# adolliou/euispice_coreg

Hardware: AMD Instinct MI355X
Metric: lag-points/sec (whole node) on 2048² grid, 60×60 CRVAL sweep; argmax-shift match (higher is better)
Workload: dtype f64; 1 GPU; headline: Carrington 'fa' 2048x2048 grid lon(200,300) lat(-20,20), 60x60 CRVAL lags arange(-30,30,1) arcsec, small 2048^2 HRIEUV-like, ref 3072^2 FSI-like, order 2, solar_r 1.004; lag_points=3600, parallelism=single GPU, no collective, resident=True, sweeps_in_flight=2, small_stored_f32=True, use_lds=True

## Files before the change

### euispice_coreg_amd/_lib.py

```python
from __future__ import annotations

import ctypes as C
import os

import numpy as np

_HERE = os.path.dirname(os.path.abspath(__file__))
LIB_PATH = os.environ.get("COREG_HIP_LIB", os.path.join(_HERE, "libcoreg_hip.so"))

COREG_OK = 0
COREG_EINVAL, COREG_EHIP, COREG_ESTATE, COREG_ENOTIMPL, COREG_ENOMEM = -1, -2, -3, -4, -5
COREG_F32, COREG_F64 = 0, 1
PROJ_TAN, PROJ_CAR = 0, 1
METHOD_CORRELATION, METHOD_RESIDUS = 0, 1
CDELT_INTENDED, CDELT_REFERENCE = 0, 1


class CoregError(RuntimeError):
    def __init__(self, code, msg):
        super().__init__(f"libcoreg_hip error {code}: {msg}")
        self.code = code


class Wcs2d(C.Structure):
    _fields_ = [("naxis1", C.c_int32), ("naxis2", C.c_int32),
                ("crpix1", C.c_double), ("crpix2", C.c_double),
                ("crval1", C.c_double), ("crval2", C.c_double),
                ("cdelt1", C.c_double), ("cdelt2", C.c_double),
                ("pc1_1", C.c_double), ("pc1_2", C.c_double), ("pc2_1", C.c_double), ("pc2_2", C.c_double),
                ("crota", C.c_double), ("unit_to_deg", C.c_double), ("lonpole", C.c_double),
                ("dsun_obs", C.c_double), ("crln_obs", C.c_double), ("crlt_obs", C.c_double),
                ("latpole", C.c_double), ("proj", C.c_int32), ("reserved", C.c_int32)]


class Lags(C.Structure):
    _fields_ = [("crval1", C.POINTER(C.c_double)), ("n_crval1", C.c_int32),
                ("crval2", C.POINTER(C.c_double)), ("n_crval2", C.c_int32),
                ("cdelt1", C.POINTER(C.c_double)), ("n_cdelt1", C.c_int32),
                ("cdelt2", C.POINTER(C.c_double)), ("n_cdelt2", C.c_int32),
                ("crota", C.POINTER(C.c_double)), ("n_crota", C.c_int32)]


class CarrGrid(C.Structure):
    _fields_ = [("lon0", C.c_double), ("lon1", C.c_double), ("n_lon", C.c_int32),
                ("lat0", C.c_double), ("lat1", C.c_double), ("n_lat", C.c_int32),
                ("lat_cos", C.POINTER(C.c_float)), ("lat_sin", C.POINTER(C.c_float))]


class DiffRot(C.Structure):
    _fields_ = [("delta_t_days", C.c_double), ("c0", C.c_double), ("c1", C.c_double), ("c2", C.c_double)]


class Stats(C.Structure):
    _fields_ = [("sweep_kernel_ms", C.c_double), ("precompute_ms", C.c_double), ("total_gpu_ms", C.c_double),
                ("n_lags", C.c_int64), ("n_grid_points", C.c_int64), ("n_active_points", C.c_int64),
                ("n_sweep_launches", C.c_int64), ("small_is_f32", C.c_int32), ("used_lds", C.c_int32)]


class FitsPixels(C.Structure):
    _fields_ = [("data", C.c_void_p), ("bitpix", C.c_int32), ("reserved", C.c_int32), ("bscale", C.c_double),
                ("bzero", C.c_double)]


class FitsTiled(C.Structure):
    _fields_ = [("heap", C.c_void_p), ("heap_bytes", C.c_int64), ("tile_offset", C.c_void_p), ("tile_nbytes", C.c_void_p),
                ("n_tiles", C.c_int32), ("zbitpix", C.c_int32), ("naxis1", C.c_int32), ("naxis2", C.c_int32),
                ("ztile1", C.c_int32), ("ztile2", C.c_int32), ("blocksize", C.c_int32), ("bytepix", C.c_int32),
                ("quantize", C.c_int32), ("dither0", C.c_int32), ("has_blank", C.c_int32), ("blank", C.c_int32),
                ("zscale", C.c_void_p), ("zzero", C.c_void_p), ("zscale0", C.c_double), ("zzero0", C.c_double),
                ("bscale", C.c_double), ("bzero", C.c_double)]


def _is_tiled(img):
    return hasattr(img, "tile_nbytes") and hasattr(img, "ztile") and getattr(img, "on_gpu", False)


def _fits_tiled(ci):
    off = np.ascontiguousarray(ci.tile_offset, dtype=np.int64)
    nb = np.ascontiguousarray(ci.tile_nbytes, dtype=np.int32)
    keep = [off, nb, ci._heap]
    zs = zz = None
    if ci.zscale is not None and ci.zzero is not None:
        zs = np.ascontiguousarray(ci.zscale, dtype=np.float64)
        zz = np.ascontiguousarray(ci.zzero, dtype=np.float64)
        keep += [zs, zz]
    t = FitsTiled(ci._heap.ctypes.data, int(ci._heap.size), off.ctypes.data, nb.ctypes.data, int(ci.n_tiles), int(ci.zbitpix),
                  int(ci.shape[1]), int(ci.shape[0]), int(ci.ztile[0]), int(ci.ztile[1]), int(ci.blocksize), int(ci.bytepix),
                  int(ci.quantize), int(ci.dither0), int(bool(ci.has_blank)), int(ci.blank),
                  zs.ctypes.data if zs is not None else None, zz.ctypes.data if zz is not None else None,
                  float(ci.zscale0), float(ci.zzero0), float(ci.bscale), float(ci.bzero))
    return t, keep


def decode_tiled_host(ci, out):
    t, keep = _fits_tiled(ci)
    status = np.zeros(ci.n_tiles, dtype=np.int32)
    rc = load_library().coreg_decode_tiled_host(C.byref(t), out.ctypes.data, COREG_F32 if out.dtype == np.float32 else COREG_F64,
                                                status.ctypes.data)
    if rc != COREG_OK:
        raise CoregError(rc, "coreg_decode_tiled_host: bad arguments (unsupported tiling / codec parameters)")
    del keep
    return status


def encode_tiled_host(pixels, tile, bytepix=4, blocksize=32, quantize=0, dither0=1, scale=1.0):
    a = np.ascontiguousarray(pixels)
    if a.ndim != 2:
        raise ValueError("image must be 2-D")
    ny, nx = a.shape
    tx, ty = int(tile[0]), int(tile[1])
    nt = (-(-nx // tx)) * (-(-ny // ty))
    if a.dtype == np.float32:
        dt = COREG_F32
    elif a.dtype == np.float64:
        dt = COREG_F64
    elif a.dtype == np.int32:
        dt = 2
    else:
        raise TypeError("pixels must be float32, float64 or int32 (stored integers)")
    is_float = dt != 2
    n_blocks = nt * (-(-(tx * ty) // int(blocksize)) + 1)
    cap = a.size * int(bytepix) + n_blocks + 8 * nt + 64
    heap = np.empty(cap, dtype=np.uint8)
    nbytes = np.zeros(nt, dtype=np.int32)
    offs = np.zeros(nt, dtype=np.int64)
    zs = np.zeros(nt, dtype=np.float64) if is_float else None
    zz = np.zeros(nt, dtype=np.float64) if is_float else None
    used = C.c_longlong(0)
    rc = load_library().coreg_encode_tiled_host(a.ctypes.data, dt, ny, nx, tx, ty, int(bytepix), int(blocksize), int(quantize),
                                                int(dither0), float(scale), heap.ctypes.data, cap, nbytes.ctypes.data,
                                                offs.ctypes.data, zs.ctypes.data if is_float else None,
                                                zz.ctypes.data if is_float else None, C.byref(used))
    if rc != COREG_OK:
        raise CoregError(rc, "coreg_encode_tiled_host: bad arguments, or a tile's range does not fit 32-bit integers at "
                             "this scale")
    return heap[:used.value].copy(), nbytes, offs, zs, zz


def _is_raw(img):
    return hasattr(img, "bitpix") and hasattr(img, "ptr")


def _fits_pixels(raw) -> FitsPixels:
    if len(raw.shape) != 2:
        raise ValueError("image must be 2-D")
    return FitsPixels(raw.ptr, int(raw.bitpix), 0, float(raw.bscale), float(raw.bzero))


def _image_kind(img):
    if _is_tiled(img):
        return "tiled", int(img.zbitpix) == -32
    if _is_raw(img):
        return "fits", int(img.bitpix) == -32
    return "array", np.asarray(img).dtype == np.float32


def _image_args(img, what="image"):
    kind, f32 = _image_kind(img)
    if kind == "tiled":
        t, keep = _fits_tiled(img)
        return kind, (C.byref(t),), (img, t, keep)
    if kind == "fits":
        px = _fits_pixels(img)
        return kind, (C.byref(px), img.shape[0], img.shape[1]), (img, px)
    if np.ndim(img) != 2:
        raise ValueError(f"{what} must be 2-D")
    a = np.ascontiguousarray(img, dtype=np.float32 if f32 else np.float64)
    return ("f32" if f32 else "f64"), (a.ctypes.data, a.shape[0], a.shape[1]), a


def _sweep_out(n, out_dev_ptr):
    if out_dev_ptr is None:
        out = np.empty(n, dtype=np.float64)
        return out, _P(out.ctypes.data), 0
    return None, _P(int(out_dev_ptr)), 1


_P = C.c_void_p
_WP = C.POINTER(Wcs2d)
SYMBOLS = [
    ("coreg_version", C.c_char_p, []),
    ("coreg_create", C.c_int, [C.POINTER(_P), C.c_int]),
    ("coreg_destroy", None, [_P]),
    ("coreg_last_error", C.c_char_p, [_P]),
    ("coreg_set_stream", C.c_int, [_P, _P]),
    ("coreg_synchronize", C.c_int, [_P]),
    ("coreg_set_small", C.c_int, [_P, _P, C.c_int32, C.c_int32]),
    ("coreg_set_small_f32", C.c_int, [_P, _P, C.c_int32, C.c_int32]),
    ("coreg_set_small_fits", C.c_int, [_P, C.POINTER(FitsPixels), C.c_int32, C.c_int32]),
    ("coreg_prepare_reference_carrington_fits", C.c_int,
     [_P, C.POINTER(FitsPixels), C.c_int32, C.c_int32, _WP, C.POINTER(CarrGrid), C.c_double, C.c_int]),
    ("coreg_prepare_reference_helioprojective_fits", C.c_int,
     [_P, C.POINTER(FitsPixels), C.c_int32, C.c_int32, _WP, _WP, C.c_int]),
    ("coreg_set_small_tiled", C.c_int, [_P, C.POINTER(FitsTiled)]),
    ("coreg_prepare_reference_carrington_tiled", C.c_int,
     [_P, C.POINTER(FitsTiled), _WP, C.POINTER(CarrGrid), C.c_double, C.c_int]),
    ("coreg_prepare_reference_helioprojective_tiled", C.c_int, [_P, C.POINTER(FitsTiled), _WP, _WP, C.c_int]),
    ("coreg_decode_tiled_host", C.c_int, [C.POINTER(FitsTiled), _P, C.c_int, _P]),
    ("coreg_encode_tiled_host", C.c_int, [_P, C.c_int, C.c_int, C.c_int, C.c_int, C.c_int, C.c_int, C.c_int, C.c_int, C.c_int,
                                          C.c_double, _P, C.c_longlong, _P, _P, _P, _P, C.POINTER(C.c_longlong)]),
    ("coreg_threshold_small", C.c_int, [_P, C.c_int, C.c_double, C.c_int, C.c_double, C.POINTER(C.c_longlong)]),
    ("coreg_set_reference_on_grid", C.c_int, [_P, _P, C.c_int, C.c_int32, C.c_int32]),
    ("coreg_prepare_reference_carrington", C.c_int,
     [_P, _P, C.c_int32, C.c_int32, _WP, C.POINTER(CarrGrid), C.c_double, C.c_int]),
    ("coreg_prepare_reference_helioprojective", C.c_int, [_P, _P, C.c_int32, C.c_int32, _WP, _WP, C.c_int]),
    ("coreg_prepare_reference_carrington_f32", C.c_int,
     [_P, _P, C.c_int32, C.c_int32, _WP, C.POINTER(CarrGrid), C.c_double, C.c_int]),
    ("coreg_prepare_reference_helioprojective_f32", C.c_int, [_P, _P, C.c_int32, C.c_int32, _WP, _WP, C.c_int]),
    ("coreg_set_small_from_device", C.c_int, [_P, _P, C.c_int, C.c_int32, C.c_int32]),
    ("coreg_prepare_reference_carrington_from_device", C.c_int,
     [_P, _P, C.c_int, C.c_int32, C.c_int32, _WP, C.POINTER(CarrGrid), C.c_double, C.c_int]),
    ("coreg_prepare_reference_helioprojective_from_device", C.c_int,
     [_P, _P, C.c_int, C.c_int32, C.c_int32, _WP, _WP, C.c_int]),
    ("coreg_get_reference_on_grid", C.c_int, [_P, _P, C.c_int]),
    ("coreg_resample_carrington", C.c_int, [_P, _WP, C.POINTER(CarrGrid), C.c_double, C.c_int, _P]),
    ("coreg_resample_helioprojective", C.c_int, [_P, _WP, _WP, C.c_int, _P]),
    ("coreg_resample_helioprojective_f64", C.c_int, [_P, _WP, _WP, C.c_int, _P]),
    ("coreg_set_reference_rotation", C.c_int, [_P, C.POINTER(DiffRot)]),
    ("coreg_set_small_rotation", C.c_int, [_P, C.POINTER(DiffRot)]),
    ("coreg_sweep_carrington", C.c_int,
     [_P, _WP, C.POINTER(CarrGrid), C.c_double, C.POINTER(Lags), C.c_int, C.c_int, C.c_int, C.c_int64, C.c_int64, _P,
      C.c_int]),
    ("coreg_sweep_helioprojective", C.c_int,
     [_P, _WP, _WP, C.POINTER(Lags), C.c_int, C.c_int, C.c_int, C.c_int64, C.c_int64, _P, C.c_int]),
    ("coreg_sums_size", C.c_int, [_P, C.POINTER(C.c_int64)]),
    ("coreg_copy_sums", C.c_int, [_P, _P, C.c_int]),
    ("coreg_finalize_sums", C.c_int, [_P, _P, C.c_int, _P, C.c_int]),
    ("coreg_get_pivots", C.c_int, [_P, C.POINTER(C.c_double)]),
    ("coreg_set_pivots", C.c_int, [_P, C.POINTER(C.c_double)]),
    ("coreg_last_stats", C.c_int, [_P, C.POINTER(Stats)]),
    ("coreg_last_visit_counts", C.c_int, [_P, C.POINTER(C.c_int64)]),
    ("coreg_last_tap_fix", C.c_int, [_P, C.POINTER(C.c_int64)]),
    ("coreg_set_option", C.c_int, [_P, C.c_char_p, C.c_int64]),
    ("coreg_shift_header", C.c_int,
     [_WP, C.c_double, C.c_double, C.c_double, C.c_double, C.c_double, C.c_int, _WP]),
    ("coreg_homography", C.c_int, [_WP, _WP, C.POINTER(C.c_double)]),
    ("coreg_lag_homography", C.c_int,
     [_WP, _WP, C.POINTER(Lags), C.POINTER(C.c_int32), C.c_int, C.POINTER(C.c_double)]),
    ("coreg_carrington_origin", C.c_int, [_WP, C.POINTER(C.c_double), C.POINTER(C.c_double)]),
    ("coreg_diffrot_table", C.c_int, [C.POINTER(CarrGrid), C.POINTER(DiffRot), _P]),
    ("coreg_car_map", C.c_int, [_WP, _WP, C.c_int64, _P, _P, _P, _P]),
    ("coreg_wcslib_pixel_to_pixel", C.c_int, [_WP, _WP, C.c_int64, _P, _P, _P, _P, _P, _P]),
    ("coreg_car_tile_margin", C.c_int, [_WP, _WP, C.c_int32, C.c_double, C.POINTER(C.c_double)]),
    ("coreg_nansum_planes_be", C.c_int, [_P, C.c_int32, C.c_int64, _P, C.c_int32, _P]),
    ("coreg_fit_gaussian2d", C.c_int,
     [C.c_int32, _P, _P, _P, _P, _P, _P, C.c_int32, C.c_double, C.c_double, C.c_double, C.c_int32, _P,
      C.POINTER(C.c_int32), C.POINTER(C.c_int32)]),
    ("coreg_set_context_frames", C.c_int, [_P, C.c_int32, C.c_int32, C.c_int32, C.c_int, _WP, C.POINTER(_P)]),
    ("coreg_context_frame_from_small", C.c_int, [_P, C.c_int32]),
    ("coreg_sweep_context", C.c_int,
     [_P, _WP, _WP, C.POINTER(C.c_int32), C.POINTER(Lags), C.c_int, C.c_int, C.c_int, C.c_int, C.c_double, C.c_int,
      C.c_double, C.c_int64, C.c_int64, _P, C.c_int]),
    ("coreg_context_lag_headers", C.c_int,
     [_WP, _WP, C.c_double, C.c_double, C.c_double, C.c_double, C.c_double, C.c_int, _WP, _WP, _WP]),
    ("coreg_device_count", C.c_int, []),
    ("coreg_physical_device_count", C.c_int, []),
    ("coreg_multi_create", C.c_int, [C.POINTER(_P), C.c_int, C.POINTER(C.c_int)]),
    ("coreg_multi_destroy", None, [_P]),
    ("coreg_multi_size", C.c_int, [_P]),
    ("coreg_multi_handle", _P, [_P, C.c_int]),
    ("coreg_multi_last_error", C.c_char_p, [_P]),
    ("coreg_multi_collective", C.c_char_p, [_P]),
    ("coreg_multi_rccl_status", C.c_char_p, [_P]),
    ("coreg_multi_last_mode", C.c_int, [_P]),
    ("coreg_multi_set_option", C.c_int, [_P, C.c_char_p, C.c_int64]),
    ("coreg_multi_set_small", C.c_int, [_P, _P, C.c_int, C.c_int32, C.c_int32]),
    ("coreg_multi_set_small_fits", C.c_int, [_P, C.POINTER(FitsPixels), C.c_int32, C.c_int32]),
    ("coreg_multi_prepare_reference_carrington_fits", C.c_int,
     [_P, C.POINTER(FitsPixels), C.c_int32, C.c_int32, _WP, C.POINTER(CarrGrid), C.c_double, C.c_int]),
    ("coreg_multi_prepare_reference_helioprojective_fits", C.c_int,
     [_P, C.POINTER(FitsPixels), C.c_int32, C.c_int32, _WP, _WP, C.c_int]),
    ("coreg_multi_set_small_tiled", C.c_int, [_P, C.POINTER(FitsTiled)]),
    ("coreg_multi_prepare_reference_carrington_tiled", C.c_int,
     [_P, C.POINTER(FitsTiled), _WP, C.POINTER(CarrGrid), C.c_double, C.c_int]),
    ("coreg_multi_prepare_reference_helioprojective_tiled", C.c_int, [_P, C.POINTER(FitsTiled), _WP, _WP, C.c_int]),
    ("coreg_multi_threshold_small", C.c_int, [_P, C.c_int, C.c_double, C.c_int, C.c_double, C.POINTER(C.c_longlong)]),
    ("coreg_multi_set_reference_on_grid", C.c_int, [_P, _P, C.c_int, C.c_int32, C.c_int32]),
    ("coreg_multi_prepare_reference_carrington", C.c_int,
     [_P, _P, C.c_int, C.c_int32, C.c_int32, _WP, C.POINTER(CarrGrid), C.c_double, C.c_int]),
    ("coreg_multi_prepare_reference_helioprojective", C.c_int, [_P, _P, C.c_int, C.c_int32, C.c_int32, _WP, _WP, C.c_int]),
    ("coreg_multi_set_reference_rotation", C.c_int, [_P, C.POINTER(DiffRot)]),
    ("coreg_multi_set_small_rotation", C.c_int, [_P, C.POINTER(DiffRot)]),
    ("coreg_multi_sweep_carrington", C.c_int,
     [_P, _WP, C.POINTER(CarrGrid), C.c_double, C.POINTER(Lags), C.c_int, C.c_int, C.c_int, _P]),
    ("coreg_multi_sweep_helioprojective", C.c_int, [_P, _WP, _WP, C.POINTER(Lags), C.c_int, C.c_int, C.c_int, _P]),
    ("coreg_multi_last_stats", C.c_int, [_P, C.c_int, C.POINTER(Stats)]),
    ("coreg_multi_plan", C.c_int,
     [C.c_int32, C.c_int32, C.c_int64, C.c_int32, C.c_int32, C.POINTER(C.c_int32), C.POINTER(C.c_int32),
      C.POINTER(C.c_int32), C.POINTER(C.c_int32)]),
]

_lib = None


def _preload_torch_hip_runtime():
    import importlib.util
    import sys
    if "torch" in sys.modules or os.environ.get("COREG_NO_TORCH_PRELOAD", "0") == "1":
        return
    try:
        spec = importlib.util.find_spec("torch")
    except (ImportError, ValueError):
        return
    if spec is None or not spec.submodule_search_locations:
        return
    libdir = os.path.join(list(spec.submodule_search_locations)[0], "lib")
    cand = os.path.join(libdir, "libamdhip64.so")
    if os.path.exists(cand):
        try:
            C.CDLL(cand, mode=C.RTLD_GLOBAL)
        except OSError:
            return
        rccl = os.path.join(libdir, "librccl.so")
        if os.path.exists(rccl):
            os.environ.setdefault("COREG_RCCL_LIB", rccl)


def load_library():
    global _lib
    if _lib is not None:
        return _lib
    _preload_torch_hip_runtime()
    if not os.path.exists(LIB_PATH):
        raise ImportError(
            f"{LIB_PATH} not found: the HIP extension has not been built. "
            "Run `python -c 'import __graft_entry__ as g; g.build()'` at the repo root "
            "(hipcc --offload-arch=gfx950). There is no CPU fallback.")
    lib = C.CDLL(LIB_PATH)
    for name, restype, argtypes in SYMBOLS:
        fn = getattr(lib, name)
        fn.restype = restype
        fn.argtypes = argtypes
    _lib = lib
    return lib


_UNIT_TO_DEG = {"deg": 1.0, "arcsec": 1.0 / 3600.0, "arcmin": 1.0 / 60.0, "rad": 180.0 / np.pi, "mas": 1.0 / 3.6e6}


def unit_to_deg(unit) -> float:
    u = str(unit).strip()
    if u not in _UNIT_TO_DEG:
        raise ValueError(f"unsupported CUNIT {unit!r}")
    return _UNIT_TO_DEG[u]


def wcs_from_header(hdr, carrington=False) -> Wcs2d:
    w = Wcs2d()
    if "ZNAXIS1" in hdr:
        w.naxis1, w.naxis2 = int(hdr["ZNAXIS1"]), int(hdr["ZNAXIS2"])
    else:
        w.naxis1, w.naxis2 = int(hdr.get("NAXIS1", 0)), int(hdr.get("NAXIS2", 0))
    w.crpix1, w.crpix2 = float(hdr["CRPIX1"]), float(hdr["CRPIX2"])
    w.crval1, w.crval2 = float(hdr["CRVAL1"]), float(hdr["CRVAL2"])
    w.cdelt1, w.cdelt2 = float(hdr["CDELT1"]), float(hdr["CDELT2"])
    w.pc1_1, w.pc1_2 = float(hdr.get("PC1_1", 1.0)), float(hdr.get("PC1_2", 0.0))
    w.pc2_1, w.pc2_2 = float(hdr.get("PC2_1", 0.0)), float(hdr.get("PC2_2", 1.0))
    w.crota = float(hdr["CROTA"] if "CROTA" in hdr else hdr.get("CROTA2", 0.0))
    u1 = hdr.get("CUNIT1", "deg")
    if str(u1).strip() != str(hdr.get("CUNIT2", u1)).strip():
        raise ValueError("CUNIT1 and CUNIT2 must be equal")
    w.unit_to_deg = unit_to_deg(u1)
    if str(hdr.get("CTYPE1", "")).strip().upper().endswith("-CAR"):
        w.proj = PROJ_CAR
        w.lonpole = float(hdr["LONPOLE"]) if "LONPOLE" in hdr else float("nan")
    else:
        w.proj = PROJ_TAN
        w.lonpole = float(hdr.get("LONPOLE", 180.0))
    w.latpole = float(hdr["LATPOLE"]) if "LATPOLE" in hdr else float("nan")
    if carrington:
        w.dsun_obs = float(hdr["DSUN_OBS"])
        w.crln_obs = float(hdr["CRLN_OBS"])
        w.crlt_obs = float(hdr["CRLT_OBS"])
    return w


def _dptr(a):
    return a.ctypes.data_as(C.POINTER(C.c_double))


class LagSet:

    def __init__(self, crval1, crval2, cdelt1, cdelt2, crota):
        def arr(v):
            return np.ascontiguousarray(np.atleast_1d(np.asarray([0.0] if v is None else v, dtype=np.float64)))

        self.arrays = [arr(crval1), arr(crval2), arr(cdelt1), arr(cdelt2), arr(crota)]
        a = self.arrays
        self.c = Lags(_dptr(a[0]), len(a[0]), _dptr(a[1]), len(a[1]), _dptr(a[2]), len(a[2]), _dptr(a[3]), len(a[3]),
                      _dptr(a[4]), len(a[4]))
        self.shape = tuple(len(x) for x in a)
        self.size = int(np.prod(self.shape))


class Grid:

    def __init__(self, lonlims, latlims, shape, numpy_lat_trig=True):
        self.n_lon, self.n_lat = int(shape[0]), int(shape[1])
        self._cos = self._sin = None
        cp = sp = None
        if numpy_lat_trig:
            lat = np.radians(np.linspace(latlims[0], latlims[1], self.n_lat, dtype=np.float32))
            self._cos = np.ascontiguousarray(np.cos(lat), dtype=np.float32)
            self._sin = np.ascontiguousarray(np.sin(lat), dtype=np.float32)
            cp = self._cos.ctypes.data_as(C.POINTER(C.c_float))
            sp = self._sin.ctypes.data_as(C.POINTER(C.c_float))
        self.c = CarrGrid(float(lonlims[0]), float(lonlims[1]), self.n_lon, float(latlims[0]), float(latlims[1]),
                          self.n_lat, cp, sp)


class _ImageIntake:

    def _intake(self, stem, img, what, *tail):
        kind, args, keep = _image_args(img, what)
        suffix, dtype_arg = self._variants[kind]
        if dtype_arg:
            args = (args[0], COREG_F32 if kind == "f32" else COREG_F64) + args[1:]
        self._chk(getattr(self._lib, self._prefix + stem + suffix)(getattr(self, self._ptr), *args, *tail))
        return kind, keep

    def set_small(self, img):
        previous = getattr(self, "_small_keepalive", None)
        kind, keep = self._intake("set_small", img, "small image")
        if kind in ("fits", "f32"):
            self._small_keepalive = keep
            del previous

    def drop_small_keepalive(self):
        self._small_keepalive = None

    def set_rotation(self, role, rot):
        if role not in ("reference", "small"):
            raise ValueError("role must be 'reference' or 'small'")
        fn = getattr(self._lib, f"{self._prefix}set_{role}_rotation")
        arg = None if rot is None else C.byref(DiffRot(*(float(v) for v in rot)))
        self._chk(fn(getattr(self, self._ptr), arg))

    def prepare_reference_carrington(self, large, hdr_large, grid: Grid, solar_r, order=2):
        w = wcs_from_header(hdr_large, carrington=True)
        self.reference_tag = None
        self._intake("prepare_reference_carrington", large, "reference image", C.byref(w), C.byref(grid.c),
                     float(solar_r), int(order))

    def prepare_reference_helioprojective(self, large, hdr_large, hdr_small, order=2):
        wl, ws = wcs_from_header(hdr_large), wcs_from_header(hdr_small)
        self.reference_tag = None
        self._intake("prepare_reference_helioprojective", large, "reference image", C.byref(wl), C.byref(ws), int(order))


class CoregHandle(_ImageIntake):
    _prefix, _ptr = "coreg_", "_h"
    _variants = {"tiled": ("_tiled", False), "fits": ("_fits", False), "f32": ("_f32", False), "f64": ("", False)}

    def __init__(self, device=-1):
        self._lib = load_library()
        self._h = _P()
        rc = self._lib.coreg_create(C.byref(self._h), int(device))
        if rc != COREG_OK:
            self._h = None
            raise CoregError(rc, "coreg_create failed (no HIP device visible?)")
        self.reference_tag = None

    def close(self):
        if getattr(self, "_h", None):
            self._lib.coreg_destroy(self._h)
            self._h = None

    def __del__(self):
        try:
            self.close()
        except Exception:
            pass

    def __enter__(self):
        return self

    def __exit__(self, *exc):
        self.close()

    def _chk(self, rc):
        if rc != COREG_OK:
            raise CoregError(rc, self._lib.coreg_last_error(self._h).decode("utf-8", "replace"))

    def set_option(self, name, value):
        self._chk(self._lib.coreg_set_option(self._h, name.encode(), int(value)))

    def set_stream(self, stream_ptr):
        self._chk(self._lib.coreg_set_stream(self._h, _P(stream_ptr)))

    def synchronize(self):
        self._chk(self._lib.coreg_synchronize(self._h))

    def threshold_small(self, vmin=None, vmax=None) -> int:
        n = C.c_longlong(0)
        self._chk(self._lib.coreg_threshold_small(self._h, int(vmin is not None), float(vmin or 0.0),
                                                  int(vmax is not None), float(vmax or 0.0), C.byref(n)))
        return int(n.value)

    def set_reference_on_grid(self, ref):
        ref = np.ascontiguousarray(ref)
        if ref.ndim != 2 or ref.dtype not in (np.float32, np.float64):
            raise ValueError("reference on grid must be a 2-D float32/float64 array")
        dt = COREG_F32 if ref.dtype == np.float32 else COREG_F64
        self.reference_tag = None
        self._chk(self._lib.coreg_set_reference_on_grid(self._h, ref.ctypes.data, dt, ref.shape[0], ref.shape[1]))

    @staticmethod
    def _dev_dtype(dtype):
        dt = np.dtype(dtype)
        if dt == np.float32:
            return COREG_F32
        if dt == np.float64:
            return COREG_F64
        raise ValueError("device images must be float32 or float64")

    def set_small_from_device(self, dev_ptr, shape, dtype=np.float32):
        self._chk(self._lib.coreg_set_small_from_device(self._h, _P(int(dev_ptr)), self._dev_dtype(dtype),
                                                        int(shape[0]), int(shape[1])))

    def prepare_reference_carrington_from_device(self, dev_ptr, shape, dtype, hdr_large, grid: Grid, solar_r, order=2):
        w = wcs_from_header(hdr_large, carrington=True)
        self.reference_tag = None
        self._chk(self._lib.coreg_prepare_reference_carrington_from_device(
            self._h, _P(int(dev_ptr)), self._dev_dtype(dtype), int(shape[0]), int(shape[1]), C.byref(w),
            C.byref(grid.c), float(solar_r), int(order)))

    def prepare_reference_helioprojective_from_device(self, dev_ptr, shape, dtype, hdr_large, hdr_small, order=2):
        wl, ws = wcs_from_header(hdr_large), wcs_from_header(hdr_small)
        self.reference_tag = None
        self._chk(self._lib.coreg_prepare_reference_helioprojective_from_device(
            self._h, _P(int(dev_ptr)), self._dev_dtype(dtype), int(shape[0]), int(shape[1]), C.byref(wl), C.byref(ws),
            int(order)))

    def get_reference_on_grid(self, shape, dtype):
        out = np.empty(shape, dtype=dtype)
        dt = COREG_F32 if out.dtype == np.float32 else COREG_F64
        self._chk(self._lib.coreg_get_reference_on_grid(self._h, out.ctypes.data, dt))
        return out

    def resample_carrington(self, hdr, grid: Grid, solar_r, order=2):
        w = wcs_from_header(hdr, carrington=True)
        out = np.empty((grid.n_lat, grid.n_lon), dtype=np.float64)
        self._chk(self._lib.coreg_resample_carrington(self._h, C.byref(w), C.byref(grid.c), float(solar_r), int(order),
                                                      out.ctypes.data))
        return out

    def resample_helioprojective(self, hdr_target, hdr, order=2, dtype=np.float32):
        wt, w = wcs_from_header(hdr_target), wcs_from_header(hdr)
        out = np.empty((wt.naxis2, wt.naxis1), dtype=dtype)
        fn = self._lib.coreg_resample_helioprojective if out.dtype == np.float32 else \
            self._lib.coreg_resample_helioprojective_f64
        self._chk(fn(self._h, C.byref(wt), C.byref(w), int(order), out.ctypes.data))
        return out

    def sweep_carrington(self, hdr_small, grid: Grid, solar_r, lags: LagSet, order=2, method=METHOD_CORRELATION,
                         cdelt_semantics=CDELT_INTENDED, lag_begin=0, lag_end=None, out_dev_ptr=None):
        lag_end = lags.size if lag_end is None else int(lag_end)
        w = wcs_from_header(hdr_small, carrington=True)
        out, ptr, on_dev = _sweep_out(lag_end - lag_begin, out_dev_ptr)
        self._chk(self._lib.coreg_sweep_carrington(self._h, C.byref(w), C.byref(grid.c), float(solar_r),
                                                   C.byref(lags.c), int(order), int(method), int(cdelt_semantics),
                                                   int(lag_begin), lag_end, ptr, on_dev))
        return out

    def sweep_helioprojective(self, hdr_target, hdr_small, lags: LagSet, order=2, method=METHOD_CORRELATION,
                              cdelt_semantics=CDELT_INTENDED, lag_begin=0, lag_end=None, out_dev_ptr=None):
        lag_end = lags.size if lag_end is None else int(lag_end)
        wt, w = wcs_from_header(hdr_target), wcs_from_header(hdr_small)
        out, ptr, on_dev = _sweep_out(lag_end - lag_begin, out_dev_ptr)
        self._chk(self._lib.coreg_sweep_helioprojective(self._h, C.byref(wt), C.byref(w), C.byref(lags.c), int(order),
                                                        int(method), int(cdelt_semantics), int(lag_begin), lag_end,
                                                        ptr, on_dev))
        return out

    def set_context_frames(self, frames, headers, dtype=None):
        frames = list(frames)
        if len(frames) != len(headers) or not frames:
            raise ValueError("one header per frame, at least one frame")

        kinds = [_image_kind(f) for f in frames]
        if dtype is None:
            dtype = np.float32 if all(f32 for _, f32 in kinds) else np.float64
        dtype = np.dtype(dtype)
        shape = tuple(frames[0].shape)
        if any(tuple(f.shape) != shape for f in frames) or len(shape) != 2:
            raise ValueError("all frames must be 2-D images of one shape")
        hdrs = (Wcs2d * len(frames))(*[wcs_from_header(hh) for hh in headers])
        host = []
        ptrs = (_P * len(frames))()
        for k, f in enumerate(frames):
            if kinds[k][0] != "array":
                continue
            a = np.ascontiguousarray(f, dtype=dtype)
            host.append(a)
            ptrs[k] = a.ctypes.data
        self._chk(self._lib.coreg_set_context_frames(self._h, len(frames), shape[0], shape[1],
                                                     COREG_F32 if dtype == np.float32 else COREG_F64, hdrs, ptrs))
        for k, f in enumerate(frames):
            if kinds[k][0] != "array":
                self.set_small(f)
                self._chk(self._lib.coreg_context_frame_from_small(self._h, k))
        self._context_frames = (len(frames), shape, dtype)

    def sweep_context(self, hdr_target, hdr_small, col_frame, lags: LagSet, order=2, method=METHOD_CORRELATION,
                      cdelt_semantics=CDELT_INTENDED, vmin=None, vmax=None, lag_begin=0, lag_end=None, out_dev_ptr=None):
        lag_end = lags.size if lag_end is None else int(lag_end)
        wt, w = wcs_from_header(hdr_target), wcs_from_header(hdr_small)
        cf = np.ascontiguousarray(col_frame, dtype=np.int32)
        if cf.size != w.naxis1:
            raise ValueError("col_frame needs one entry per raster column")
        out, ptr, on_dev = _sweep_out(lag_end - lag_begin, out_dev_ptr)
        self._chk(self._lib.coreg_sweep_context(
            self._h, C.byref(wt), C.byref(w), cf.ctypes.data_as(C.POINTER(C.c_int32)), C.byref(lags.c), int(order),
            int(method), int(cdelt_semantics), int(vmin is not None), float(0.0 if vmin is None else vmin),
            int(vmax is not None), float(0.0 if vmax is None else vmax), int(lag_begin), lag_end, ptr, on_dev))
        return out

    def set_point_shard(self, rank, world):
        self.set_option("shard_world", int(world))
        self.set_option("shard_rank", int(rank))

    def sums_size(self) -> int:
        n = C.c_int64(0)
        self._chk(self._lib.coreg_sums_size(self._h, C.byref(n)))
        return int(n.value)

    def copy_sums(self, dst_ptr=None):
        if dst_ptr is not None:
            self._chk(self._lib.coreg_copy_sums(self._h, _P(int(dst_ptr)), 1))
            return None
        out = np.empty(self.sums_size(), dtype=np.float64)
        self._chk(self._lib.coreg_copy_sums(self._h, out.ctypes.data, 0))
        return out

    def finalize_sums(self, sums, n_out, out_dev_ptr=None):
        if isinstance(sums, np.ndarray):
            sums = np.ascontiguousarray(sums, dtype=np.float64)
            sptr, s_dev = sums.ctypes.data, 0
        else:
            sptr, s_dev = int(sums), 1
        if out_dev_ptr is None:
            out = np.empty(int(n_out), dtype=np.float64)
            self._chk(self._lib.coreg_finalize_sums(self._h, _P(sptr), s_dev, out.ctypes.data, 0))
            return out
        self._chk(self._lib.coreg_finalize_sums(self._h, _P(sptr), s_dev, _P(int(out_dev_ptr)), 1))
        return None

    def get_pivots(self):
        p = (C.c_double * 2)()
        self._chk(self._lib.coreg_get_pivots(self._h, p))
        return float(p[0]), float(p[1])

    def set_pivots(self, pivot_ref, pivot_small):
        p = (C.c_double * 2)(float(pivot_ref), float(pivot_small))
        self._chk(self._lib.coreg_set_pivots(self._h, p))

    def last_stats(self) -> dict:
        s = Stats()
        self._chk(self._lib.coreg_last_stats(self._h, C.byref(s)))
        return {f: getattr(s, f) for f, _ in Stats._fields_}

    def last_visit_counts(self) -> dict:
        c = (C.c_int64 * 6)()
        self._chk(self._lib.coreg_last_visit_counts(self._h, c))
        return {"visits": c[0], "lds": c[1], "interior": c[2], "all_finite": c[3], "refined_lag_points": c[4],
                "flagged_not_refined": c[5]}


    def last_tap_fix(self) -> dict:
        c = (C.c_int64 * 3)()
        self._chk(self._lib.coreg_last_tap_fix(self._h, c))
        return {"samples": c[0], "lag_points": c[1], "overflow": bool(c[2])}


class _HandleView(CoregHandle):

    def __init__(self, lib, ptr):
        self._lib = lib
        self._h = _P(ptr)
        self.reference_tag = None

    def close(self):
        self._h = None


MULTI_MODES = {0: "none", 1: "blocks", 2: "slices", 3: "points", 4: "combos"}


def device_count() -> int:
    return max(0, int(load_library().coreg_device_count()))


def physical_device_count() -> int:
    return max(0, int(load_library().coreg_physical_device_count()))


def multi_plan(n_crval1, n_crval2, n_inner, world, per_combo_launch=True):
    mode, gc, g1, g2 = C.c_int32(), C.c_int32(), C.c_int32(), C.c_int32()
    rc = load_library().coreg_multi_plan(int(n_crval1), int(n_crval2), int(n_inner), int(world), int(per_combo_launch),
                                         C.byref(mode), C.byref(gc), C.byref(g1), C.byref(g2))
    if rc != COREG_OK:
        raise CoregError(rc, "coreg_multi_plan: bad arguments")
    return MULTI_MODES[mode.value], gc.value, g1.value, g2.value


class MultiHandle(_ImageIntake):
    _prefix, _ptr = "coreg_multi_", "_m"
    _variants = {"tiled": ("_tiled", False), "fits": ("_fits", False), "f32": ("", True), "f64": ("", True)}

    def __init__(self, n_devices=0, device_ids=None):
        self._lib = load_library()
        self._m = _P()
        ids = None
        if device_ids is not None:
            ids = (C.c_int * len(device_ids))(*[int(d) for d in device_ids])
            n_devices = len(device_ids)
        rc = self._lib.coreg_multi_create(C.byref(self._m), int(n_devices), ids)
        if rc != COREG_OK:
            self._m = None
            raise CoregError(rc, "coreg_multi_create failed (no HIP device visible?)")
        self.reference_tag = None
        self.size = int(self._lib.coreg_multi_size(self._m))
        self.primary = _HandleView(self._lib, self._lib.coreg_multi_handle(self._m, 0))

    def close(self):
        if getattr(self, "_m", None):
            self.primary.close()
            self._lib.coreg_multi_destroy(self._m)
            self._m = None

    def __del__(self):
        try:
            self.close()
        except Exception:
            pass

    def __enter__(self):
        return self

    def __exit__(self, *exc):
        self.close()

    def _chk(self, rc):
        if rc != COREG_OK:
            raise CoregError(rc, self._lib.coreg_multi_last_error(self._m).decode("utf-8", "replace"))

    @property
    def collective(self) -> str:
        return self._lib.coreg_multi_collective(self._m).decode()

    @property
    def rccl_status(self) -> str:
        return self._lib.coreg_multi_rccl_status(self._m).decode()

    @property
    def last_mode(self) -> str:
        return MULTI_MODES[int(self._lib.coreg_multi_last_mode(self._m))]

    def handle(self, k) -> CoregHandle:
        ptr = self._lib.coreg_multi_handle(self._m, int(k))
        if not ptr:
            raise IndexError(k)
        return _HandleView(self._lib, ptr)

    def set_option(self, name, value):
        self._chk(self._lib.coreg_multi_set_option(self._m, name.encode(), int(value)))

    def synchronize(self):
        for k in range(self.size):
            self.handle(k).synchronize()

    def threshold_small(self, vmin=None, vmax=None) -> int:
        n = C.c_longlong(0)
        self._chk(self._lib.coreg_multi_threshold_small(self._m, int(vmin is not None), float(vmin or 0.0),
                                                        int(vmax is not None), float(vmax or 0.0), C.byref(n)))
        return int(n.value)

    def set_reference_on_grid(self, ref):
        ref = np.ascontiguousarray(ref)
        if ref.ndim != 2 or ref.dtype not in (np.float32, np.float64):
            raise ValueError("reference on grid must be a 2-D float32/float64 array")
        self.reference_tag = None
        self._chk(self._lib.coreg_multi_set_reference_on_grid(
            self._m, ref.ctypes.data, COREG_F32 if ref.dtype == np.float32 else COREG_F64, ref.shape[0], ref.shape[1]))

    def _whole(self, lags, lag_begin, lag_end):
        if int(lag_begin) != 0 or (lag_end is not None and int(lag_end) != lags.size):
            raise ValueError("a multi-GPU sweep covers the whole lag set (the library cuts it itself)")

    def sweep_carrington(self, hdr_small, grid: Grid, solar_r, lags: LagSet, order=2, method=METHOD_CORRELATION,
                         cdelt_semantics=CDELT_INTENDED, lag_begin=0, lag_end=None):
        self._whole(lags, lag_begin, lag_end)
        w = wcs_from_header(hdr_small, carrington=True)
        out = np.empty(lags.size, dtype=np.float64)
        self._chk(self._lib.coreg_multi_sweep_carrington(self._m, C.byref(w), C.byref(grid.c), float(solar_r),
                                                         C.byref(lags.c), int(order), int(method), int(cdelt_semantics),
                                                         out.ctypes.data))
        return out

    def sweep_helioprojective(self, hdr_target, hdr_small, lags: LagSet, order=2, method=METHOD_CORRELATION,
                              cdelt_semantics=CDELT_INTENDED, lag_begin=0, lag_end=None):
        self._whole(lags, lag_begin, lag_end)
        wt, w = wcs_from_header(hdr_target), wcs_from_header(hdr_small)
        out = np.empty(lags.size, dtype=np.float64)
        self._chk(self._lib.coreg_multi_sweep_helioprojective(self._m, C.byref(wt), C.byref(w), C.byref(lags.c),
                                                              int(order), int(method), int(cdelt_semantics),
                                                              out.ctypes.data))
        return out

    def resample_helioprojective(self, hdr_target, hdr, order=2, dtype=np.float32):
        return self.primary.resample_helioprojective(hdr_target, hdr, order=order, dtype=dtype)

    def get_reference_on_grid(self, shape, dtype):
        return self.primary.get_reference_on_grid(shape, dtype)

    def last_stats(self, k=None):
        def one(i):
            s = Stats()
            self._chk(self._lib.coreg_multi_last_stats(self._m, int(i), C.byref(s)))
            return {f: getattr(s, f) for f, _ in Stats._fields_}
        if k is not None:
            return one(k)
        per = [one(i) for i in range(self.size)]
        out = dict(per[0])
        out["per_device_sweep_kernel_ms"] = [p["sweep_kernel_ms"] for p in per]
        out["n_lags"] = sum(p["n_lags"] for p in per) if self.last_mode != "points" else per[0]["n_lags"]
        out["n_devices"] = self.size
        out["collective"] = self.collective
        out["lag_sharding"] = self.last_mode
        return out


_SHARED = {}


def shared_handle(device=-1, slot=0) -> CoregHandle:
    key = (int(device), int(slot))
    h = _SHARED.get(key)
    if h is None or getattr(h, "_h", None) is None:
        h = CoregHandle(device)
        _SHARED[key] = h
    return h


def shared_multi_handle() -> MultiHandle:
    h = _SHARED.get("multi")
    if h is None or getattr(h, "_m", None) is None:
        h = MultiHandle(0)
        _SHARED["multi"] = h
    return h


def _close_shared():
    for h in list(_SHARED.values()):
        try:
            h.close()
        except Exception:
            pass
    _SHARED.clear()


import atexit

atexit.register(_close_shared)


def shift_header(hdr, d_crval1, d_crval2, d_cdelt1, d_cdelt2, d_crota, cdelt_semantics=CDELT_INTENDED):
    lib = load_library()
    w = wcs_from_header(hdr)
    out = Wcs2d()
    rc = lib.coreg_shift_header(C.byref(w), d_crval1, d_crval2, d_cdelt1, d_cdelt2, d_crota, cdelt_semantics,
                                C.byref(out))
    if rc < 0:
        raise CoregError(rc, "coreg_shift_header")
    return rc, out


def homography(hdr_from, hdr_to):
    lib = load_library()
    a, b = wcs_from_header(hdr_from), wcs_from_header(hdr_to)
    h = (C.c_double * 9)()
    rc = lib.coreg_homography(C.byref(a), C.byref(b), h)
    if rc != COREG_OK:
        raise CoregError(rc, "coreg_homography")
    return np.array(h[:]).reshape(3, 3)


def lag_homography(hdr_target, hdr_small, lags: "LagSet", idx, cdelt_semantics=CDELT_INTENDED):
    lib = load_library()
    a, b = wcs_from_header(hdr_target), wcs_from_header(hdr_small)
    ii = (C.c_int32 * 5)(*[int(i) for i in idx])
    h = (C.c_double * 9)()
    rc = lib.coreg_lag_homography(C.byref(a), C.byref(b), C.byref(lags.c), ii, cdelt_semantics, h)
    if rc < 0:
        raise CoregError(rc, "coreg_lag_homography")
    return rc, np.array(h[:]).reshape(3, 3)


def car_map(hdr_from, hdr_to, px, py):
    lib = load_library()
    px = np.ascontiguousarray(px, dtype=np.float64).ravel()
    py = np.ascontiguousarray(py, dtype=np.float64).ravel()
    ox, oy = np.empty_like(px), np.empty_like(py)
    wf, wt = wcs_from_header(hdr_from), wcs_from_header(hdr_to)
    rc = lib.coreg_car_map(C.byref(wf), C.byref(wt), px.size, px.ctypes.data, py.ctypes.data, ox.ctypes.data,
                           oy.ctypes.data)
    if rc == 1:
        return None
    if rc != COREG_OK:
        raise CoregError(rc, "coreg_car_map: bad arguments")
    return ox, oy


def car_tile_margin(hdr_target, hdr_shifted, tile_w, tile_abs_lat_rad):
    lib = load_library()
    wf, wt = wcs_from_header(hdr_target), wcs_from_header(hdr_shifted)
    m = C.c_double()
    rc = lib.coreg_car_tile_margin(C.byref(wf), C.byref(wt), int(tile_w), float(tile_abs_lat_rad), C.byref(m))
    if rc == 1:
        return None
    if rc != COREG_OK:
        raise CoregError(rc, "coreg_car_tile_margin: bad arguments")
    return m.value


def context_lag_headers(hdr_target, hdr_small, d_crval1, d_crval2, d_cdelt1, d_cdelt2, d_crota,
                        cdelt_semantics=CDELT_INTENDED):
    lib = load_library()
    wt, w = wcs_from_header(hdr_target), wcs_from_header(hdr_small)
    out = [Wcs2d(), Wcs2d(), Wcs2d()]
    rc = lib.coreg_context_lag_headers(C.byref(wt), C.byref(w), float(d_crval1), float(d_crval2), float(d_cdelt1),
                                       float(d_cdelt2), float(d_crota), int(cdelt_semantics), *[C.byref(o) for o in out])
    if rc < 0:
        raise CoregError(rc, "coreg_context_lag_headers: bad arguments")
    return None if rc else tuple(out)


def wcs_to_dict(w: Wcs2d) -> dict:
    unit = {v: k for k, v in _UNIT_TO_DEG.items()}.get(w.unit_to_deg, "deg")
    return {"NAXIS1": w.naxis1, "NAXIS2": w.naxis2, "CRPIX1": w.crpix1, "CRPIX2": w.crpix2, "CRVAL1": w.crval1,
            "CRVAL2": w.crval2, "CDELT1": w.cdelt1, "CDELT2": w.cdelt2, "PC1_1": w.pc1_1, "PC1_2": w.pc1_2,
            "PC2_1": w.pc2_1, "PC2_2": w.pc2_2, "CROTA": w.crota, "CUNIT1": unit, "CUNIT2": unit,
            "CTYPE1": "HPLN-TAN", "CTYPE2": "HPLT-TAN", "LONPOLE": w.lonpole}


def wcslib_pixel_to_pixel(hdr_from, hdr_to, px, py):
    lib = load_library()
    px = np.ascontiguousarray(px, dtype=np.float64).ravel()
    py = np.ascontiguousarray(py, dtype=np.float64).ravel()
    out = [np.empty_like(px) for _ in range(4)]
    wf, wt = wcs_from_header(hdr_from), wcs_from_header(hdr_to)
    rc = lib.coreg_wcslib_pixel_to_pixel(C.byref(wf), C.byref(wt), px.size, px.ctypes.data, py.ctypes.data,
                                         *[o.ctypes.data for o in out])
    if rc != COREG_OK:
        raise CoregError(rc, "coreg_wcslib_pixel_to_pixel")
    return tuple(out)


def nansum_planes_be(cube_be, plane_index):
    a = cube_be
    if a.dtype.kind != "f" or a.dtype.byteorder != ">" or a.dtype.itemsize not in (4, 8) or not a.flags.c_contiguous:
        return None
    idx = np.ascontiguousarray(plane_index, dtype=np.int64)
    if idx.size and (idx.min() < 0 or idx.max() >= a.shape[0]):
        raise IndexError("plane index out of range")
    n_pix = int(np.prod(a.shape[1:]))
    out = np.empty(a.shape[1:], dtype=np.float64)
    rc = load_library().coreg_nansum_planes_be(a.ctypes.data, -8 * a.dtype.itemsize, n_pix, idx.ctypes.data, idx.size,
                                               out.ctypes.data)
    if rc != COREG_OK:
        raise CoregError(rc, "coreg_nansum_planes_be: bad arguments")
    return out


def fit_gaussian2d(x, y, z, p0, lb, ub, jac="2-point", ftol=1e-8, xtol=1e-8, gtol=1e-8, max_nfev=0):
    lib = load_library()
    arrs = [np.ascontiguousarray(np.asarray(a, dtype=np.float64).ravel()) for a in (x, y, z, p0, lb, ub)]
    if not (arrs[0].size == arrs[1].size == arrs[2].size) or any(a.size != 6 for a in arrs[3:]):
        raise ValueError("fit_gaussian2d: x, y, z must have one length; p0, lb, ub six entries")
    if jac not in ("2-point", "analytic"):
        raise ValueError("jac must be '2-point' or 'analytic'")
    popt = np.empty(6)
    nfev, status = C.c_int32(0), C.c_int32(0)
    rc = lib.coreg_fit_gaussian2d(arrs[0].size, *[a.ctypes.data for a in arrs], int(jac == "analytic"), float(ftol),
                                  float(xtol), float(gtol), int(max_nfev), popt.ctypes.data, C.byref(nfev),
                                  C.byref(status))
    if rc != COREG_OK:
        raise CoregError(rc, "coreg_fit_gaussian2d: bad arguments (sizes, bounds, or p0 outside the bounds)")
    return popt, int(status.value), int(nfev.value)


def diffrot_table(grid: Grid, rot):
    out = np.empty(grid.n_lat, dtype=np.float64)
    r = DiffRot(*(float(v) for v in rot))
    rc = load_library().coreg_diffrot_table(C.byref(grid.c), C.byref(r), out.ctypes.data)
    if rc != COREG_OK:
        raise CoregError(rc, "coreg_diffrot_table: bad grid, or a non-finite delta_t / coefficient")
    return out


def carrington_origin(hdr):
    lib = load_library()
    w = wcs_from_header(hdr, carrington=True)
    x0, y0 = C.c_double(), C.c_double()
    rc = lib.coreg_carrington_origin(C.byref(w), C.byref(x0), C.byref(y0))
    if rc != COREG_OK:
        raise CoregError(rc, "coreg_carrington_origin")
    return x0.value, y0.value
```

### euispice_coreg_amd/csrc/abi_host.hpp

```cpp
#pragma once
extern "C" {
int coreg_shift_header(const coreg_wcs2d* ref, double d_crval1, double d_crval2, double d_cdelt1, double d_cdelt2,
                       double d_crota, int cdelt_semantics, coreg_wcs2d* out) {
    if (!ref || !out) return COREG_EINVAL;
    return shift_header(*ref, d_crval1, d_crval2, d_cdelt1, d_cdelt2, d_crota, cdelt_semantics, out);
}

int coreg_car_map(const coreg_wcs2d* from, const coreg_wcs2d* to, int64_t n, const double* px, const double* py,
                  double* ox, double* oy) {
    if (!from || !to || n < 0 || (n > 0 && (!px || !py || !ox || !oy))) return COREG_EINVAL;
    if (from->proj != COREG_PROJ_CAR || to->proj != COREG_PROJ_CAR) return COREG_EINVAL;
    CarMapHost m;
    if (m.init(*from, *to)) return 1;
    for (int64_t i = 0; i < n; ++i) m.apply(px[i], py[i], &ox[i], &oy[i]);
    return COREG_OK;
}

int coreg_last_visit_counts(coreg_handle* h, int64_t* counts6) {
    int64_t* counts5 = counts6;
    if (!h || !counts5) return COREG_EINVAL;
    RETCHK(bind_device(h));
    HIPCHK(hipStreamSynchronize(h->stream));
    long long info[8] = {0, 0, 0, 0, 0, 0, 0, 0};
    if (h->tile_info.p) HIPCHK(hipMemcpy(info, h->tile_info.p, 7 * sizeof(long long), hipMemcpyDeviceToHost));
    for (int k = 0; k < 4; ++k) counts5[k] = info[3 + k];
    long long refined[2] = {0, 0};
    if (h->counters.p) HIPCHK(hipMemcpy(refined, h->counters.p, sizeof(refined), hipMemcpyDeviceToHost));
    counts5[4] = refined[0];
    counts6[5] = refined[1];
    return COREG_OK;
}

int coreg_last_tap_fix(coreg_handle* h, int64_t* counts3) {
    if (!h || !counts3) return COREG_EINVAL;
    for (int k = 0; k < 3; ++k) counts3[k] = h->tap_last[k];
    return COREG_OK;
}

int coreg_car_tile_margin(const coreg_wcs2d* hdr_target, const coreg_wcs2d* hdr_shifted, int32_t tile_w,
                          double tile_abs_lat_rad, double* margin_px) {
    if (!hdr_target || !hdr_shifted || !margin_px || tile_w < 1 || tile_w > kTilePts) return COREG_EINVAL;
    if (hdr_target->proj != COREG_PROJ_CAR || hdr_shifted->proj != COREG_PROJ_CAR) return COREG_EINVAL;
    CarMapHost m;
    if (m.init(*hdr_target, *hdr_shifted)) return 1;
    *margin_px = car_tile_margin(car_box_c(*hdr_target, *hdr_shifted, tile_w), tile_abs_lat_rad + car_pole_sep(m.r));
    return COREG_OK;
}

int coreg_homography(const coreg_wcs2d* from, const coreg_wcs2d* to, double* h9) {
    if (!from || !to || !h9) return COREG_EINVAL;
    if (from->proj != COREG_PROJ_TAN || to->proj != COREG_PROJ_TAN) return COREG_ENOTIMPL;
    homography(*from, *to, h9);
    return COREG_OK;
}

int coreg_lag_homography(const coreg_wcs2d* hdr_target, const coreg_wcs2d* hdr_small, const coreg_lags* lags,
                         const int32_t idx[5], int cdelt_semantics, double* h9) {
    if (!hdr_target || !hdr_small || !lags || !idx || !h9) return COREG_EINVAL;
    if (hdr_target->proj != COREG_PROJ_TAN || hdr_small->proj != COREG_PROJ_TAN) return COREG_ENOTIMPL;
    if (idx[0] < 0 || idx[0] >= lags->n_crval1 || idx[1] < 0 || idx[1] >= lags->n_crval2 || idx[2] < 0 ||
        idx[2] >= lags->n_cdelt1 || idx[3] < 0 || idx[3] >= lags->n_cdelt2 || idx[4] < 0 || idx[4] >= lags->n_crota)
        return COREG_EINVAL;
    coreg_wcs2d hc;
    if (shift_header(*hdr_small, 0.0, 0.0, lags->cdelt1[idx[2]], lags->cdelt2[idx[3]], lags->crota[idx[4]],
                     cdelt_semantics, &hc))
        return 1;
    HomographyFamily fam;
    fam.init(*hdr_target, *hdr_small, lags->crval1, lags->n_crval1, lags->crval2, lags->n_crval2);
    fam.get(HomographyFamily::combo(hc), idx[0], idx[1], h9);
    return COREG_OK;
}

int coreg_wcslib_pixel_to_pixel(const coreg_wcs2d* from, const coreg_wcs2d* to, int64_t n, const double* px,
                                const double* py, double* ox, double* oy, double* lng, double* lat) {
    if (!from || !to || n < 0 || (n > 0 && (!px || !py || !ox || !oy))) return COREG_EINVAL;
    if (from->proj == COREG_PROJ_CAR && to->proj == COREG_PROJ_CAR) {
        WcslibCar a, b;
        a.init(*from);
        b.init(*to);
        if (!a.valid || !b.valid) return COREG_EINVAL;
        for (int64_t i = 0; i < n; ++i) {
            double l, t;
            a.p2s(px[i], py[i], &l, &t);
            if (lng) lng[i] = l;
            if (lat) lat[i] = t;
            b.s2p(l, t, &ox[i], &oy[i]);
        }
        return COREG_OK;
    }
    if (from->proj != COREG_PROJ_TAN || to->proj != COREG_PROJ_TAN) return COREG_ENOTIMPL;
    WcslibTan a, b;
    a.init(*from);
    b.init(*to);
    for (int64_t i = 0; i < n; ++i) {
        double l, t;
        a.p2s(px[i], py[i], &l, &t);
        if (lng) lng[i] = l;
        if (lat) lat[i] = t;
        b.s2p(ang2pipi_deg(l), ang2pipi_deg(t), &ox[i], &oy[i]);
    }
    return COREG_OK;
}

int coreg_carrington_origin(const coreg_wcs2d* hdr, double* x0, double* y0) {
    if (!hdr || !x0 || !y0) return COREG_EINVAL;
    carr_origin(*hdr, x0, y0);
    return COREG_OK;
}

int coreg_diffrot_table(const coreg_carr_grid* grid, const coreg_diffrot* rot, double* dx) {
    if (!grid || !rot || !dx || grid->n_lon < 1 || grid->n_lat < 1 || !diffrot_valid(*rot)) return COREG_EINVAL;
    CarrTables t;
    carr_tables(*grid, 0.0, t);
    std::vector<double> v;
    diffrot_dx(t.sin_lat.data(), grid->n_lat, *rot, v);
    std::copy(v.begin(), v.end(), dx);
    return COREG_OK;
}

int coreg_nansum_planes_be(const void* cube, int32_t bitpix, int64_t n_pixels, const int64_t* plane_index, int32_t n_sel,
                           double* out) {
    if (!cube || !out || n_pixels < 0 || n_sel < 0 || (n_sel > 0 && !plane_index) || (bitpix != -32 && bitpix != -64))
        return COREG_EINVAL;
    for (int k = 0; k < n_sel; ++k)
        if (plane_index[k] < 0) return COREG_EINVAL;
    auto work = [&](int64_t lo, int64_t hi) {
        for (int64_t p = lo; p < hi; ++p) out[p] = 0.0;
        for (int k = 0; k < n_sel; ++k) {
            if (bitpix == -32) {
                const uint32_t* src = (const uint32_t*)cube + (size_t)plane_index[k] * (size_t)n_pixels;
                for (int64_t p = lo; p < hi; ++p) {
                    const uint32_t u = __builtin_bswap32(src[p]);
                    float f;
                    std::memcpy(&f, &u, sizeof(f));
                    const double v = (double)f;
                    out[p] += (v != v) ? 0.0 : v;
                }
            } else {
                const uint64_t* src = (const uint64_t*)cube + (size_t)plane_index[k] * (size_t)n_pixels;
                for (int64_t p = lo; p < hi; ++p) {
                    const uint64_t u = __builtin_bswap64(src[p]);
                    double v;
                    std::memcpy(&v, &u, sizeof(v));
                    out[p] += (v != v) ? 0.0 : v;
                }
            }
        }
    };
    parallel_for(n_pixels, (unsigned)std::min<int64_t>(12, n_pixels * std::max(n_sel, 1) / (1 << 18)), 0, work);
    return COREG_OK;
}

int coreg_fit_gaussian2d(int32_t m, const double* x, const double* y, const double* z, const double* p0,
                         const double* lb, const double* ub, int32_t jac, double ftol, double xtol, double gtol,
                         int32_t max_nfev, double* popt, int32_t* nfev, int32_t* status) {
    if (!x || !y || !z || !p0 || !lb || !ub || !popt || !status || m < 1 || m > coregfit::MMAX) return COREG_EINVAL;
    coregfit::Problem P{m, x, y, z};
    int n = 0;
    const int st = coregfit::fit(P, p0, lb, ub, jac != 0, ftol > 0 ? ftol : 1e-8, xtol > 0 ? xtol : 1e-8,
                                 gtol > 0 ? gtol : 1e-8, max_nfev, popt, &n, nullptr);
    if (st == -2) return COREG_EINVAL;
    if (nfev) *nfev = n;
    *status = st;
    return COREG_OK;
}

}
```

### euispice_coreg_amd/csrc/abi_sweeps.hpp

```cpp
#pragma once
namespace {
struct SweepCall {
    const coreg_lags* lags = nullptr;
    LagDims d;
    int order = 0, method = 0, sem = 0;
    long long lag_begin = 0, lag_end = 0, n_out = 0;
    double* corr_out = nullptr;
    int out_on_device = 0;
    double* out_dev = nullptr;
    long long row() const { return (long long)d.n2 * d.nc; }
    int i1_lo() const { return (int)(lag_begin / row()); }
    int i1_hi() const { return (int)((lag_end - 1) / row()); }
};

template <typename OwnChecks>
int open_sweep(coreg_handle* h, ComboRange combo, OwnChecks own_checks, const coreg_lags* lags, int order, int method,
               int sem, int64_t lag_begin, int64_t lag_end, int grid_w, int grid_h, const char* grid_what,
               double* corr_out, int out_on_device, SweepCall* call) {
    if (method != COREG_METHOD_CORRELATION && method != COREG_METHOD_RESIDUS)
        return fail(h, COREG_ENOTIMPL, "method must be COREG_METHOD_CORRELATION or COREG_METHOD_RESIDUS");
    RETCHK(check_order(h, order));
    RETCHK(own_checks());
    RETCHK(check_lags(h, lags, &call->d, lag_begin, lag_end, combo));
    RETCHK(bind_device_nowait(h));
    if (h->ref.p && (h->gW != grid_w || h->gH != grid_h))
        return fail(h, COREG_EINVAL, std::string("reference-on-grid shape differs from ") + grid_what);
    call->lags = lags;
    call->order = order;
    call->method = method;
    call->sem = sem;
    call->lag_begin = lag_begin;
    call->lag_end = lag_end;
    call->n_out = lag_end - lag_begin;
    call->corr_out = corr_out;
    call->out_on_device = out_on_device;
    return begin_sweep(h, call->n_out, corr_out, out_on_device, &call->out_dev);
}

int close_sweep(coreg_handle* h, const SweepCall& call) {
    return end_sweep(h, call.n_out, call.corr_out, call.out_on_device, call.out_dev);
}

int close_empty_sweep(coreg_handle* h, const SweepCall& call) {
    RETCHK(fill_nan(h, call.out_dev, call.n_out));
    return close_sweep(h, call);
}

template <typename MapAt>
Geometry local_geometry(const coreg_wcs2d& target, const SweepCall& call, MapAt at) {
    const coreg_lags& l = *call.lags;
    int e1[3], e2[3];
    extreme_lags(l.crval1, call.d.n1, e1);
    extreme_lags(l.crval2, call.d.n2, e2);
    const double v1 = l.crval1[e1[1]], v2 = l.crval2[e2[1]];
    const double s1 = lag_step(l.crval1, call.d.n1), s2 = lag_step(l.crval2, call.d.n2);
    const double u = target.naxis1 * 0.5, v = target.naxis2 * 0.5;
    double x0, y0, xi, yi, xj, yj, xa, ya, xb, yb;
    Geometry g;
    if (!at(v1, v2, u, v, &x0, &y0) || !at(v1, v2, u + 1, v, &xi, &yi) || !at(v1, v2, u, v + 1, &xj, &yj) ||
        !at(v1 + s1, v2, u, v, &xa, &ya) || !at(v1, v2 + s2, u, v, &xb, &yb))
        return g;
    g.dx_di = xi - x0;
    g.dy_di = yi - y0;
    g.dx_dj = xj - x0;
    g.dy_dj = yj - y0;
    g.ax = xa - x0;
    g.ay = ya - y0;
    g.bx = xb - x0;
    g.by = yb - y0;
    return g;
}

Plan plan_sweep(coreg_handle* h, const Geometry& geo, const SweepCall& call) {
    return choose_plan(h, geo, call.i1_hi() - call.i1_lo() + 1, call.d.n2, h->opt_use_lds ? lds_window_elems(h) : (1LL << 40));
}

bool combo_slots(const SweepCall& call, const coreg_wcs2d& small, const Plan& plan, long long c, coreg_wcs2d* hc,
                 SlotList* slots) {
    const long long first = (call.lag_begin - c + call.d.nc - 1) / call.d.nc;
    if (first * call.d.nc + c >= call.lag_end) return false;
    int i3, i4, i5;
    call.d.inner(c, &i3, &i4, &i5);
    if (shift_header(small, 0.0, 0.0, call.lags->cdelt1[i3], call.lags->cdelt2[i4], call.lags->crota[i5], call.sem, hc))
        return false;
    build_slots(call.d, c, call.lag_begin, call.lag_end, plan.sw, plan.sh, slots);
    return slots->n_batches > 0;
}

template <int MODE>
int precompute(coreg_handle* h, const PrecomputeArgs& pa, int n_tiles, int n_groups, int n_batches, bool launch = true) {
    if (launch) RETCHK(launch_precompute<MODE>(h, pa, n_tiles, n_groups, n_batches));
    h->last_precompute = [pa, n_tiles, n_groups, n_batches](coreg_handle* hh) {
        return launch_precompute<MODE>(hh, pa, n_tiles, n_groups, n_batches);
    };
    return COREG_OK;
}

int finalize_pending(coreg_handle* h, const coreg_handle::PendingFinalize& pf, long long* refine_count, double* out_dev,
                     FinalizeArgs* f) {
    *f = FinalizeArgs{};
    RETCHK(fill_refine(h, &f->refine, pf.refine.mode, pf.refine.order, pf.refine.lane_params, pf.refine.car_inv,
                       pf.n_slots));
    f->refine.enabled = pf.refine.enabled;
    f->refine_count = refine_count;
    f->partials = h->sums.as<double>() + pf.slot_off;
    f->n_groups = 1;
    f->n_slots = pf.n_slots;
    f->part_stride = h->sums_slots;
    f->out_index = h->fin_outidx.as<long long>() + pf.slot_off;
    f->lag_begin = pf.lag_begin;
    f->out = out_dev;
    f->residus = pf.residus;
    f->n_required = (long long)h->gW * h->gH;
    hipLaunchKernelGGL(k_finalize, dim3((unsigned)((pf.n_slots + kFinSlots - 1) / kFinSlots)),
                       dim3(kFinSlots * kFinLanes), 0, h->stream, *f);
    return COREG_OK;
}
}

extern "C" {
int coreg_sweep_carrington(coreg_handle* h, const coreg_wcs2d* hdr_small, const coreg_carr_grid* grid, double solar_r,
                           const coreg_lags* lags, int order, int method, int cdelt_semantics, int64_t lag_begin,
                           int64_t lag_end, double* corr_out, int out_on_device) {
    if (!h) return COREG_EINVAL;
    const ComboRange combo = take_combo_range(h);
    trace("sweep_carrington: enter");
    if (!hdr_small || !grid) return fail(h, COREG_EINVAL, "sweep_carrington: null header/grid");
    auto own_checks = [&] {
        RETCHK(check_wcs(h, hdr_small, true));
        RETCHK(check_grid(h, grid));
        if (!std::isfinite(solar_r) || !(solar_r > 0.0)) return fail(h, COREG_EINVAL, "solar_r must be positive");
        return COREG_OK;
    };
    SweepCall call;
    RETCHK(open_sweep(h, combo, own_checks, lags, order, method, cdelt_semantics, lag_begin, lag_end, grid->n_lon,
                      grid->n_lat, "the Carrington grid", corr_out, out_on_device, &call));
    if (call.n_out == 0) return close_sweep(h, call);
    const LagDims& d = call.d;

    CarrDev cd;
    std::memset(&cd, 0, sizeof(cd));
    RETCHK(upload_carr_tables(h, *grid, *hdr_small, &cd, h->has_rot_small ? &h->rot_small : nullptr));
    double row_slip = 0.0;
    for (size_t j = 1; j < h->tabs.dx.size(); ++j)
        row_slip = std::max(row_slip, std::fabs(h->tabs.dx[j] - h->tabs.dx[j - 1]));
    row_slip *= kDeg2Rad * (1.0 + 1e-9);

    Geometry geo;
    {
        const CarrCommon c0 = carr_common(*hdr_small, solar_r);
        const int ic = grid->n_lon / 2, jc = grid->n_lat / 2;
        double a0, a1, b0, b1, c0x, c0y;
        carr_term_host(h->tabs, c0, ic, jc, &a0, &a1);
        carr_term_host(h->tabs, c0, std::min(ic + 1, grid->n_lon - 1), jc, &b0, &b1);
        carr_term_host(h->tabs, c0, ic, std::min(jc + 1, grid->n_lat - 1), &c0x, &c0y);
        geo.dx_di = b0 - a0;
        geo.dy_di = b1 - a1;
        geo.dx_dj = c0x - a0;
        geo.dy_dj = c0y - a1;
        const double s1 = lag_step(lags->crval1, d.n1), s2 = lag_step(lags->crval2, d.n2);
        geo.ax = c0.cr * s1 / hdr_small->cdelt1;
        geo.ay = c0.sr * s1 / hdr_small->cdelt2;
        geo.bx = c0.sr * s2 / hdr_small->cdelt1;
        geo.by = c0.cr * s2 / hdr_small->cdelt2;
    }
    const Plan plan = plan_sweep(h, geo, call);
    PrecomputeArgs pa;
    int n_tiles;
    RETCHK(setup_precompute(h, plan, method, &pa, &n_tiles));

    struct Launch {
        size_t slot_off;
        int n_batches;
        CarrCommon cc;
        double f0lo, f0hi, f1lo, f1hi;
    };
    std::vector<Launch> launches;
    std::vector<double> params;
    std::vector<long long> outidx;
    SlotList slots;
    for (long long c = 0; c < d.nc; ++c) {
        coreg_wcs2d hc;
        if (!combo_slots(call, *hdr_small, plan, c, &hc, &slots)) continue;
        const size_t ns = slots.i1.size();
        Launch L;
        L.slot_off = outidx.size();
        L.n_batches = slots.n_batches;
        L.cc = carr_common(hc, solar_r);
        const size_t pbase = params.size();
        params.resize(pbase + 2 * ns);
        double x0min = 1e300, x0max = -1e300, y0min = 1e300, y0max = -1e300;
        const double roll = hc.crota * kDeg2Rad;
        const double rc = std::cos(roll), rs = std::sin(roll);
        const double nan = std::numeric_limits<double>::quiet_NaN();
        for (size_t s = 0; s < ns; ++s) {
            if (slots.outidx[s] < 0) {
                params[pbase + s] = nan;
                params[pbase + ns + s] = nan;
                continue;
            }
            const double v1 = hdr_small->crval1 + lags->crval1[slots.i1[s]];
            const double v2 = hdr_small->crval2 + lags->crval2[slots.i2[s]];
            const double dx = rc * v1 + rs * v2;
            const double dy = -rs * v1 + rc * v2;
            const double x0 = (hc.crpix1 - 1) - dx / hc.cdelt1;
            const double y0 = (hc.crpix2 - 1) - dy / hc.cdelt2;
            params[pbase + s] = x0;
            params[pbase + ns + s] = y0;
            x0min = std::min(x0min, x0);
            x0max = std::max(x0max, x0);
            y0min = std::min(y0min, y0);
            y0max = std::max(y0max, y0);
        }
        outidx.insert(outidx.end(), slots.outidx.begin(), slots.outidx.end());
        L.f0lo = -x0max;
        L.f0hi = (double)(h->sW - 1) - x0min;
        L.f1lo = -y0max;
        L.f1hi = (double)(h->sH - 1) - y0min;
        launches.push_back(L);
    }
    if (launches.empty()) return close_empty_sweep(h, call);
    RETCHK(upload_plan(h, params, outidx, call.out_dev, call.n_out));
    RETCHK(prepare_sharded(h, outidx.size(), call.n_out, lag_begin));
    for (const Launch& L : launches) {
        set_carr_common(&cd, L.cc);
        pa.carr = cd;
        pa.f0lo = L.f0lo;
        pa.f0hi = L.f0hi;
        pa.f1lo = L.f1lo;
        pa.f1hi = L.f1hi;
        {
            const double dm1 = L.cc.dist - 1.0;
            pa.tile_skip = (h->opt_tile_skip && dm1 > 0.0) ? 1 : 0;
            const double per_rad = pa.tile_skip ? (1.0 / dm1 + 1.0 / (dm1 * dm1)) * kRad2Deg * 3600.0 : 0.0;
            pa.lip_x = per_rad / std::fabs(L.cc.cdelt1) * (1.0 + 1e-9);
            pa.lip_y = per_rad / std::fabs(L.cc.cdelt2) * (1.0 + 1e-9);
            pa.dlon = grid->n_lon > 1 ? (std::fabs(grid->lon1 - grid->lon0) / (grid->n_lon - 1) * 1.001 + 1e-4) * kDeg2Rad : 0.0;
            pa.dlat = grid->n_lat > 1 ? (std::fabs(grid->lat1 - grid->lat0) / (grid->n_lat - 1) * 1.001 + 1e-4) * kDeg2Rad : 0.0;
            pa.dlat += row_slip;
        }
        RETCHK(precompute<MODE_TRANSLATE>(h, pa, n_tiles, pick_groups(h, L.n_batches, n_tiles), L.n_batches));
        RETCHK(launch_sweep(h, MODE_TRANSLATE, order, method, h->lane_params.as<double>() + 2 * L.slot_off,
                            h->out_index.as<long long>() + L.slot_off, L.n_batches, n_tiles, lag_begin, call.out_dev,
                            nullptr, nullptr, (long long)L.slot_off,
                            pick_pitch(h, plan, h->opt_use_lds ? lds_window_elems(h) : 0, order)));
    }
    return close_sweep(h, call);
}

static int sweep_car(coreg_handle* h, const SweepCall& call, const coreg_wcs2d* hdr_target, const coreg_wcs2d* hdr_small) {
    const coreg_lags* lags = call.lags;
    const LagDims& d = call.d;
    const int order = call.order;
    Mat3 r_target;
    if (car_native_to_celestial(*hdr_target, &r_target))
        return fail(h, COREG_EINVAL, "hdr_target: no valid native pole for this CRVAL2 / LONPOLE (CAR)");
    auto shifted_by = [&](const coreg_wcs2d& base, double v1, double v2) {
        coreg_wcs2d hl = base;
        hl.crval1 = hdr_small->crval1 + v1;
        hl.crval2 = hdr_small->crval2 + v2;
        return hl;
    };
    auto shifted = [&](const coreg_wcs2d& base, int i1, int i2) {
        return shifted_by(base, lags->crval1[i1], lags->crval2[i2]);
    };
    const Plan plan = plan_sweep(h, local_geometry(*hdr_target, call, [&](double v1, double v2, double u, double v,
                                                                        double* x, double* y) {
        CarMapHost m;
        if (m.init(*hdr_target, shifted_by(*hdr_small, v1, v2))) return false;
        m.apply(u, v, x, y);
        return true;
    }), call);

    const int i1_lo = call.i1_lo(), i1_hi = call.i1_hi();
    std::vector<double> rot((size_t)(i1_hi - i1_lo + 1) * d.n2 * 9);
    const double nanv = std::numeric_limits<double>::quiet_NaN();
    for (int i1 = i1_lo; i1 <= i1_hi; ++i1)
        for (int i2 = 0; i2 < d.n2; ++i2) {
            double* r = &rot[((size_t)(i1 - i1_lo) * d.n2 + i2) * 9];
            Mat3 rs;
            if (car_native_to_celestial(shifted(*hdr_small, i1, i2), &rs)) {
                for (int k = 0; k < 9; ++k) r[k] = nanv;
                continue;
            }
            const Mat3 m = mat_mul(mat_T(rs), r_target);
            for (int a = 0; a < 3; ++a)
                for (int b = 0; b < 3; ++b) r[3 * a + b] = (double)m.m[a][b];
        }

    struct Launch {
        size_t slot_off;
        int n_batches;
        LaunchU inv;
        bool identity;
        coreg_wcs2d hc;
        std::vector<int> i1, i2;
        std::vector<unsigned char> tap_skip;
        bool tap_any = false;
    };
    std::vector<Launch> launches;
    std::vector<double> params;
    std::vector<long long> outidx;
    SlotList slots;
    long long identity_out = -1;
    BorderFix id_fix;
    std::vector<std::vector<unsigned char>> id_flags;
    auto same_header = [](const coreg_wcs2d& a, const coreg_wcs2d& b) {
        auto eq = [](double x, double y) { return x == y || (x != x && y != y); };
        return a.proj == b.proj && a.crpix1 == b.crpix1 && a.crpix2 == b.crpix2 && a.crval1 == b.crval1 &&
               a.crval2 == b.crval2 && a.cdelt1 == b.cdelt1 && a.cdelt2 == b.cdelt2 && a.pc1_1 == b.pc1_1 &&
               a.pc1_2 == b.pc1_2 && a.pc2_1 == b.pc2_1 && a.pc2_2 == b.pc2_2 && a.unit_to_deg == b.unit_to_deg &&
               eq(a.lonpole, b.lonpole) && eq(a.latpole, b.latpole) && a.naxis1 == b.naxis1 && a.naxis2 == b.naxis2;
    };
    for (long long c = 0; c < d.nc; ++c) {
        coreg_wcs2d hc;
        if (!combo_slots(call, *hdr_small, plan, c, &hc, &slots)) continue;
        const size_t ns = slots.i1.size();
        Launch L;
        L.slot_off = outidx.size();
        L.n_batches = slots.n_batches;
        std::memset(&L.inv, 0, sizeof(L.inv));
        set_affine(&L.inv, car_native_to_pix(hc));
        L.inv.box_c = car_box_c(*hdr_target, hc, plan.tile_w);
        L.inv.pole_sep = 0.0;
        L.identity = false;
        const size_t pbase = params.size();
        params.resize(pbase + 9 * ns);
        for (size_t s = 0; s < ns; ++s) {
            bool pad = slots.outidx[s] < 0;
            if (!pad && h->opt_border_fix && identity_out < 0 && h->gW == h->sW && h->gH == h->sH) {
                const coreg_wcs2d hl = shifted(hc, slots.i1[s], slots.i2[s]);
                if (same_header(hl, *hdr_target)) {
                    identity_out = slots.outidx[s];
                    slots.outidx[s] = -1;
                    pad = true;
                }
            }
            const double* r = &rot[((size_t)(slots.i1[s] - i1_lo) * d.n2 + slots.i2[s]) * 9];
            for (int k = 0; k < 9; ++k) params[pbase + (size_t)k * ns + s] = pad ? nanv : r[k];
            if (!pad && r[8] == r[8]) L.inv.pole_sep = std::max(L.inv.pole_sep, car_pole_sep(r));
            unsigned char skip = 1;
            if (!pad && h->opt_tap_fix && r[8] == r[8] && h->gW == h->sW && h->gH == h->sH) {
                const coreg_wcs2d hl = shifted(hc, slots.i1[s], slots.i2[s]);
                if (hl.crval1 == hdr_target->crval1 || hl.crval2 == hdr_target->crval2) skip = 0;
            }
            L.tap_skip.push_back(skip);
            L.tap_any = L.tap_any || !skip;
        }
        L.hc = hc;
        L.i1 = slots.i1;
        L.i2 = slots.i2;
        outidx.insert(outidx.end(), slots.outidx.begin(), slots.outidx.end());
        launches.push_back(L);
    }
    if (identity_out >= 0) {
        Launch L;
        std::memset(&L.inv, 0, sizeof(L.inv));
        L.slot_off = outidx.size();
        L.n_batches = 1;
        L.identity = true;
        const size_t ns = kBlock, pbase = params.size();
        params.resize(pbase + 9 * ns, nanv);
        const double ident[9] = {1, 0, 0, 0, 1, 0, 0, 0, 1};
        for (int k = 0; k < 9; ++k) params[pbase + (size_t)k * ns] = ident[k];
        outidx.push_back(identity_out);
        outidx.insert(outidx.end(), ns - 1, -1);
        launches.push_back(L);
        {
            AxisInvariance inv;
            inv.rows = inv.cols = true;
            BorderFix::Item it;
            it.slot = 0;
            it.first = 0;
            wcslib_dropped_border_pixels(h, *hdr_target, *hdr_target, inv, &id_fix.pixels);
            it.n = (int)id_fix.pixels.size();
            it.flags_off = -1;
            if (order & 1) {
                it.flags_off = 0;
                id_flags.push_back(wcslib_tap_shift_flags(h, *hdr_target, *hdr_target, inv));
            }
            if (it.n > 0 || it.flags_off >= 0) id_fix.items.push_back(it);
        }
    }
    if (launches.empty()) return close_empty_sweep(h, call);
    trace("sweep_helioprojective: lane parameters laid out");
    RETCHK(upload_plan(h, params, outidx, call.out_dev, call.n_out));
    RETCHK(prepare_sharded(h, outidx.size(), call.n_out, call.lag_begin));
    trace("sweep_helioprojective: plan in page-locked memory");

    PrecomputeArgs pa;
    int n_tiles;
    RETCHK(setup_precompute(h, plan, call.method, &pa, &n_tiles));
    set_affine(&pa.car_fwd, car_pix_to_native(*hdr_target));
    const double inf = std::numeric_limits<double>::infinity();
    pa.f0lo = pa.f1lo = -inf;
    pa.f0hi = pa.f1hi = inf;
    if (!id_fix.items.empty()) RETCHK(upload_border_pixels(h, id_fix.pixels));
    RETCHK(upload_border_flags(h, id_flags));
    int last_groups = -1, last_batches = -1;
    for (const Launch& L : launches) {
        if (L.identity) {
            PrecomputeArgs pi = pa;
            std::memset(&pi.car_fwd, 0, sizeof(pi.car_fwd));
            RETCHK(precompute<MODE_HOMOGRAPHY>(h, pi, n_tiles, pick_groups(h, 1, n_tiles), 1));
            last_groups = last_batches = -1;
            RETCHK(launch_sweep(h, MODE_HOMOGRAPHY, order, call.method, h->lane_params.as<double>() + 9 * L.slot_off,
                                h->out_index.as<long long>() + L.slot_off, 1, n_tiles, call.lag_begin, call.out_dev, nullptr,
                                &id_fix, (long long)L.slot_off));
            continue;
        }
        const int ng = pick_groups(h, L.n_batches, n_tiles);
        RETCHK(precompute<MODE_CAR>(h, pa, n_tiles, ng, L.n_batches, ng != last_groups || L.n_batches != last_batches));
        last_groups = ng;
        last_batches = L.n_batches;
        BorderFix tap;
        if (L.tap_any) {
            const double box[4] = {0.0, (double)(h->gW - 1), 0.0, (double)(h->gH - 1)};
            h->tap_last[0] = h->tap_last[1] = h->tap_last[2] = 0;
            RETCHK(prepare_tap_fix(
                h, MODE_CAR, order, *hdr_target, (long long)L.tap_skip.size(), L.tap_skip, box,
                [&](int slot) { return shifted(L.hc, L.i1[(size_t)slot], L.i2[(size_t)slot]); }, &tap,
                h->lane_params.as<double>() + 9 * L.slot_off, &L.inv, &pa.car_fwd));
        }
        RETCHK(launch_sweep(h, MODE_CAR, order, call.method, h->lane_params.as<double>() + 9 * L.slot_off,
                            h->out_index.as<long long>() + L.slot_off, L.n_batches, n_tiles, call.lag_begin, call.out_dev,
                            &L.inv, L.tap_any ? &tap : nullptr, (long long)L.slot_off));
    }
    return close_sweep(h, call);
}

int coreg_sweep_helioprojective(coreg_handle* h, const coreg_wcs2d* hdr_target, const coreg_wcs2d* hdr_small,
                                const coreg_lags* lags, int order, int method, int cdelt_semantics, int64_t lag_begin,
                                int64_t lag_end, double* corr_out, int out_on_device) {
    if (!h) return COREG_EINVAL;
    const ComboRange combo = take_combo_range(h);
    if (!hdr_target || !hdr_small) return fail(h, COREG_EINVAL, "sweep_helioprojective: null header");
    if (hdr_target->proj != hdr_small->proj || (hdr_small->proj != COREG_PROJ_TAN && hdr_small->proj != COREG_PROJ_CAR))
        return fail(h, COREG_ENOTIMPL, "both headers must be TAN (helioprojective) or both CAR (Carrington maps)");
    auto own_checks = [&] {
        RETCHK(check_wcs(h, hdr_target, false));
        return check_wcs(h, hdr_small, false);
    };
    SweepCall call;
    RETCHK(open_sweep(h, combo, own_checks, lags, order, method, cdelt_semantics, lag_begin, lag_end,
                      hdr_target->naxis1, hdr_target->naxis2, "hdr_target NAXIS1/NAXIS2", corr_out, out_on_device, &call));
    if (call.n_out == 0) return close_sweep(h, call);
    if (hdr_small->proj == COREG_PROJ_CAR) return sweep_car(h, call, hdr_target, hdr_small);
    const LagDims& d = call.d;

    trace("sweep_helioprojective: enter (checks done)");
    const Plan plan = plan_sweep(h, local_geometry(*hdr_target, call, [&](double v1, double v2, double u, double v,
                                                                        double* x, double* y) {
        coreg_wcs2d hl = *hdr_small;
        hl.crval1 = hdr_small->crval1 + v1;
        hl.crval2 = hdr_small->crval2 + v2;
        double hm[9];
        homography(*hdr_target, hl, hm);
        apply_h(hm, u, v, x, y);
        return true;
    }), call);

    std::vector<long long> outidx;
    int n_batches = 0;
    double fx0 = 1e300, fx1 = -1e300, fy0 = 1e300, fy1 = -1e300;
    HomographyFamily fam;
    fam.init(*hdr_target, *hdr_small, lags->crval1, d.n1, lags->crval2, d.n2, d.nc > 1);
    BorderFix fix;
    std::vector<std::vector<unsigned char>> flags_host;
    const bool tap_fixing = h->opt_tap_fix != 0;
    std::vector<coreg_wcs2d> tap_combo;
    std::vector<int> tap_slot_combo, tap_slot_i1, tap_slot_i2;
    std::vector<unsigned char> tap_skip;
    const int i1_lo = call.i1_lo(), i1_hi = call.i1_hi();
    fam.fill_products(i1_lo, i1_hi);
    const double nanv = std::numeric_limits<double>::quiet_NaN();
    struct ComboPlan {
        bool used = false;
        coreg_wcs2d hc;
        SlotList slots;
        std::vector<double> hs;
        double box[4] = {1e300, -1e300, 1e300, -1e300};
    };
    std::vector<ComboPlan> cps((size_t)d.nc);
    int e1[3], e2[3];
    extreme_lags(lags->crval1 + i1_lo, i1_hi - i1_lo + 1, e1);
    extreme_lags(lags->crval2, d.n2, e2);
    auto plan_combo = [&](long long c) {
        ComboPlan& cp = cps[(size_t)c];
        cp.used = combo_slots(call, *hdr_small, plan, c, &cp.hc, &cp.slots);
        if (!cp.used) return;
        const Mat3d B = HomographyFamily::combo(cp.hc);
        const size_t n = cp.slots.i1.size();
        cp.hs.resize(9 * n);
        for (size_t s = 0; s < n; ++s) {
            double* hm = &cp.hs[9 * s];
            if (cp.slots.outidx[s] < 0) {
                for (int k = 0; k < 9; ++k) hm[k] = nanv;
            } else {
                fam.get(B, cp.slots.i1[s], cp.slots.i2[s], hm);
            }
        }
        for (int a1 = 0; a1 < 3; ++a1)
            for (int a2 = 0; a2 < 3; ++a2) {
                coreg_wcs2d hl = cp.hc;
                hl.crval1 = hdr_small->crval1 + lags->crval1[i1_lo + e1[a1]];
                hl.crval2 = hdr_small->crval2 + lags->crval2[e2[a2]];
                double hi[9];
                homography(hl, *hdr_target, hi);
                for (int k = 0; k < 4; ++k) {
                    double px, py;
                    apply_h(hi, (k & 1) ? (double)(h->sW - 1) : 0.0, (k & 2) ? (double)(h->sH - 1) : 0.0, &px, &py);
                    cp.box[0] = std::min(cp.box[0], px);
                    cp.box[1] = std::max(cp.box[1], px);
                    cp.box[2] = std::min(cp.box[2], py);
                    cp.box[3] = std::max(cp.box[3], py);
                }
            }
    };
    trace("sweep_helioprojective: geometry + lag family ready");
    const unsigned plan_threads = (d.nc >= 2 && (long long)d.nc * d.n1 * d.n2 >= 16384) ? 8u : 1u;
    parallel_for(d.nc, plan_threads, 1, [&](long long lo, long long hi) {
        for (long long c = lo; c < hi; ++c) plan_combo(c);
    });
    for (long long c = 0; c < d.nc; ++c) {
        ComboPlan& cp = cps[(size_t)c];
        if (!cp.used) continue;
        const SlotList& slots = cp.slots;
        const coreg_wcs2d& hc = cp.hc;
        if (tap_fixing) {
            tap_combo.push_back(hc);
            for (size_t s = 0; s < slots.i1.size(); ++s) {
                tap_slot_combo.push_back((int)tap_combo.size() - 1);
                tap_slot_i1.push_back(slots.outidx[s] < 0 ? 0 : slots.i1[s]);
                tap_slot_i2.push_back(slots.outidx[s] < 0 ? 0 : slots.i2[s]);
                tap_skip.push_back(slots.outidx[s] < 0 ? 1 : 0);
            }
        }
        if (h->opt_border_fix) {
            for (size_t s = 0; s < slots.i1.size(); ++s) {
                if (slots.outidx[s] < 0) continue;
                const double v1 = hdr_small->crval1 + lags->crval1[slots.i1[s]];
                const double v2 = hdr_small->crval2 + lags->crval2[slots.i2[s]];
                if (v1 != hdr_target->crval1 || v2 != hdr_target->crval2) continue;
                coreg_wcs2d hl = hc;
                hl.crval1 = v1;
                hl.crval2 = v2;
                double* hm = &cp.hs[9 * s];
                const AxisInvariance inv = snap_invariant_axes(*hdr_target, hl, h->gW, h->gH, hm);
                if (inv.rows || inv.cols) {
                    BorderFix::Item it;
                    it.slot = (long long)(outidx.size() + s);
                    it.first = (int)fix.pixels.size();
                    wcslib_dropped_border_pixels(h, *hdr_target, hl, inv, &fix.pixels);
                    it.n = (int)fix.pixels.size() - it.first;
                    it.flags_off = -1;
                    if (order & 1) {
                        it.flags_off = (long long)flags_host.size() * h->gW * h->gH;
                        flags_host.push_back(wcslib_tap_shift_flags(h, *hdr_target, hl, inv));
                    }
                    if (it.n > 0 || it.flags_off >= 0) fix.items.push_back(it);
                    if (tap_fixing) tap_skip[(size_t)it.slot] = 1;
                }
            }
        }
        fx0 = std::min(fx0, cp.box[0]);
        fx1 = std::max(fx1, cp.box[1]);
        fy0 = std::min(fy0, cp.box[2]);
        fy1 = std::max(fy1, cp.box[3]);
        outidx.insert(outidx.end(), slots.outidx.begin(), slots.outidx.end());
        n_batches += slots.n_batches;
    }
    if (n_batches == 0) return close_empty_sweep(h, call);
    trace("sweep_helioprojective: combinations planned");
    const size_t ns = outidx.size();
    std::vector<double> params(9 * ns);
    double eps_max = 0.0;
    {
        std::vector<size_t> off((size_t)d.nc + 1, 0);
        for (long long c = 0; c < d.nc; ++c) off[(size_t)c + 1] = off[(size_t)c] + (cps[(size_t)c].used ? cps[(size_t)c].slots.i1.size() : 0);
        std::vector<double> eps_of((size_t)d.nc, 0.0);
        auto transpose = [&](long long c) {
            const ComboPlan& cp = cps[(size_t)c];
            if (!cp.used) return;
            const size_t n = cp.slots.i1.size(), at = off[(size_t)c];
            double em = 0.0;
            for (size_t s = 0; s < n; ++s) {
                const double* hm = &cp.hs[9 * s];
                for (int k = 0; k < 9; ++k) params[(size_t)k * ns + at + s] = hm[k];
                const double e = std::fabs(hm[6]) * (double)h->gW + std::fabs(hm[7]) * (double)h->gH;
                if (e == e) em = std::max(em, e);
            }
            eps_of[(size_t)c] = em;
        };
        parallel_for(d.nc, plan_threads, 1, [&](long long lo, long long hi) {
            for (long long c = lo; c < hi; ++c) transpose(c);
        });
        for (double e : eps_of) eps_max = std::max(eps_max, e);
    }
    const int sweep_mode = (h->opt_h_series && eps_max < 4.0e-6) ? MODE_HOMOGRAPHY_SERIES : MODE_HOMOGRAPHY;
    RETCHK(upload_plan(h, params, outidx, call.out_dev, call.n_out));
    RETCHK(prepare_sharded(h, outidx.size(), call.n_out, lag_begin));

    PrecomputeArgs pa;
    int n_tiles;
    RETCHK(setup_precompute(h, plan, method, &pa, &n_tiles));
    pa.f0lo = std::floor(fx0) - 3.0;
    pa.f0hi = std::ceil(fx1) + 3.0;
    pa.f1lo = std::floor(fy0) - 3.0;
    pa.f1hi = std::ceil(fy1) + 3.0;
    if (!fix.items.empty()) RETCHK(upload_border_pixels(h, fix.pixels));
    RETCHK(upload_border_flags(h, flags_host));
    RETCHK(precompute<MODE_HOMOGRAPHY>(h, pa, n_tiles, pick_groups(h, n_batches, n_tiles), n_batches));
    h->tap_last[0] = h->tap_last[1] = h->tap_last[2] = 0;
    const double tap_box[4] = {pa.f0lo, pa.f0hi, pa.f1lo, pa.f1hi};
    trace("sweep_helioprojective: precompute launched");
    if (tap_fixing)
        RETCHK(prepare_tap_fix(
            h, sweep_mode, order, *hdr_target, (long long)ns, tap_skip, tap_box,
            [&](int slot) {
                coreg_wcs2d hl = tap_combo[(size_t)tap_slot_combo[(size_t)slot]];
                hl.crval1 = hdr_small->crval1 + lags->crval1[tap_slot_i1[(size_t)slot]];
                hl.crval2 = hdr_small->crval2 + lags->crval2[tap_slot_i2[(size_t)slot]];
                return hl;
            },
            &fix));
    trace("sweep_helioprojective: single-sample scan done");
    RETCHK(launch_sweep(h, sweep_mode, order, method, h->lane_params.as<double>(), h->out_index.as<long long>(), n_batches,
                        n_tiles, lag_begin, call.out_dev, nullptr, &fix, 0,
                        pick_pitch(h, plan, h->opt_use_lds ? lds_window_elems(h) : 0, order)));
    return close_sweep(h, call);
}


int coreg_sums_size(coreg_handle* h, int64_t* n_doubles) {
    if (!h || !n_doubles) return COREG_EINVAL;
    *n_doubles = (int64_t)h->sums_slots * kNumSums;
    return COREG_OK;
}

int coreg_copy_sums(coreg_handle* h, double* dst, int dst_on_device) {
    if (!h || !dst) return COREG_EINVAL;
    if (h->sums_slots <= 0 || h->pending_fin.empty()) return fail(h, COREG_ESTATE, "no point-sharded sweep is pending");
    RETCHK(bind_device(h));
    const size_t bytes = (size_t)h->sums_slots * kNumSums * sizeof(double);
    HIPCHK(hipMemcpyAsync(dst, h->sums.p, bytes, dst_on_device ? hipMemcpyDeviceToDevice : hipMemcpyDeviceToHost,
                          h->stream));
    if (!dst_on_device) HIPCHK(hipStreamSynchronize(h->stream));
    return COREG_OK;
}

int coreg_finalize_sums(coreg_handle* h, const double* sums, int sums_on_device, double* corr_out, int out_on_device) {
    if (!h || !sums) return COREG_EINVAL;
    if (h->sums_slots <= 0 || h->pending_fin.empty()) return fail(h, COREG_ESTATE, "no point-sharded sweep is pending");
    if (!corr_out && h->pending_n_out > 0) return fail(h, COREG_EINVAL, "corr_out is null");
    RETCHK(bind_device(h));
    const long long n_out = h->pending_n_out;
    const size_t bytes = (size_t)h->sums_slots * kNumSums * sizeof(double);
    if ((const void*)sums != h->sums.p) {
        HIPCHK(hipMemcpyAsync(h->sums.p, sums, bytes, sums_on_device ? hipMemcpyDeviceToDevice : hipMemcpyHostToDevice,
                              h->stream));
        if (!sums_on_device) HIPCHK(hipStreamSynchronize(h->stream));
    }
    double* out_dev = corr_out;
    if (!out_on_device) {
        HIPCHK(h->out_dev.reserve((size_t)std::max<long long>(n_out, 1) * sizeof(double)));
        out_dev = h->out_dev.as<double>();
    }
    if (n_out > 0) {
        hipLaunchKernelGGL(k_fill, dim3((unsigned)((n_out + 255) / 256)), dim3(256), 0, h->stream, out_dev,
                           (long long)n_out, std::numeric_limits<double>::quiet_NaN());
        HIPCHK(hipGetLastError());
    }
    const size_t n_pending = h->pending_fin.size();
    size_t points_of = n_pending - 1;
    bool probe_says_nothing_flagged = false;
    if (n_pending > 1) {
        long long* probe = h->counters.as<long long>() + 2;
        HIPCHK(hipMemsetAsync(probe, 0, sizeof(long long), h->stream));
        for (size_t ip = 0; ip < n_pending; ++ip) {
            const coreg_handle::PendingFinalize& pf = h->pending_fin[ip];
            FinalizeArgs f;
            RETCHK(finalize_pending(h, pf, nullptr, out_dev, &f));
            if (f.refine.enabled)
                hipLaunchKernelGGL(k_refine_list, dim3(1), dim3(kListThreads), 0, h->stream, f.refine, pf.n_slots, probe);
        }
        HIPCHK(hipGetLastError());
        long long flagged = 0;
        HIPCHK(hipMemcpyAsync(&flagged, probe, sizeof(flagged), hipMemcpyDeviceToHost, h->stream));
        HIPCHK(hipStreamSynchronize(h->stream));
        probe_says_nothing_flagged = flagged == 0;
    }
    for (size_t ip = 0; ip < n_pending && !probe_says_nothing_flagged; ++ip) {
        const coreg_handle::PendingFinalize& pf = h->pending_fin[ip];
        FinalizeArgs f;
        RETCHK(finalize_pending(h, pf, h->counters.as<long long>(), out_dev, &f));
        const RefineArgs rf = f.refine;
        if (!rf.enabled) continue;
        hipLaunchKernelGGL(k_refine_list, dim3(1), dim3(kListThreads), 0, h->stream, rf, pf.n_slots, h->counters.as<long long>());
        HIPCHK(hipGetLastError());
        int head[2] = {0, 0};
        HIPCHK(hipMemcpyAsync(head, rf.head, sizeof(head), hipMemcpyDeviceToHost, h->stream));
        HIPCHK(hipStreamSynchronize(h->stream));
        if (head[0] == 0) continue;
        if (points_of != ip && pf.replay_precompute) {
            RETCHK(pf.replay_precompute(h));
            points_of = ip;
        }
        RefineArgs rf2 = rf;
        if (!pf.fixes.empty()) {
            HIPCHK(h->rf_fix_slab.reserve((size_t)kNumSums * pf.n_slots * sizeof(double)));
            HIPCHK(hipMemsetAsync(h->rf_fix_slab.p, 0, (size_t)kNumSums * pf.n_slots * sizeof(double), h->stream));
            rf2.fix_slab = h->rf_fix_slab.as<double>();
            RETCHK(launch_fix_kernels(h, pf.fixes, h->rf_fix_slab.as<double>(), rf.slot_pivots, rf.flags));
        }
        RETCHK(launch_refine(h, rf2, pf.n_slots, f.out_index, pf.lag_begin, out_dev, false));
    }
    HIPCHK(hipGetLastError());
    if (!out_on_device && n_out > 0) {
        HIPCHK(hipMemcpyAsync(corr_out, out_dev, (size_t)n_out * sizeof(double), hipMemcpyDeviceToHost, h->stream));
        HIPCHK(hipStreamSynchronize(h->stream));
    }
    return COREG_OK;
}

int coreg_get_pivots(coreg_handle* h, double* pivots2) {
    if (!h || !pivots2) return COREG_EINVAL;
    RETCHK(bind_device(h));
    HIPCHK(hipMemcpyAsync(pivots2, h->pivots.p, 2 * sizeof(double), hipMemcpyDeviceToHost, h->stream));
    HIPCHK(hipStreamSynchronize(h->stream));
    return COREG_OK;
}

int coreg_set_pivots(coreg_handle* h, const double* pivots2) {
    if (!h || !pivots2) return COREG_EINVAL;
    if (!(pivots2[0] == pivots2[0]) || !(pivots2[1] == pivots2[1]) || std::isinf(pivots2[0]) || std::isinf(pivots2[1]))
        return fail(h, COREG_EINVAL, "set_pivots: pivots must be finite");
    RETCHK(bind_device(h));
    HIPCHK(hipMemcpyAsync(h->pivots.p, pivots2, 2 * sizeof(double), hipMemcpyHostToDevice, h->stream));
    HIPCHK(hipStreamSynchronize(h->stream));
    return COREG_OK;
}

int coreg_last_stats(coreg_handle* h, coreg_stats* out) {
    if (!h || !out) return COREG_EINVAL;
    RETCHK(bind_device(h));
    RETCHK(collect_stats(h));
    *out = h->stats;
    return COREG_OK;
}

}
```

### euispice_coreg_amd/csrc/coreg_hip.hip

```cpp
#include <hip/hip_runtime.h>

#include <algorithm>
#include <chrono>
#include <cmath>
#include <cstdio>
#include <cstdlib>
#include <cstring>
#include <limits>
#include <condition_variable>
#include <map>
#include <memory>
#include <mutex>
#include <string>
#include <thread>
#include <functional>
#include <vector>

#include "fit.hpp"
#include "geometry.hpp"
#include "kernels.hpp"
#include <atomic>
#include "ricecomp.hpp"
#include "riceenc.hpp"

using namespace coreg;

#define COREG_VERSION "0.1.0"

#include "host_state.hpp"
#include "host_upload.hpp"
#include "host_plan.hpp"
#include "host_fix_launch.hpp"
#include "host_sweep_launch.hpp"
#include "host_fix_lists.hpp"
#include "host_sweep_io.hpp"
#include "host_context.hpp"


extern "C" {

const char* coreg_version(void) { return "coreg_hip " COREG_VERSION " (gfx950)"; }

int coreg_create(coreg_handle** out, int device) {
    if (!out) return COREG_EINVAL;
    *out = nullptr;
    coreg_handle* h = new (std::nothrow) coreg_handle();
    if (!h) return COREG_ENOMEM;
    int ndev = 0;
    hipError_t e = hipGetDeviceCount(&ndev);
    if (e != hipSuccess || ndev < 1) {
        delete h;
        return COREG_EHIP;
    }
    if (device < 0) {
        if (hipGetDevice(&device) != hipSuccess) device = 0;
    }
    if (device >= ndev) {
        delete h;
        return COREG_EINVAL;
    }
    h->device = device;
    if (hipSetDevice(device) != hipSuccess || hipStreamCreateWithFlags(&h->stream, hipStreamNonBlocking) != hipSuccess ||
        hipEventCreate(&h->ev_end[0]) != hipSuccess ||
        hipEventCreate(&h->ev_end[1]) != hipSuccess || hipEventRecord(h->ev_end[0], h->stream) != hipSuccess ||
        hipEventRecord(h->ev_end[1], h->stream) != hipSuccess ||
        h->pivots.reserve(2 * sizeof(double)) != hipSuccess ||
        hipMemsetAsync(h->pivots.p, 0, 2 * sizeof(double), h->stream) != hipSuccess) {
        h->own_stream = h->stream != nullptr;
        coreg_destroy(h);
        return COREG_EHIP;
    }
    h->own_stream = true;
    std::memset(&h->stats, 0, sizeof(h->stats));
    *out = h;
    return COREG_OK;
}

void coreg_destroy(coreg_handle* h) {
    if (!h) return;
    (void)hipSetDevice(h->device);
    if (h->up_thread.joinable()) {
        {
            std::unique_lock<std::mutex> lk(h->up_m);
            h->up_cv.wait(lk, [&] { return !h->up_busy && !h->up_has; });
            h->up_stop = true;
        }
        h->up_cv.notify_all();
        h->up_thread.join();
    }
    if (h->stream) (void)hipStreamSynchronize(h->stream);
    context_release(h);
    if (h->up_stream) (void)hipStreamSynchronize(h->up_stream);
    for (int k = 0; k < 2; ++k) {
        h->pin_small[k].release();
        if (h->ev_pin_small[k]) (void)hipEventDestroy(h->ev_pin_small[k]);
    }
    DevBuf* bufs[] = {&h->rf_flags, &h->rf_pivots, &h->rf_list, &h->rf_head, &h->rf_partial, &h->small, &h->ref, &h->pivots, &h->red_sum, &h->red_cnt, &h->t_sin_lon, &h->t_cos_lon,
                      &h->t_cos_lat, &h->t_sin_lat, &h->pts, &h->tile_count, &h->tile_list, &h->tile_cum, &h->group_first,
                      &h->tile_info, &h->tile_bbox, &h->counters, &h->lane_params, &h->out_index, &h->partials, &h->out_dev,
                      &h->tmp_img, &h->up_f64, &h->up_flag, &h->up_raw, &h->rice_blob, &h->rice_rand, &h->dec_img, &h->border_dev, &h->sums, &h->fin_outidx, &h->border_flags, &h->fix_partial, &h->rf_fix_slab};
    for (DevBuf* b : bufs) b->release();
    for (int k = 0; k < 2; ++k) {
        h->pin_img[k].release();
        if (h->ev_img[k]) (void)hipEventDestroy(h->ev_img[k]);
    }
    for (auto& e : h->ev_sweep) {
        (void)hipEventDestroy(e.a);
        (void)hipEventDestroy(e.b);
    }
    for (auto& e : h->ev_pre) {
        (void)hipEventDestroy(e.a);
        (void)hipEventDestroy(e.b);
    }
    for (int k = 0; k < 2; ++k) {
        if (h->ev_end[k]) (void)hipEventDestroy(h->ev_end[k]);
        h->pin_plan[k].release();
    }
    h->pin_info.release();
    h->pin_border.release();
    h->bbox_buf.release();
    if (h->aux_stream) (void)hipStreamDestroy(h->aux_stream);
    if (h->up_stream) (void)hipStreamDestroy(h->up_stream);
    if (h->ev_small) (void)hipEventDestroy(h->ev_small);
    if (h->ev_main) (void)hipEventDestroy(h->ev_main);
    h->red_sum_up.release();
    h->red_cnt_up.release();
    if (h->own_stream && h->stream) (void)hipStreamDestroy(h->stream);
    delete h;
}

const char* coreg_last_error(const coreg_handle* h) { return h ? h->err.c_str() : "null handle"; }

int coreg_set_stream(coreg_handle* h, void* hip_stream) {
    if (!h) return COREG_EINVAL;
    RETCHK(bind_device(h));
    RETCHK(collect_stats(h));
    HIPCHK(hipStreamSynchronize(h->stream));
    if (h->own_stream && h->stream) HIPCHK(hipStreamDestroy(h->stream));
    h->stream = (hipStream_t)hip_stream;
    h->own_stream = false;
    return COREG_OK;
}

int coreg_synchronize(coreg_handle* h) {
    if (!h) return COREG_EINVAL;
    RETCHK(bind_device(h));
    HIPCHK(hipStreamSynchronize(h->stream));
    return COREG_OK;
}

int coreg_set_option(coreg_handle* h, const char* name, int64_t value) {
    if (!h || !name) return COREG_EINVAL;
    const std::string n(name);
    if (n == "use_lds") {
        h->opt_use_lds = value ? 1 : 0;
    } else if (n == "clean_path") {
        h->opt_clean_path = value ? 1 : 0;
    } else if (n == "tap_nan_filter") {
        if (value < 0 || value > 2) return fail(h, COREG_EINVAL, "tap_nan_filter must be 0, 1 or 2");
        h->opt_tap_nan_filter = value;
    } else if (n == "overlap_upload") {
        h->opt_overlap_upload = value ? 1 : 0;
    } else if (n == "async_upload") {
        h->opt_async_upload = value ? 1 : 0;
    } else if (n == "refine") {
        h->opt_refine = value ? 1 : 0;
    } else if (n == "refine_cond_log10") {
        if (value < -3 || value > 15) return fail(h, COREG_EINVAL, "refine_cond_log10 must be in [-3, 15]");
        h->opt_refine_cond_log10 = value;
    } else if (n == "refine_max") {
        if (value < 0 || value > 16) return fail(h, COREG_EINVAL, "refine_max must be in [0, 16]");
    } else if (n == "tile_w") {
        if (value != 0 && (value < 1 || value > kTilePts || (value & (value - 1)) != 0))
            return fail(h, COREG_EINVAL, "tile_w must be 0 or a power of two <= 1024");
        h->opt_tile_w = value;
    } else if (n == "n_groups") {
        if (value < 0) return fail(h, COREG_EINVAL, "n_groups must be >= 0");
        h->opt_n_groups = value;
    } else if (n == "skew") {
        (void)value;
    } else if (n == "shard_world") {
        if (value < 1 || value > 64) return fail(h, COREG_EINVAL, "shard_world must be in [1, 64]");
        h->opt_shard_world = value;
        if (h->opt_shard_rank >= value) h->opt_shard_rank = 0;
    } else if (n == "combo_begin") {
        if (value < 0) return fail(h, COREG_EINVAL, "combo_begin must be >= 0");
        h->opt_combo_begin = value;
    } else if (n == "combo_end") {
        if (value < 0) return fail(h, COREG_EINVAL, "combo_end must be >= 0");
        h->opt_combo_end = value;
    } else if (n == "shard_rank") {
        if (value < 0 || value >= h->opt_shard_world) return fail(h, COREG_EINVAL, "shard_rank must be in [0, shard_world)");
        h->opt_shard_rank = value;
    } else if (n == "border_fix") {
        h->opt_border_fix = value ? 1 : 0;
    } else if (n == "tap_fix") {
        h->opt_tap_fix = value ? 1 : 0;
    } else if (n == "tap_cap") {
        if (value < 1 || value > (1 << 26)) return fail(h, COREG_EINVAL, "tap_cap must be in [1, 2^26]");
        h->opt_tap_cap = value;
    } else if (n == "pitch") {
        h->opt_pitch = value;
    } else if (n == "taper_frac") {
        if (value < -1 || value > 1000) return fail(h, COREG_EINVAL, "taper_frac must be in [-1, 1000]");
        h->opt_taper_frac = value;
    } else if (n == "taper_min") {
        if (value < 16 || value > 1024) return fail(h, COREG_EINVAL, "taper_min must be in [16, 1024]");
        h->opt_taper_min = value;
    } else if (n == "taper_rounds") {
        if (value < 1) return fail(h, COREG_EINVAL, "taper_rounds must be >= 1");
        h->opt_taper_rounds = value;
    } else if (n == "crop_reference") {
        h->opt_crop_reference = value ? 1 : 0;
    } else if (n == "tile_skip") {
        h->opt_tile_skip = value ? 1 : 0;
    } else if (n == "h_series") {
        h->opt_h_series = value ? 1 : 0;
    } else if (n == "h_incr") {
        h->opt_h_incr = value ? 1 : 0;
    } else if (n == "patch_w") {
        if (value < 0 || value > kBlock) return fail(h, COREG_EINVAL, "patch_w must be in [0, 256]");
        h->opt_patch_w = value;
    } else if (n == "lds_bytes") {
        if (value < 1024 || value > 159 * 1024) return fail(h, COREG_EINVAL, "lds_bytes must be in [1 KiB, 159 KiB]");
        h->opt_lds_bytes = value;
    } else {
        return fail(h, COREG_EINVAL, "unknown option: " + n);
    }
    return COREG_OK;
}

}

#include "abi_images.hpp"
#include "abi_sweeps.hpp"
#include "abi_host.hpp"
#include "abi_context.hpp"


#include "multi.hpp"
```

### euispice_coreg_amd/csrc/host_plan.hpp

```cpp
#pragma once
namespace {
template <typename Fn>
void parallel_for(long long n, unsigned max_threads, long long grain, Fn fn) {
    if (n <= 0) return;
    const long long nt_max = std::max<long long>(1, std::min(max_threads, std::thread::hardware_concurrency()));
    if (grain <= 0) grain = (n + nt_max - 1) / nt_max;
    const long long nt = std::min(nt_max, (n + grain - 1) / grain);
    if (nt <= 1) {
        fn(0ll, n);
        return;
    }
    std::atomic<long long> next(0);
    auto worker = [&] {
        for (long long lo = next.fetch_add(grain); lo < n; lo = next.fetch_add(grain)) fn(lo, std::min(n, lo + grain));
    };
    std::vector<std::thread> th;
    for (long long t = 1; t < nt; ++t) th.emplace_back(worker);
    worker();
    for (auto& x : th) x.join();
}

struct LagDims {
    int n1, n2, n3, n4, n5;
    long long nc;
    long long c0;
    long long total() const { return (long long)n1 * n2 * nc; }
    void inner(long long c, int* i3, int* i4, int* i5) const {
        const long long g = c + c0;
        *i5 = (int)(g % n5);
        *i4 = (int)((g / n5) % n4);
        *i3 = (int)(g / ((long long)n5 * n4));
    }
};

struct ComboRange {
    long long begin = 0, end = 0;
};
ComboRange take_combo_range(coreg_handle* h) {
    ComboRange r;
    r.begin = h->opt_combo_begin;
    r.end = h->opt_combo_end;
    h->opt_combo_begin = h->opt_combo_end = 0;
    return r;
}
int check_lags(coreg_handle* h, const coreg_lags* l, LagDims* d, int64_t begin, int64_t end, ComboRange combo = ComboRange()) {
    if (!l || !l->crval1 || !l->crval2 || !l->cdelt1 || !l->cdelt2 || !l->crota)
        return fail(h, COREG_EINVAL, "lags: null array");
    if (l->n_crval1 < 1 || l->n_crval2 < 1 || l->n_cdelt1 < 1 || l->n_cdelt2 < 1 || l->n_crota < 1)
        return fail(h, COREG_EINVAL, "lags: every axis needs at least one value");
    d->n1 = l->n_crval1;
    d->n2 = l->n_crval2;
    d->n3 = l->n_cdelt1;
    d->n4 = l->n_cdelt2;
    d->n5 = l->n_crota;
    d->nc = (long long)d->n3 * d->n4 * d->n5;
    d->c0 = 0;
    {
        const long long cb = combo.begin, ce = combo.end;
        if (cb != 0 || ce != 0) {
            if (cb < 0 || ce <= cb || ce > d->nc)
                return fail(h, COREG_EINVAL, "combo_begin/combo_end outside [0, n_cdelt1 * n_cdelt2 * n_crota]");
            d->c0 = cb;
            d->nc = ce - cb;
        }
    }
    if (begin < 0 || end > d->total() || begin > end)
        return fail(h, COREG_EINVAL, "lag_begin/lag_end outside [0, n_lags]");
    const double* ax[5] = {l->crval1, l->crval2, l->cdelt1, l->cdelt2, l->crota};
    const int32_t na[5] = {l->n_crval1, l->n_crval2, l->n_cdelt1, l->n_cdelt2, l->n_crota};
    for (int k = 0; k < 5; ++k)
        for (int32_t i = 0; i < na[k]; ++i)
            if (!std::isfinite(ax[k][i])) return fail(h, COREG_EINVAL, "lags: a non-finite value");
    return COREG_OK;
}

static int check_wcs(coreg_handle* h, const coreg_wcs2d* w, bool carrington_transform) {
    const char* why = wcs_problem(*w, carrington_transform);
    return why ? fail(h, COREG_EINVAL, why) : COREG_OK;
}
static int check_grid(coreg_handle* h, const coreg_carr_grid* g) {
    if (g->n_lon >= 1 && g->n_lat >= 1 && too_many(g->n_lon, g->n_lat))
        return fail(h, COREG_EINVAL, "Carrington grid: more than 2^31 - 1 points");
    const char* why = grid_problem(*g);
    return why ? fail(h, COREG_EINVAL, why) : COREG_OK;
}

struct Geometry {
    double dx_di = 1, dx_dj = 0, dy_di = 0, dy_dj = 1;
    double ax = 0, ay = 0, bx = 0, by = 0;
};
struct Plan {
    int tile_w = 32;
    int sw = 16, sh = 16;
    double window = 0;
    double win_w = 0, win_h = 0;
};

Plan choose_plan(coreg_handle* h, const Geometry& g, int m1, int n2, long long lds_elems) {
    Plan best, fallback;
    double best_cost = std::numeric_limits<double>::max(), fb_win = std::numeric_limits<double>::max();
    const int sw_hi = h->opt_patch_w > 0 ? std::min<int>((int)h->opt_patch_w, kBlock) : kBlock;
    for (int tw = 4; tw <= 256; tw *= 2) {
        if (h->opt_tile_w > 0 && tw != h->opt_tile_w) continue;
        const int th = kTilePts / tw;
        if (th < 1) continue;
        const double tex = tw * std::fabs(g.dx_di) + th * std::fabs(g.dx_dj);
        const double tey = tw * std::fabs(g.dy_di) + th * std::fabs(g.dy_dj);
        for (int sw = 1; sw <= std::min(m1, sw_hi); ++sw) {
            int sh = std::min(n2, kBlock / sw);
            if (sh < 1) break;
            const int cols = (m1 + sw - 1) / sw, rows = (n2 + sh - 1) / sh;
            sh = (n2 + rows - 1) / rows;
            const int sw2 = (m1 + cols - 1) / cols;
            const double ex = tex + sw2 * std::fabs(g.ax) + sh * std::fabs(g.bx) + 6.0;
            const double ey = tey + sw2 * std::fabs(g.ay) + sh * std::fabs(g.by) + 6.0;
            const double win = (ex + 1.0) * ey;
            if (win < fb_win) {
                fb_win = win;
                fallback.tile_w = tw;
                fallback.sw = sw2;
                fallback.sh = sh;
                fallback.window = win;
                fallback.win_w = ex + 1.0;
                fallback.win_h = ey;
            }
            if (win > 0.94 * (double)lds_elems) continue;
            const double cost = (double)cols * rows * (1.0 + 0.08 * win / (double)lds_elems);
            if (cost < best_cost) {
                best_cost = cost;
                best.tile_w = tw;
                best.sw = sw2;
                best.sh = sh;
                best.window = win;
                best.win_w = ex + 1.0;
                best.win_h = ey;
            }
        }
    }
    const Plan& r = best_cost < std::numeric_limits<double>::max() ? best : fallback;
    if (std::getenv("COREG_DEBUG_PLAN"))
        std::fprintf(stderr, "[coreg plan] tile %d x %d, lag patch %d x %d, window estimate %.0f (%.1f x %.1f) of %lld elements; "
                     "geometry d/di (%.3f, %.3f) d/dj (%.3f, %.3f) lag1 (%.3f, %.3f) lag2 (%.3f, %.3f)\n", r.tile_w,
                     kTilePts / r.tile_w, r.sw, r.sh, r.window, r.win_w, r.win_h, lds_elems, g.dx_di, g.dy_di, g.dx_dj, g.dy_dj, g.ax, g.ay,
                     g.bx, g.by);
    return r;
}

void extreme_lags(const double* v, int n, int out[3]) {
    int lo = 0, hi = 0;
    for (int i = 1; i < n; ++i) {
        if (v[i] < v[lo] || v[lo] != v[lo]) lo = i;
        if (v[i] > v[hi] || v[hi] != v[hi]) hi = i;
    }
    const double mid = 0.5 * (v[lo] + v[hi]);
    int m = lo;
    for (int i = 0; i < n; ++i)
        if (std::fabs(v[i] - mid) < std::fabs(v[m] - mid)) m = i;
    out[0] = lo;
    out[1] = m;
    out[2] = hi;
}

double lag_step(const double* v, int n) {
    if (n < 2) return 0.0;
    double lo = v[0], hi = v[0];
    for (int i = 1; i < n; ++i) {
        lo = std::min(lo, v[i]);
        hi = std::max(hi, v[i]);
    }
    return (hi - lo) / (double)(n - 1);
}

struct SlotList {
    std::vector<int> i1, i2;
    std::vector<long long> outidx;
    int n_batches = 0;
};

void build_slots(const LagDims& d, long long c, long long begin, long long end, int sw, int sh, SlotList* s) {
    s->i1.clear();
    s->i2.clear();
    s->outidx.clear();
    s->n_batches = 0;
    {
        const size_t cap = (size_t)((d.n1 + sw - 1) / sw + 1) * ((d.n2 + sh - 1) / sh) * kBlock;
        s->i1.reserve(cap);
        s->i2.reserve(cap);
        s->outidx.reserve(cap);
    }
    const long long row = (long long)d.n2 * d.nc;
    const int i1_lo = (int)(begin / row);
    const int i1_hi = (int)((end - 1) / row);
    const int m1 = i1_hi - i1_lo + 1;
    for (int p1 = 0; p1 * sw < m1; ++p1)
        for (int p2 = 0; p2 * sh < d.n2; ++p2) {
            bool any = false;
            const size_t at = s->i1.size();
            for (int t = 0; t < kBlock; ++t) {
                int lx = t % sw, ly = t / sw;
                bool valid = ly < sh;
                if (!valid) lx = ly = 0;
                int i1 = i1_lo + p1 * sw + lx, i2 = p2 * sh + ly;
                if (i1 > i1_hi) {
                    i1 = i1_hi;
                    valid = false;
                }
                if (i2 > d.n2 - 1) {
                    i2 = d.n2 - 1;
                    valid = false;
                }
                const long long idx = ((long long)i1 * d.n2 + i2) * d.nc + c;
                if (idx < begin || idx >= end) valid = false;
                s->i1.push_back(i1);
                s->i2.push_back(i2);
                s->outidx.push_back(valid ? idx : -1);
                any |= valid;
            }
            if (!any) {
                s->i1.resize(at);
                s->i2.resize(at);
                s->outidx.resize(at);
            } else {
                s->n_batches++;
            }
        }
}

int pick_groups(coreg_handle* h, int n_batches, int n_tiles) {
    if (h->opt_shard_world > 1) {
        const long long per_rank = 8 * std::max<long long>(1, std::llround(256.0 / (8.0 * n_batches)));
        return (int)std::min<long long>(per_rank * h->opt_shard_world, 1000 / (8 * h->opt_shard_world) * 8 * h->opt_shard_world);
    }
    long long g = h->opt_n_groups > 0 ? h->opt_n_groups : (4096 + n_batches - 1) / n_batches;
    (void)n_tiles;
    g = std::max<long long>(8, std::min<long long>(h->opt_n_groups > 0 ? 1000 : 256, ((g + 7) / 8) * 8));
    return (int)g;
}

void pick_taper(const coreg_handle* h, int n_groups, int n_batches, int* tmin, int* tfrac) {
    *tmin = (int)h->opt_taper_min;
    if (h->opt_taper_frac >= 0) {
        *tfrac = (int)h->opt_taper_frac;
        return;
    }
    const double rounds = (double)n_groups * n_batches / 256.0;
    *tfrac = (rounds >= (double)h->opt_taper_rounds && n_groups >= 128 && h->opt_shard_world <= 1) ? 512 : 0;
}

template <int MODE>
int launch_precompute(coreg_handle* h, const PrecomputeArgs& a, int n_tiles, int n_groups, int n_batches) {
    EventPair* ev = next_event(h, h->ev_pre, h->ev_pre_used);
    if (!ev) return fail(h, COREG_EHIP, "hipEventCreate failed");
    int tmin, tfrac;
    pick_taper(h, n_groups, n_batches, &tmin, &tfrac);
    PrecomputeArgs b = a;
    b.prologue = h->pending_prologue;
    const bool with_prologue = b.prologue.src != nullptr;
    std::memset(&h->pending_prologue, 0, sizeof(h->pending_prologue));
    HIPCHK(hipEventRecord(ev->a, h->stream));
    if (h->ref_dtype == COREG_F32)
        hipLaunchKernelGGL((k_precompute<MODE, float>), dim3(n_tiles), dim3(256), 0, h->stream, b);
    else
        hipLaunchKernelGGL((k_precompute<MODE, double>), dim3(n_tiles), dim3(256), 0, h->stream, b);
    (void)with_prologue;
    hipLaunchKernelGGL(k_tile_list, dim3(1), dim3(1024), 0, h->stream, (const int*)a.tile_count, n_tiles, n_groups,
                       h->tile_list.as<int>(), h->tile_cum.as<int>(), h->group_first.as<int>(),
                       h->tile_info.as<long long>(), tmin, tfrac);
    ev->b_is_next_sweep = true;
    ev->next_sweep_index = h->ev_sweep_used;
    HIPCHK(hipGetLastError());
    return COREG_OK;
}

int reserve_tiles(coreg_handle* h, int n_tiles) {
    const size_t pts = (size_t)n_tiles * kTilePts + (size_t)(kPointGroups + 1) * kChunk;
    HIPCHK(h->pts.reserve(pts * sizeof(Pt)));
    HIPCHK(h->tile_count.reserve(n_tiles * sizeof(int)));
    HIPCHK(h->tile_list.reserve(n_tiles * sizeof(int)));
    HIPCHK(h->tile_cum.reserve((n_tiles + 1) * sizeof(int)));
    HIPCHK(h->group_first.reserve(2 * 1024 * sizeof(int) + 64));
    HIPCHK(h->tile_info.reserve(8 * sizeof(long long)));
    HIPCHK(h->tile_bbox.reserve((size_t)n_tiles * 4 * sizeof(double)));
    return COREG_OK;
}

int setup_precompute(coreg_handle* h, const Plan& plan, int method, PrecomputeArgs* a, int* n_tiles) {
    std::memset(a, 0, sizeof(*a));
    a->tile_w = plan.tile_w;
    a->tile_h = kTilePts / plan.tile_w;
    a->tiles_x = (h->gW + a->tile_w - 1) / a->tile_w;
    a->tiles_y = (h->gH + a->tile_h - 1) / a->tile_h;
    *n_tiles = a->tiles_x * a->tiles_y;
    RETCHK(reserve_tiles(h, *n_tiles));
    a->ref = h->ref.p;
    a->gw = h->gW;
    a->gh = h->gH;
    a->pivot_a = h->pivots.as<double>();
    a->pts = h->pts.as<Pt>();
    a->tile_count = h->tile_count.as<int>();
    a->tile_bbox = h->tile_bbox.as<double>();
    a->residus = method == COREG_METHOD_RESIDUS ? 1 : 0;
    return COREG_OK;
}

long long lds_window_elems(const coreg_handle* h);

int pick_pitch(const coreg_handle* h, const Plan& plan, long long lds_elems, int order = 2) {
    if (h->opt_pitch == 0 || !h->opt_use_lds) return 0;
    static const int kPitches[] = {89, 121, 153, 185, 217};
    if (h->opt_pitch > 0) {
        for (int p : kPitches)
            if (p == h->opt_pitch) return p;
        return 0;
    }
    for (int p : kPitches)
        if ((double)p >= plan.win_w + (order > 2 ? 4.0 : 2.0) &&
            (double)p * (plan.win_h + (order > 2 ? 2.0 : 0.0)) <= 0.985 * (double)lds_elems)
            return p;
    return 0;
}

}
```

### euispice_coreg_amd/csrc/host_state.hpp

```cpp
#pragma once
namespace {

struct DevBuf {
    void* p = nullptr;
    size_t cap = 0;
    hipError_t reserve(size_t bytes) {
        if (bytes <= cap) return hipSuccess;
        if (p) {
            hipError_t e = hipFree(p);
            if (e != hipSuccess) return e;
            p = nullptr;
            cap = 0;
        }
        const size_t want = bytes + bytes / 4 + 256;
        hipError_t e = hipMalloc(&p, want);
        if (e != hipSuccess) return e;
        cap = want;
        return hipSuccess;
    }
    void release() {
        if (p) (void)hipFree(p);
        p = nullptr;
        cap = 0;
    }
    template <typename T>
    T* as() const {
        return (T*)p;
    }
};

struct PinBuf {
    void* p = nullptr;
    size_t cap = 0;
    hipError_t reserve(size_t bytes) {
        if (bytes <= cap) return hipSuccess;
        if (p) (void)hipHostFree(p);
        p = nullptr;
        cap = 0;
        const size_t want = bytes + bytes / 2 + 4096;
        hipError_t e = hipHostMalloc(&p, want, hipHostMallocDefault);
        if (e != hipSuccess) return e;
        cap = want;
        return hipSuccess;
    }
    void release() {
        if (p) (void)hipHostFree(p);
        p = nullptr;
        cap = 0;
    }
};

enum SrcKind {
    SRC_HOST = 0,
    SRC_PINNED = 1,
    SRC_DEVICE = 2,
    SRC_TILED = 3,
};

struct PixFmt {
    int bitpix = 0;
    bool f32 = false;
    double bscale = 1.0, bzero = 0.0;
    bool raw() const { return bitpix != 0; }
    bool scaled() const { return bscale != 1.0 || bzero != 0.0; }
    size_t elem() const { return raw() ? (size_t)(bitpix < 0 ? -bitpix : bitpix) / 8 : (f32 ? 4 : 8); }
    bool swap_only() const { return bitpix == -32 && !scaled(); }
    static PixFmt native(bool is_f32) {
        PixFmt f;
        f.f32 = is_f32;
        return f;
    }
};

constexpr int kMaxDevices = 64;
std::mutex g_attr_mutex;

struct EventPair {
    hipEvent_t a = nullptr, b = nullptr;
    bool b_is_next_sweep = false;
    size_t next_sweep_index = 0;
};

}

struct KeptTapLists {
    DevBuf all;
    ~KeptTapLists() { all.release(); }
};
struct FixLaunch {
    std::vector<BorderFixArgs> border;
    std::vector<ParityFixArgs> parity;
    TapFixArgs tap = {};
    bool have_tap = false;
    int tap_segs = 0, tap_mode = 0;
    long long tap_count = 0;
    std::shared_ptr<KeptTapLists> kept;
    bool small_f32 = true;
    bool empty() const { return border.empty() && parity.empty() && !have_tap; }
};

struct ContextState;

struct coreg_handle {
    int device = 0;
    hipStream_t stream = nullptr;
    bool own_stream = false;
    std::string err;

    ContextState* ctx = nullptr;

    DevBuf small;
    int sW = 0, sH = 0;
    bool small_f32 = false;
    DevBuf ref;
    int gW = 0, gH = 0;
    int ref_dtype = -1;
    DevBuf pivots, red_sum, red_cnt;
    DevBuf t_sin_lon, t_cos_lon, t_cos_lat, t_sin_lat, t_lon_deg, t_dx;
    coreg_diffrot rot_ref = {}, rot_small = {};
    bool has_rot_ref = false, has_rot_small = false;
    CarrTables tabs;
    std::vector<double> tabs_key;
    PinBuf pin_img[2];
    hipEvent_t ev_img[2] = {nullptr, nullptr};
    int pin_img_next = 0;
    DevBuf pts, tile_count, tile_list, tile_cum, group_first, tile_info, tile_bbox;
    DevBuf rf_fix_slab;
    DevBuf counters;
    DevBuf lane_params, out_index, partials, out_dev, tmp_img;
    DevBuf up_f64, up_flag;
    DevBuf up_raw;
    DevBuf rice_blob, rice_rand, dec_img;
    PrologueArgs pending_prologue = {};
    DevBuf bbox_buf;
    hipStream_t aux_stream = nullptr;
    hipStream_t up_stream = nullptr;
    hipEvent_t ev_small = nullptr, ev_main = nullptr;
    bool small_pending = false;
    DevBuf red_sum_up, red_cnt_up;
    int64_t opt_overlap_upload = 1;
    int64_t opt_tap_nan_filter = 2;
    int64_t opt_async_upload = 0;
    std::thread up_thread;
    std::mutex up_m;
    std::condition_variable up_cv;
    std::function<hipError_t()> up_job;
    bool up_has = false, up_stop = false, up_busy = false;
    hipError_t up_rc = hipSuccess;
    PinBuf pin_small[2];
    hipEvent_t ev_pin_small[2] = {nullptr, nullptr};
    int pin_small_next = 0;
    std::map<std::vector<double>, std::vector<int>> border_cache;
    std::map<std::vector<double>, std::vector<unsigned char>> flags_cache;
    DevBuf border_flags, fix_partial;
    DevBuf border_dev;
    PinBuf pin_border;
    int64_t opt_border_fix = 1;
    int64_t opt_tap_fix = 1, opt_tap_cap = 1 << 24;
    DevBuf tap_count, tap_segq, tap_list, tap_skip, tap_seg_slot, tap_seg_begin, tap_pixel, tap_xw, tap_yw;
    long long tap_last[3] = {0, 0, 0};
    int64_t opt_shard_world = 1, opt_shard_rank = 0;
    int64_t opt_combo_begin = 0, opt_combo_end = 0;
    DevBuf sums;
    long long sums_slots = 0;
    struct PendingFinalize {
        long long slot_off, n_slots, lag_begin;
        const long long* outidx_dev;
        int residus;
        RefineArgs refine;
        std::function<int(coreg_handle*)> replay_precompute;
        FixLaunch fixes;
    };
    std::function<int(coreg_handle*)> last_precompute;
    DevBuf rf_flags, rf_pivots, rf_list, rf_head, rf_partial;
    std::vector<PendingFinalize> pending_fin;
    DevBuf fin_outidx;
    long long pending_n_out = 0;

    int64_t opt_crop_reference = 1;
    int64_t opt_taper_min = 128, opt_taper_frac = -1, opt_taper_rounds = 6;
    int64_t opt_use_lds = 1, opt_clean_path = 1, opt_refine = 1, opt_refine_cond_log10 = 5, opt_tile_w = 0, opt_n_groups = 0, opt_lds_bytes = (159 * 1024 * kPointGroups) / 4, opt_patch_w = 0, opt_h_series = 1, opt_h_incr = 1, opt_tile_skip = 1, opt_pitch = -1;

    coreg_stats stats;
    bool stats_pending = false;
    PinBuf pin_info;
    std::vector<EventPair> ev_sweep, ev_pre;
    size_t ev_sweep_used = 0, ev_pre_used = 0;
    hipEvent_t ev_t1 = nullptr;
    hipEvent_t ev_end[2] = {nullptr, nullptr};
    PinBuf pin_plan[2];
    int plan_slot = 0;
    bool plan_open = false;
};
```

### euispice_coreg_amd/csrc/kernels_sweep.hpp

```cpp
#pragma once
namespace coreg {
struct SweepArgs {
    const void* img;
    int W, H;
    const Pt* pts;
    const int* tile_count;
    const int* tile_list;
    const int* tile_cum;
    const int* group_first;
    long long* tile_info;
    const double* tile_bbox;
    const double* lane_params;
    long long n_slots;
    int n_batches;
    int n_groups;
    int group_lo;
    double* partials;
    const double* pivots;
    int use_lds;
    int clean_path;
    int lds_elems;
    LaunchU car_inv;
};

struct Acc {
    int n;
    double a, b, aa, bb, ab;
};

template <int N>
struct Taps;
template <>
struct Taps<3> {
    double t[9];
    __device__ __forceinline__ void issue(unsigned a0, unsigned a1, unsigned a2) {
        asm volatile(
            "ds_read_b64 %0, %9\n\tds_read_b64 %1, %9 offset:8\n\tds_read_b64 %2, %9 offset:16\n\t"
            "ds_read_b64 %3, %10\n\tds_read_b64 %4, %10 offset:8\n\tds_read_b64 %5, %10 offset:16\n\t"
            "ds_read_b64 %6, %11\n\tds_read_b64 %7, %11 offset:8\n\tds_read_b64 %8, %11 offset:16"
            : "=&v"(t[0]), "=&v"(t[1]), "=&v"(t[2]), "=&v"(t[3]), "=&v"(t[4]), "=&v"(t[5]), "=&v"(t[6]), "=&v"(t[7]),
              "=&v"(t[8])
            : "v"(a0), "v"(a1), "v"(a2));
    }
    __device__ __forceinline__ void wait_after(double& w0, double& w1, double& w2, double& w3, double& w4, double& w5) {
        asm volatile("s_waitcnt lgkmcnt(0)"
                     : "+v"(t[0]), "+v"(t[1]), "+v"(t[2]), "+v"(t[3]), "+v"(t[4]), "+v"(t[5]), "+v"(t[6]), "+v"(t[7]),
                       "+v"(t[8]), "+v"(w0), "+v"(w1), "+v"(w2), "+v"(w3), "+v"(w4), "+v"(w5));
    }
    __device__ __forceinline__ void issue_before(unsigned a0, unsigned a1, unsigned a2, double& fx, double& fy) {
        asm volatile(
            "ds_read_b64 %0, %11\n\tds_read_b64 %1, %11 offset:8\n\tds_read_b64 %2, %11 offset:16\n\t"
            "ds_read_b64 %3, %12\n\tds_read_b64 %4, %12 offset:8\n\tds_read_b64 %5, %12 offset:16\n\t"
            "ds_read_b64 %6, %13\n\tds_read_b64 %7, %13 offset:8\n\tds_read_b64 %8, %13 offset:16"
            : "=&v"(t[0]), "=&v"(t[1]), "=&v"(t[2]), "=&v"(t[3]), "=&v"(t[4]), "=&v"(t[5]), "=&v"(t[6]), "=&v"(t[7]),
              "=&v"(t[8]), "+v"(fx), "+v"(fy)
            : "v"(a0), "v"(a1), "v"(a2));
    }
    __device__ __forceinline__ void wait() {
        asm volatile("s_waitcnt lgkmcnt(0)"
                     : "+v"(t[0]), "+v"(t[1]), "+v"(t[2]), "+v"(t[3]), "+v"(t[4]), "+v"(t[5]), "+v"(t[6]), "+v"(t[7]),
                       "+v"(t[8]));
    }
    template <int P>
    __device__ __forceinline__ void issue_before_imm(unsigned a0, double& fx, double& fy) {
        static_assert(P > 0 && (2 * P + 2) * 8 < 65536, "LDS immediate offsets are 16 bits");
        asm volatile(
            "ds_read_b64 %0, %11\n\tds_read_b64 %1, %11 offset:8\n\tds_read_b64 %2, %11 offset:16\n\t"
            "ds_read_b64 %3, %11 offset:%12\n\tds_read_b64 %4, %11 offset:%13\n\tds_read_b64 %5, %11 offset:%14\n\t"
            "ds_read_b64 %6, %11 offset:%15\n\tds_read_b64 %7, %11 offset:%16\n\tds_read_b64 %8, %11 offset:%17"
            : "=&v"(t[0]), "=&v"(t[1]), "=&v"(t[2]), "=&v"(t[3]), "=&v"(t[4]), "=&v"(t[5]), "=&v"(t[6]), "=&v"(t[7]),
              "=&v"(t[8]), "+v"(fx), "+v"(fy)
            : "v"(a0), "n"(P * 8), "n"(P * 8 + 8), "n"(P * 8 + 16), "n"(2 * P * 8), "n"(2 * P * 8 + 8),
              "n"(2 * P * 8 + 16));
    }
};
template <>
struct Taps<2> {
    double t[4];
    __device__ __forceinline__ void issue(unsigned a0, unsigned a1, unsigned) {
        asm volatile(
            "ds_read_b64 %0, %4\n\tds_read_b64 %1, %4 offset:8\n\t"
            "ds_read_b64 %2, %5\n\tds_read_b64 %3, %5 offset:8"
            : "=&v"(t[0]), "=&v"(t[1]), "=&v"(t[2]), "=&v"(t[3])
            : "v"(a0), "v"(a1));
    }
    __device__ __forceinline__ void issue_before(unsigned a0, unsigned a1, unsigned a2, double&, double&) {
        issue(a0, a1, a2);
    }
    __device__ __forceinline__ void wait_after(double&, double&, double&, double&, double&, double&) { wait(); }
    __device__ __forceinline__ void wait() {
        asm volatile("s_waitcnt lgkmcnt(0)" : "+v"(t[0]), "+v"(t[1]), "+v"(t[2]), "+v"(t[3]));
    }
};

template <>
struct Taps<4> {
    double t[16];
    __device__ __forceinline__ void issue_before(unsigned a0, unsigned a1, unsigned a2, unsigned a3, double& fx,
                                                 double& fy) {
        asm volatile(
            "ds_read_b64 %0, %18\n\tds_read_b64 %1, %18 offset:8\n\tds_read_b64 %2, %18 offset:16\n\t"
            "ds_read_b64 %3, %18 offset:24\n\t"
            "ds_read_b64 %4, %19\n\tds_read_b64 %5, %19 offset:8\n\tds_read_b64 %6, %19 offset:16\n\t"
            "ds_read_b64 %7, %19 offset:24\n\t"
            "ds_read_b64 %8, %20\n\tds_read_b64 %9, %20 offset:8\n\tds_read_b64 %10, %20 offset:16\n\t"
            "ds_read_b64 %11, %20 offset:24\n\t"
            "ds_read_b64 %12, %21\n\tds_read_b64 %13, %21 offset:8\n\tds_read_b64 %14, %21 offset:16\n\t"
            "ds_read_b64 %15, %21 offset:24"
            : "=&v"(t[0]), "=&v"(t[1]), "=&v"(t[2]), "=&v"(t[3]), "=&v"(t[4]), "=&v"(t[5]), "=&v"(t[6]), "=&v"(t[7]),
              "=&v"(t[8]), "=&v"(t[9]), "=&v"(t[10]), "=&v"(t[11]), "=&v"(t[12]), "=&v"(t[13]), "=&v"(t[14]),
              "=&v"(t[15]), "+v"(fx), "+v"(fy)
            : "v"(a0), "v"(a1), "v"(a2), "v"(a3));
    }
    template <int P>
    __device__ __forceinline__ void issue_before_imm(unsigned a0, double& fx, double& fy) {
        static_assert(P > 0 && (3 * P + 3) * 8 < 65536, "LDS immediate offsets are 16 bits");
        asm volatile(
            "ds_read_b64 %0, %18\n\tds_read_b64 %1, %18 offset:8\n\tds_read_b64 %2, %18 offset:16\n\t"
            "ds_read_b64 %3, %18 offset:24\n\t"
            "ds_read_b64 %4, %18 offset:%19\n\tds_read_b64 %5, %18 offset:%20\n\tds_read_b64 %6, %18 offset:%21\n\t"
            "ds_read_b64 %7, %18 offset:%22\n\t"
            "ds_read_b64 %8, %18 offset:%23\n\tds_read_b64 %9, %18 offset:%24\n\tds_read_b64 %10, %18 offset:%25\n\t"
            "ds_read_b64 %11, %18 offset:%26\n\t"
            "ds_read_b64 %12, %18 offset:%27\n\tds_read_b64 %13, %18 offset:%28\n\tds_read_b64 %14, %18 offset:%29\n\t"
            "ds_read_b64 %15, %18 offset:%30"
            : "=&v"(t[0]), "=&v"(t[1]), "=&v"(t[2]), "=&v"(t[3]), "=&v"(t[4]), "=&v"(t[5]), "=&v"(t[6]), "=&v"(t[7]),
              "=&v"(t[8]), "=&v"(t[9]), "=&v"(t[10]), "=&v"(t[11]), "=&v"(t[12]), "=&v"(t[13]), "=&v"(t[14]),
              "=&v"(t[15]), "+v"(fx), "+v"(fy)
            : "v"(a0), "n"(P * 8), "n"(P * 8 + 8), "n"(P * 8 + 16), "n"(P * 8 + 24), "n"(2 * P * 8), "n"(2 * P * 8 + 8),
              "n"(2 * P * 8 + 16), "n"(2 * P * 8 + 24), "n"(3 * P * 8), "n"(3 * P * 8 + 8), "n"(3 * P * 8 + 16),
              "n"(3 * P * 8 + 24));
    }
    __device__ __forceinline__ void wait_after(double* wx, double* wy) {
        asm volatile("s_waitcnt lgkmcnt(0)"
                     : "+v"(t[0]), "+v"(t[1]), "+v"(t[2]), "+v"(t[3]), "+v"(t[4]), "+v"(t[5]), "+v"(t[6]), "+v"(t[7]),
                       "+v"(t[8]), "+v"(t[9]), "+v"(t[10]), "+v"(t[11]), "+v"(t[12]), "+v"(t[13]), "+v"(t[14]),
                       "+v"(t[15]), "+v"(wx[0]), "+v"(wx[1]), "+v"(wx[2]), "+v"(wx[3]), "+v"(wy[0]), "+v"(wy[1]),
                       "+v"(wy[2]), "+v"(wy[3]));
    }
};

template <int PITCH, bool FOLDED = false>
__device__ __forceinline__ double gather_o3(unsigned win, int pitch, double cx, double cy, double offx, double offy) {
    int c0, r0;
    double fx, fy;
    if constexpr (FOLDED) {
        c0 = (int)cx;
        r0 = (int)cy;
        fx = __builtin_amdgcn_fract(cx);
        fy = __builtin_amdgcn_fract(cy);
    } else {
        const double flx = floor(cx), fly = floor(cy);
        c0 = (int)flx + (int)offx;
        r0 = (int)fly + (int)offy;
        fx = cx - flx;
        fy = cy - fly;
    }
    const unsigned a0 = win + 8u * (unsigned)(__mul24(r0, PITCH > 0 ? PITCH : pitch) + c0);
    Taps<4> tp;
    if constexpr (PITCH > 0) {
        tp.template issue_before_imm<PITCH>(a0, fx, fy);
    } else {
        const unsigned a1 = a0 + 8u * (unsigned)pitch;
        const unsigned a2 = a1 + 8u * (unsigned)pitch;
        const unsigned a3 = a2 + 8u * (unsigned)pitch;
        tp.issue_before(a0, a1, a2, a3, fx, fy);
    }
    double wx[4], wy[4];
    spline_weights6_o3(fx, wx);
    spline_weights6_o3(fy, wy);
    tp.wait_after(wx, wy);
    double v = 0.0;
#pragma unroll
    for (int r = 0; r < 4; ++r) {
        double row = 0.0;
#pragma unroll
        for (int c = 0; c < 4; ++c) row = fma(tp.t[r * 4 + c], wx[c], row);
        v = fma(row, wy[r], v);
    }
    return v * (1.0 / 36.0);
}

template <int PITCH>
__device__ __forceinline__ double gather_o2(unsigned win, int pitch, double ux, double uy) {
    const int c0 = (int)ux, r0 = (int)uy;
    const unsigned a0 = win + 8u * (unsigned)(__mul24(r0, PITCH > 0 ? PITCH : pitch) + c0);
    Taps<3> tp;
    double fx = __builtin_amdgcn_fract(ux), fy = __builtin_amdgcn_fract(uy);
    if constexpr (PITCH > 0) {
        tp.template issue_before_imm<PITCH>(a0, fx, fy);
    } else {
        const unsigned a1 = a0 + 8u * (unsigned)pitch;
        const unsigned a2 = a1 + 8u * (unsigned)pitch;
        tp.issue_before(a0, a1, a2, fx, fy);
    }
    double wx[3], wy[3];
    const double gx = 1.0 - fx, gy = 1.0 - fy;
    wx[0] = gx * gx;
    wx[2] = fx * fx;
    wx[1] = (2.0 - wx[0]) - wx[2];
    wy[0] = gy * gy;
    wy[2] = fy * fy;
    wy[1] = (2.0 - wy[0]) - wy[2];
    tp.wait_after(wx[0], wx[1], wx[2], wy[0], wy[1], wy[2]);
    double v = 0.0;
#pragma unroll
    for (int r = 0; r < 3; ++r) {
        double row = 0.0;
#pragma unroll
        for (int c = 0; c < 3; ++c) row = fma(tp.t[r * 3 + c], wx[c], row);
        v = fma(row, wy[r], v);
    }
    return v;
}

template <int MODE, int ORDER, typename TS, bool LDS, bool ROUND, bool RESID, bool INTERIOR = false, int PITCH = 0,
          bool CLEAN = false, bool PREMAPPED = false>
__device__ __forceinline__ void point_lag(Acc& acc, unsigned win, const TS* __restrict__ img, int pitch,
                                          int ox, int oy, int W, int H, double wmax, double hmax, double px0, double py0,
                                          double pxw, double pyw, const H9& hm, const LaunchU& cu, double b0, double b1, double av,
                                          double isa, double pivot_b) {
    constexpr int N = Spline<ORDER>::N;
    if constexpr (INTERIOR && LDS) {
        double ux, uy, mx = 0.0, my = 0.0;
        if constexpr (PREMAPPED) {
            static_assert(ORDER == 2, "the cubic gather wants the unshifted coordinate");
            ux = b0;
            uy = b1;
        } else if (MODE == MODE_TRANSLATE) {
            ux = pxw + b0;
            uy = pyw + b1;
        } else {
            if (MODE == MODE_CAR) apply_car_vec(hm, cu, b0, b1, isa, mx, my);
            else apply_map<MODE>(hm, cu, b0, b1, mx, my);
            ux = mx + pxw;
            uy = my + pyw;
        }
        double v = 0.0;
        if constexpr (ORDER == 2) {
            v = gather_o2<PITCH>(win, pitch, ux, uy);
        } else if constexpr (ORDER == 3) {
            if (MODE == MODE_TRANSLATE) v = gather_o3<PITCH, true>(win, pitch, ux, uy, 0.0, 0.0);
            else v = gather_o3<PITCH>(win, pitch, mx, my, pxw, pyw);
        } else {
            const int c0 = (int)ux, r0 = (int)uy;
            const unsigned a0 = win + 8u * (unsigned)(__mul24(r0, pitch) + c0);
            const unsigned a1 = a0 + 8u * (unsigned)pitch;
            const unsigned a2 = a1 + 8u * (unsigned)pitch;
            Taps<N> tp;
            double wx[N], wy[N];
            tp.issue(a0, a1, a2);
            spline_weights_t<ORDER>(__builtin_amdgcn_fract(ux), wx);
            spline_weights_t<ORDER>(__builtin_amdgcn_fract(uy), wy);
            tp.wait();
#pragma unroll
            for (int r = 0; r < N; ++r) {
                double row = 0.0;
#pragma unroll
                for (int c = 0; c < N; ++c) row = fma(tp.t[r * N + c], wx[c], row);
                v = fma(row, wy[r], v);
            }
        }
        double bm;
        if (ROUND) {
            v = (double)(float)v;
            bm = v - pivot_b;
        } else {
            bm = v;
        }
        if constexpr (CLEAN) {
            static_assert(!RESID && MODE != MODE_CAR, "no room for the chunk sums in Pt");
            acc.b += bm;
            acc.bb = fma(bm, bm, acc.bb);
            acc.ab = fma(av, bm, acc.ab);
        } else if (RESID) {
            const double d = (av - (ROUND ? v : v + pivot_b)) * (MODE == MODE_CAR ? 1.0 / sqrt(av) : isa);
            if (isfinite(d)) {
                acc.n += 1;
                acc.b += d;
                acc.bb = fma(d, d, acc.bb);
            }
        } else if (isfinite(v)) {
            acc.n += 1;
            acc.a += av;
            acc.b += bm;
            acc.aa = fma(av, av, acc.aa);
            acc.bb = fma(bm, bm, acc.bb);
            acc.ab = fma(av, bm, acc.ab);
        }
        return;
    }
    double nx, ny;
    if (MODE == MODE_TRANSLATE) {
        nx = px0 + b0;
        ny = py0 + b1;
    } else {
        if (MODE == MODE_CAR) apply_car_vec(hm, cu, b0, b1, isa, nx, ny);
        else apply_map<MODE>(hm, cu, b0, b1, nx, ny);
    }
    if (INTERIOR || ((nx >= 0.0) & (nx <= wmax) & (ny >= 0.0) & (ny <= hmax))) {
        int sx, sy;
        double wx[N], wy[N];
        double v = 0.0;
        if constexpr (ORDER == ORDER_RT) {
            if constexpr (LDS) {
                v = spline_lds_rt(win, pitch, ox, oy, nx, ny, cu.order_rt);
            } else {
                bool inb;
                v = spline_global_rt<TS>(img, W, H, nx, ny, cu.order_rt, inb);
            }
        } else if constexpr (LDS && ORDER == 2) {
            v = gather_o2<PITCH>(win, pitch, nx + pxw, ny + pyw);
        } else if constexpr (LDS && ORDER == 3) {
            v = gather_o3<PITCH>(win, pitch, nx, ny, pxw, pyw);
        } else if constexpr (LDS) {
            const double fx = floor(nx + (ORDER == 2 ? 0.5 : 0.0)), fy = floor(ny + (ORDER == 2 ? 0.5 : 0.0));
            const int r0 = (int)fy - (ORDER == 2 ? 1 : 0) - oy;
            const int c0 = (int)fx - (ORDER == 2 ? 1 : 0) - ox;
            const unsigned a0 = win + 8u * (unsigned)(__mul24(r0, pitch) + c0);
            const unsigned a1 = a0 + 8u * (unsigned)pitch;
            const unsigned a2 = a1 + 8u * (unsigned)pitch;
            Taps<N> tp;
            tp.issue(a0, a1, a2);
            Spline<ORDER>::eval(nx, sx, wx);
            Spline<ORDER>::eval(ny, sy, wy);
            tp.wait();
#pragma unroll
            for (int r = 0; r < N; ++r) {
                double row = 0.0;
#pragma unroll
                for (int c = 0; c < N; ++c) row = fma(tp.t[r * N + c], wx[c], row);
                v = fma(row, wy[r], v);
            }
        } else {
            Spline<ORDER>::eval(nx, sx, wx);
            Spline<ORDER>::eval(ny, sy, wy);
            int ix[N], iy[N];
#pragma unroll
            for (int k = 0; k < N; ++k) {
                ix[k] = mirror_tap<ORDER>(sx + k, W);
                iy[k] = mirror_tap<ORDER>(sy + k, H) * W;
            }
#pragma unroll
            for (int r = 0; r < N; ++r) {
                double row = 0.0;
#pragma unroll
                for (int c = 0; c < N; ++c) row = fma((double)img[iy[r] + ix[c]], wx[c], row);
                v = fma(row, wy[r], v);
            }
        }
        double bm;
        if (ROUND) {
            v = (double)(float)v;
            bm = v - pivot_b;
        } else {
            bm = LDS ? v : v - pivot_b;
        }
        if (RESID) {
            const double braw = (ROUND || !LDS) ? v : v + pivot_b;
            const double d = (av - braw) * (MODE == MODE_CAR ? 1.0 / sqrt(av) : isa);
            if (isfinite(d)) {
                acc.n += 1;
                acc.b += d;
                acc.bb = fma(d, d, acc.bb);
            }
        } else if (isfinite(v)) {
            acc.n += 1;
            acc.a += av;
            acc.b += bm;
            acc.aa = fma(av, av, acc.aa);
            acc.bb = fma(bm, bm, acc.bb);
            acc.ab = fma(av, bm, acc.ab);
        }
    }
}

#ifndef COREG_PT_SCALAR
#define COREG_PT_SCALAR 2
#endif
#ifndef COREG_PT_ANCHOR
#define COREG_PT_ANCHOR 1
#endif
typedef unsigned SPt __attribute__((ext_vector_type(8)));
__device__ __forceinline__ SPt spt_load(const Pt* __restrict__ p, double& anchor) {
    SPt r;
#if defined(__HIP_DEVICE_COMPILE__)
#if COREG_PT_ANCHOR
    asm volatile("s_load_dwordx8 %0, %2, 0x0" : "=s"(r), "+v"(anchor) : "s"(p));
#else
    asm volatile("s_load_dwordx8 %0, %1, 0x0" : "=s"(r) : "s"(p));
#endif
#else
    r = (SPt)(0u);
    (void)p;
    (void)anchor;
#endif
    return r;
}
__device__ __forceinline__ void spt_wait(SPt& r) {
#if defined(__HIP_DEVICE_COMPILE__)
    asm volatile("s_waitcnt lgkmcnt(0)" : "+s"(r));
#endif
}
__device__ __forceinline__ double spt_f64(const SPt& r, int i) {
    const unsigned long long u = ((unsigned long long)r[2 * i + 1] << 32) | (unsigned long long)r[2 * i];
    return __builtin_bit_cast(double, u);
}
__device__ __forceinline__ void load_pt_uniform(const Pt* __restrict__ p, Pt& out) {
#if defined(__HIP_DEVICE_COMPILE__) && COREG_PT_SCALAR
    typedef const __attribute__((address_space(4))) double* ConstF64;
    ConstF64 q = (ConstF64)(const double*)p;
    out.b0 = q[0];
    out.b1 = q[1];
    out.a = q[2];
    out.pad = q[3];
#else
    out = *p;
#endif
}

template <int MODE, int ORDER, typename TS, bool LDS, bool ROUND, bool RESID, bool INTERIOR = false, int PITCH = 0,
          bool CLEAN = false>
__device__ __forceinline__ void tile_points(Acc& acc, unsigned win, const TS* __restrict__ img, int pitch,
                                            int ox, int oy, int W, int H, double px0, double py0, double pxw,
                                            double pyw, const H9& hm, const LaunchU& cu, const Pt* __restrict__ pts, int p_begin, int p_end,
                                            double pivot_b, int pg) {
    const double wmax = (double)(W - 1), hmax = (double)(H - 1);
    const int n_full = p_end / kChunk;
#if defined(__HIP_DEVICE_COMPILE__) && COREG_PT_SCALAR == 2
    constexpr bool kIncr = INTERIOR && LDS && ORDER == 2 && !RESID &&
                           (MODE == MODE_HOMOGRAPHY || MODE == MODE_HOMOGRAPHY_SERIES);
    if constexpr (kIncr) {
        if (cu.h_incr) {
            H9 hv = hm;
            hv.h[0] = fma(pxw, hm.h[6], hm.h[0]);
            hv.h[1] = fma(pxw, hm.h[7], hm.h[1]);
            hv.h[2] = MODE == MODE_HOMOGRAPHY_SERIES ? hm.h[2] + pxw : fma(pxw, hm.h[8], hm.h[2]);
            hv.h[3] = fma(pyw, hm.h[6], hm.h[3]);
            hv.h[4] = fma(pyw, hm.h[7], hm.h[4]);
            hv.h[5] = MODE == MODE_HOMOGRAPHY_SERIES ? hm.h[5] + pyw : fma(pyw, hm.h[8], hm.h[5]);
            int c = p_begin / kChunk + pg;
            if (c < n_full) {
                double& anchor = hv.h[7];
                SPt cur = spt_load(pts + c * kChunk, anchor);
                spt_wait(cur);
                for (; c < n_full; c += kPointGroups) {
                    const Pt* __restrict__ q = pts + c * kChunk;
                    const bool run = cur[7] != 0u;
                    double xn = 0.0, yn = 0.0, ww = 0.0;
#pragma unroll
                    for (int k = 0; k < kChunk; ++k) {
                        SPt nxt = spt_load(k + 1 < kChunk ? q + k + 1 : q + kPointGroups * kChunk, anchor);
                        const double x = spt_f64(cur, 0), y = spt_f64(cur, 1);
                        if (k == 0 || !run) {
                            xn = fma(hv.h[0], x, fma(hv.h[1], y, hv.h[2]));
                            yn = fma(hv.h[3], x, fma(hv.h[4], y, hv.h[5]));
                            ww = MODE == MODE_HOMOGRAPHY_SERIES ? fma(hv.h[6], x, hv.h[7] * y)
                                                                : fma(hv.h[6], x, fma(hv.h[7], y, hv.h[8]));
                        } else {
                            xn += hv.h[0];
                            yn += hv.h[3];
                            ww += hv.h[6];
                        }
                        double ux, uy;
                        if (MODE == MODE_HOMOGRAPHY_SERIES) {
                            const double qq = fma(ww, ww, -ww);
                            ux = fma(xn, qq, xn);
                            uy = fma(yn, qq, yn);
                        } else {
                            double r = __builtin_amdgcn_rcp(ww);
                            r = fma(r, fma(-ww, r, 1.0), r);
                            ux = xn * r;
                            uy = yn * r;
                        }
                        point_lag<MODE, ORDER, TS, LDS, ROUND, RESID, INTERIOR, PITCH, CLEAN, true>(
                            acc, win, img, pitch, ox, oy, W, H, wmax, hmax, px0, py0, pxw, pyw, hv, cu, ux, uy,
                            spt_f64(cur, 2), spt_f64(cur, 3), pivot_b);
                        if constexpr (CLEAN) {
                            if (k == 1) acc.a += spt_f64(cur, 3);
                            if (k == 2) acc.aa += spt_f64(cur, 3);
                            if (k == kChunk - 1) acc.n += kChunk;
                        }
                        spt_wait(nxt);
                        cur = nxt;
                    }
                }
            }
            if (pg == n_full % kPointGroups) {
                for (int p = n_full * kChunk; p < p_end; ++p) {
                    Pt pt;
                    load_pt_uniform(pts + p, pt);
                    point_lag<MODE, ORDER, TS, LDS, ROUND, RESID, INTERIOR, PITCH>(acc, win, img, pitch, ox, oy, W, H, wmax,
                                                                                   hmax, px0, py0, pxw, pyw, hm, cu, pt.b0,
                                                                                   pt.b1, pt.a, pt.pad, pivot_b);
                }
            }
            return;
        }
    }
    {
        int c = p_begin / kChunk + pg;
        if (c < n_full) {
            H9 hml = hm;
            double& anchor = MODE == MODE_TRANSLATE ? (INTERIOR && LDS ? pxw : px0) : hml.h[MODE == MODE_CAR ? 0 : 7];
            SPt cur = spt_load(pts + c * kChunk, anchor);
            spt_wait(cur);
            for (; c < n_full; c += kPointGroups) {
                const Pt* __restrict__ q = pts + c * kChunk;
#pragma unroll
                for (int k = 0; k < kChunk; ++k) {
                    SPt nxt = spt_load(k + 1 < kChunk ? q + k + 1 : q + kPointGroups * kChunk, anchor);
                    point_lag<MODE, ORDER, TS, LDS, ROUND, RESID, INTERIOR, PITCH, CLEAN>(
                        acc, win, img, pitch, ox, oy, W, H, wmax, hmax, px0, py0, pxw, pyw, hml, cu, spt_f64(cur, 0),
                        spt_f64(cur, 1), spt_f64(cur, 2), spt_f64(cur, 3), pivot_b);
                    if constexpr (CLEAN) {
                        if (k == 1) acc.a += spt_f64(cur, 3);
                        if (k == 2) acc.aa += spt_f64(cur, 3);
                        if (k == kChunk - 1) acc.n += kChunk;
                    }
                    spt_wait(nxt);
                    cur = nxt;
                }
            }
        }
    }
#else
    for (int c = p_begin / kChunk + pg; c < n_full; c += kPointGroups) {
        const Pt* __restrict__ q = pts + c * kChunk;
        Pt pt[kChunk];
#pragma unroll
        for (int k = 0; k < kChunk; ++k) load_pt_uniform(q + k, pt[k]);
#pragma unroll
        for (int k = 0; k < kChunk; ++k)
            point_lag<MODE, ORDER, TS, LDS, ROUND, RESID, INTERIOR, PITCH, CLEAN>(acc, win, img, pitch, ox, oy, W, H, wmax,
                                                                                  hmax, px0, py0, pxw, pyw, hm, cu, pt[k].b0,
                                                                                  pt[k].b1, pt[k].a, pt[k].pad, pivot_b);
        if constexpr (CLEAN) {
            acc.n += kChunk;
            acc.a += pt[1].pad;
            acc.aa += pt[2].pad;
        }
    }
#endif
    if (pg == n_full % kPointGroups) {
        for (int p = n_full * kChunk; p < p_end; ++p) {
            Pt pt;
            load_pt_uniform(pts + p, pt);
            point_lag<MODE, ORDER, TS, LDS, ROUND, RESID, INTERIOR, PITCH>(acc, win, img, pitch, ox, oy, W, H, wmax, hmax,
                                                                           px0, py0, pxw, pyw, hm, cu, pt.b0, pt.b1, pt.a,
                                                                           pt.pad, pivot_b);
        }
    }
}

template <int MODE, int ORDER, typename TS, bool ROUND, bool RESID, int PITCH = 0>
__global__ void __launch_bounds__(kSweepThreads) k_sweep(const SweepArgs a) {
    extern __shared__ __align__(16) unsigned char lds_raw[];
    double* lds = (double*)lds_raw;
    constexpr int kWaves = kSweepThreads / 64;
    constexpr int kLagWaves = kBlock / 64;
    __shared__ double wred2[2][kLagWaves][4];
    __shared__ int wdirty[2][kWaves];
    constexpr bool kCleanPath = MODE != MODE_CAR && !RESID && ORDER != ORDER_RT && !(ROUND && sizeof(TS) == 8);
    int visit = 0;
    int n_vis = 0, n_vis_lds = 0, n_vis_int = 0, n_vis_clean = 0;

    const int b = blockIdx.x;
    const int slot8 = b & 7;
    const int q = b >> 3;
    const int batch = q % a.n_batches;
    const int group = a.group_lo + (q / a.n_batches) * 8 + slot8;

    const int lane = threadIdx.x & 63, wave = threadIdx.x >> 6;
    const int pg = __builtin_amdgcn_readfirstlane(threadIdx.x / kBlock);
    const long long slot = (long long)batch * kBlock + (threadIdx.x % kBlock);

    double px0 = 0.0, py0 = 0.0;
    H9 hm;
#pragma unroll
    for (int k = 0; k < 9; ++k) hm.h[k] = 0.0;
    if (MODE == MODE_TRANSLATE) {
        px0 = a.lane_params[slot];
        py0 = a.lane_params[a.n_slots + slot];
    } else {
#pragma unroll
        for (int k = 0; k < 9; ++k) hm.h[k] = a.lane_params[(long long)k * a.n_slots + slot];
    }

    const bool pad_lane = MODE == MODE_TRANSLATE ? (px0 != px0) : (hm.h[8] != hm.h[8]);

    Acc acc = {0, 0.0, 0.0, 0.0, 0.0, 0.0};

    const TS* __restrict__ img = (const TS*)a.img;
    const int W = a.W, H = a.H;
    const double inf = __builtin_inf();
    const int u_lo = a.group_first[1024 + group];
    const int u_hi = a.group_first[1024 + group + 1];
    const int n_list = (int)a.tile_info[0];
    const double pivot_b = a.pivots[1];
#if defined(__HIP_DEVICE_COMPILE__)
    const unsigned win = (unsigned)(uintptr_t)(__attribute__((address_space(3))) unsigned char*)lds_raw;
#else
    const unsigned win = 0;
#endif

    for (int tl = a.group_first[group]; tl < n_list && u_lo < u_hi; ++tl) {
        const int ubase = a.tile_cum[tl];
        if (ubase >= u_hi) break;
        const int tile = a.tile_list[tl];
        const int cnt = a.tile_count[tile];
        const int p_begin = max(u_lo - ubase, 0) * kUnitPts;
        const int p_end = min((u_hi - ubase) * kUnitPts, cnt);
        if (p_begin >= p_end) continue;
        const double* bb = a.tile_bbox + (size_t)tile * 4;
        const double bx0 = bb[0], bx1 = bb[1], by0 = bb[2], by1 = bb[3];

        double mnx, mxx, mny, mxy;
        if (MODE == MODE_TRANSLATE) {
            mnx = bx0 + px0;
            mxx = bx1 + px0;
            mny = by0 + py0;
            mxy = by1 + py0;
        } else {
            mnx = inf; mxx = -inf; mny = inf; mxy = -inf;
#pragma unroll
            for (int c = 0; c < 4; ++c) {
                double cx, cy;
                apply_map<MODE>(hm, a.car_inv, (c & 1) ? bx1 : bx0, (c & 2) ? by1 : by0, cx, cy);
                mnx = fmin(mnx, cx);
                mxx = fmax(mxx, cx);
                mny = fmin(mny, cy);
                mxy = fmax(mxy, cy);
            }
            if (MODE == MODE_CAR) {
                const double margin = car_tile_margin(a.car_inv.box_c, fmax(fabs(by0), fabs(by1)) + a.car_inv.pole_sep);
                mnx -= margin;
                mxx += margin;
                mny -= margin;
                mxy += margin;
            }
        }
        for (int o = 32; o > 0; o >>= 1) {
            mnx = fmin(mnx, __shfl_xor(mnx, o));
            mxx = fmax(mxx, __shfl_xor(mxx, o));
            mny = fmin(mny, __shfl_xor(mny, o));
            mxy = fmax(mxy, __shfl_xor(mxy, o));
        }
        double(*wred)[4] = wred2[visit & 1];
        int* wdirt = wdirty[visit & 1];
        ++visit;
        if (lane == 0 && wave < kLagWaves) {
            wred[wave][0] = mnx;
            wred[wave][1] = mxx;
            wred[wave][2] = mny;
            wred[wave][3] = mxy;
        }
        __syncthreads();
        mnx = fmin(fmin(wred[0][0], wred[1][0]), fmin(wred[2][0], wred[3][0]));
        mxx = fmax(fmax(wred[0][1], wred[1][1]), fmax(wred[2][1], wred[3][1]));
        mny = fmin(fmin(wred[0][2], wred[1][2]), fmin(wred[2][2], wred[3][2]));
        mxy = fmax(fmax(wred[0][3], wred[1][3]), fmax(wred[2][3], wred[3][3]));
        if (!(mxx >= 0.0) || !(mnx <= (double)(W - 1)) || !(mxy >= 0.0) || !(mny <= (double)(H - 1))) continue;
        constexpr double kClear = 1e-9;
        const bool interior = (mnx >= kClear) & (mxx <= (double)(W - 1) - kClear) & (mny >= kClear) &
                              (mxy <= (double)(H - 1) - kClear);
        constexpr bool kWide = ORDER == ORDER_RT || ORDER > 2;
        const int ord = ORDER == ORDER_RT ? a.car_inv.order_rt : ORDER;
        const int ap_lo = kWide ? ord / 2 + 1 : 1;
        const int ap_hi = kWide ? ord - ord / 2 + 1 : 2;
        const int ox = max((int)floor(fmax(mnx, 0.0)) - ap_lo, kWide ? -ap_lo : -1);
        const int oy = max((int)floor(fmax(mny, 0.0)) - ap_lo, kWide ? -ap_lo : -1);
        const int ex = min((int)floor(fmin(mxx, (double)(W - 1))) + ap_hi, kWide ? W - 1 + ap_hi : W);
        const int ey = min((int)floor(fmin(mxy, (double)(H - 1))) + ap_hi, kWide ? H - 1 + ap_hi : H);
        const int ww = ex - ox + 1, wh = ey - oy + 1;
        int pitch = PITCH > 0 ? PITCH : (ww | 1);
        if (PITCH == 0) {
            const int r = pitch & 31;
            const int up = r < 5 ? 5 - r : ((r > 11 && r < 21) ? 21 - r : (r > 27 ? 37 - r : 0));
            if ((long long)(pitch + up) * wh <= (long long)a.lds_elems) pitch += up;
        }
        const long long need = (long long)pitch * wh;
        const bool in_lds = a.use_lds && (need <= (long long)a.lds_elems) && (PITCH == 0 || ww <= PITCH);

        const Pt* __restrict__ pts = a.pts + (size_t)tile * kTilePts;

        bool swept = false;
        ++n_vis;
        {
          if (in_lds) {
            swept = true;
            ++n_vis_lds;
#ifndef COREG_STAGE_ROWS
#define COREG_STAGE_ROWS 8
#endif
#ifndef COREG_STAGE_COLS
#define COREG_STAGE_COLS 1
#endif
            constexpr int kStage = COREG_STAGE_ROWS, kCols = COREG_STAGE_COLS;
            const double scale = ORDER == 2 ? 0.25 : 1.0;
            const int wave_u = __builtin_amdgcn_readfirstlane(wave);
            double poison = 0.0;
            for (int r0 = wave_u; r0 < wh; r0 += kWaves * kStage) {
                for (int c0 = 0; c0 < ww; c0 += 64 * kCols) {
                    int gx[kCols];
#pragma unroll
                    for (int j = 0; j < kCols; ++j) {
                        const int c = c0 + 64 * j + lane;
                        gx[j] = kWide ? mirror_far(ox + min(c, ww - 1), W) : mirror_idx(ox + min(c, ww - 1), W);
                    }
                    TS v[kStage][kCols];
#pragma unroll
                    for (int k = 0; k < kStage; ++k) {
                        const int r = min(r0 + k * kWaves, wh - 1);
                        const int gy = kWide ? mirror_far(oy + r, H) : mirror_idx(oy + r, H);
                        const TS* __restrict__ row = img + (size_t)gy * W;
#pragma unroll
                        for (int j = 0; j < kCols; ++j) v[k][j] = row[gx[j]];
                    }
#pragma unroll
                    for (int j = 0; j < kCols; ++j) {
                        const int c = c0 + 64 * j + lane;
                        if (c < ww) {
#pragma unroll
                            for (int k = 0; k < kStage; ++k) {
                                const int r = r0 + k * kWaves;
                                if (r < wh) {
                                    const double e = (ROUND ? (double)v[k][j] : (double)v[k][j] - pivot_b) * scale;
                                    lds[r * pitch + c] = e;
                                    if (kCleanPath) poison = fma(e, 0.0, poison);
                                }
                            }
                        }
                    }
                }
            }
            if (kCleanPath && interior) {
                const int dirty = __ballot(poison != poison) != 0ull;
                if (lane == 0) wdirt[wave] = dirty;
            }
            __syncthreads();
            bool done = false;
            if constexpr (ORDER != ORDER_RT) {
                if (interior) {
                    done = true;
                    bool clean = false;
                    if constexpr (kCleanPath) clean = a.clean_path && __ballot(wdirt[lane % kWaves] != 0) == 0ull;
                    ++n_vis_int;
                    n_vis_clean += clean ? 1 : 0;
                    if (!pad_lane) {
                        const double offx = (ORDER == 2 ? 0.5 : 0.0) - (double)(ORDER / 2 + ox);
                        const double offy = (ORDER == 2 ? 0.5 : 0.0) - (double)(ORDER / 2 + oy);
                        const double pxw = MODE == MODE_TRANSLATE ? px0 + offx : offx;
                        const double pyw = MODE == MODE_TRANSLATE ? py0 + offy : offy;
                        if (kCleanPath && clean) {
                            tile_points<MODE, ORDER, TS, true, ROUND, RESID, true, PITCH, kCleanPath>(
                                acc, win, img, pitch, ox, oy, W, H, px0, py0, pxw, pyw, hm, a.car_inv, pts, p_begin, p_end,
                                pivot_b, pg);
                        } else {
                            tile_points<MODE, ORDER, TS, true, ROUND, RESID, true, PITCH>(acc, win, img, pitch, ox, oy, W, H,
                                                                                          px0, py0, pxw, pyw, hm, a.car_inv,
                                                                                          pts, p_begin, p_end, pivot_b, pg);
                        }
                    }
                }
            }
            if (!done) {
                const double offx = ORDER == 2 ? 0.5 - (double)(1 + ox) : (ORDER == 3 ? -(double)(1 + ox) : 0.0);
                const double offy = ORDER == 2 ? 0.5 - (double)(1 + oy) : (ORDER == 3 ? -(double)(1 + oy) : 0.0);
                tile_points<MODE, ORDER, TS, true, ROUND, RESID, false, PITCH>(acc, win, img, pitch, ox, oy, W, H, px0, py0,
                                                                               offx, offy, hm, a.car_inv, pts, p_begin,
                                                                               p_end, pivot_b, pg);
            }
          }
        }
        if (!swept) {
            tile_points<MODE, ORDER, TS, false, ROUND, RESID>(acc, win, img, 0, 0, 0, W, H, px0, py0, 0.0, 0.0, hm, a.car_inv, pts,
                                                              p_begin, p_end, pivot_b, pg);
        }
    }

    if (threadIdx.x == 0) {
        atomicAdd((unsigned long long*)a.tile_info + 3, (unsigned long long)n_vis);
        atomicAdd((unsigned long long*)a.tile_info + 4, (unsigned long long)n_vis_lds);
        atomicAdd((unsigned long long*)a.tile_info + 5, (unsigned long long)n_vis_int);
        atomicAdd((unsigned long long*)a.tile_info + 6, (unsigned long long)n_vis_clean);
    }
    __syncthreads();
    const int ls = threadIdx.x % kBlock;
    if (pg > 0) {
        double* st = lds + ((size_t)(pg - 1) * kNumSums) * kBlock + ls;
        st[0] = (double)acc.n;
        st[kBlock] = acc.a;
        st[2 * kBlock] = acc.b;
        st[3 * kBlock] = acc.aa;
        st[4 * kBlock] = acc.bb;
        st[5 * kBlock] = acc.ab;
    }
    __syncthreads();
    if (pg == 0) {
        double sn = (double)acc.n, sa = acc.a, sb = acc.b, saa = acc.aa, sbb = acc.bb, sab = acc.ab;
        for (int g = 0; g < kPointGroups - 1; ++g) {
            const double* st = lds + ((size_t)g * kNumSums) * kBlock + ls;
            sn += st[0];
            sa += st[kBlock];
            sb += st[2 * kBlock];
            saa += st[3 * kBlock];
            sbb += st[4 * kBlock];
            sab += st[5 * kBlock];
        }
        double* out = a.partials + (size_t)(group - a.group_lo) * kNumSums * a.n_slots + slot;
        out[0] = sn;
        out[a.n_slots] = sa;
        out[2 * a.n_slots] = sb;
        out[3 * a.n_slots] = saa;
        out[4 * a.n_slots] = sbb;
        out[5 * a.n_slots] = sab;
    }
}

}
```

### include/coreg_hip.h

```cpp
#ifndef COREG_HIP_H
#define COREG_HIP_H

#include <stdint.h>

#ifdef __cplusplus
extern "C" {
#endif

#define COREG_OK 0
#define COREG_EINVAL (-1)
#define COREG_EHIP (-2)
#define COREG_ESTATE (-3)
#define COREG_ENOTIMPL (-4)
#define COREG_ENOMEM (-5)

#define COREG_F32 0
#define COREG_F64 1
#define COREG_I32 2

#define COREG_PROJ_TAN 0
#define COREG_PROJ_CAR 1

#define COREG_METHOD_CORRELATION 0
#define COREG_METHOD_RESIDUS 1

#define COREG_CDELT_INTENDED 0
#define COREG_CDELT_REFERENCE 1

typedef struct coreg_handle coreg_handle;

typedef struct coreg_wcs2d {
    int32_t naxis1, naxis2;
    double crpix1, crpix2;
    double crval1, crval2;
    double cdelt1, cdelt2;
    double pc1_1, pc1_2, pc2_1, pc2_2;
    double crota;
    double unit_to_deg;
    double lonpole;
    double dsun_obs;
    double crln_obs;
    double crlt_obs;
    double latpole;
    int32_t proj;
    int32_t reserved;
} coreg_wcs2d;

typedef struct coreg_lags {
    const double* crval1; int32_t n_crval1;
    const double* crval2; int32_t n_crval2;
    const double* cdelt1; int32_t n_cdelt1;
    const double* cdelt2; int32_t n_cdelt2;
    const double* crota;  int32_t n_crota;
} coreg_lags;

typedef struct coreg_carr_grid {
    double lon0, lon1; int32_t n_lon;
    double lat0, lat1; int32_t n_lat;
    const float* lat_cos;
    const float* lat_sin;
} coreg_carr_grid;

typedef struct coreg_diffrot {
    double delta_t_days;
    double c0, c1, c2;
} coreg_diffrot;

typedef struct coreg_stats {
    double sweep_kernel_ms;
    double precompute_ms;
    double total_gpu_ms;
    int64_t n_lags;
    int64_t n_grid_points;
    int64_t n_active_points;
    int64_t n_sweep_launches;
    int32_t small_is_f32;
    int32_t used_lds;
} coreg_stats;

const char* coreg_version(void);

int coreg_create(coreg_handle** h, int device);
void coreg_destroy(coreg_handle* h);
const char* coreg_last_error(const coreg_handle* h);

int coreg_set_stream(coreg_handle* h, void* hip_stream);
int coreg_synchronize(coreg_handle* h);

int coreg_set_small(coreg_handle* h, const double* img, int32_t ny, int32_t nx);

int coreg_set_small_f32(coreg_handle* h, const float* img, int32_t ny, int32_t nx);

typedef struct coreg_fits_pixels {
    const void* data;
    int32_t bitpix;
    int32_t reserved;
    double bscale, bzero;
} coreg_fits_pixels;
int coreg_set_small_fits(coreg_handle* h, const coreg_fits_pixels* px, int32_t ny, int32_t nx);
int coreg_prepare_reference_carrington_fits(coreg_handle* h, const coreg_fits_pixels* px, int32_t ny, int32_t nx,
                                            const coreg_wcs2d* hdr_large, const coreg_carr_grid* grid, double solar_r,
                                            int order);
int coreg_prepare_reference_helioprojective_fits(coreg_handle* h, const coreg_fits_pixels* px, int32_t ny, int32_t nx,
                                                 const coreg_wcs2d* hdr_large, const coreg_wcs2d* hdr_small, int order);

typedef struct coreg_fits_tiled {
    const void* heap;
    int64_t heap_bytes;
    const int64_t* tile_offset;
    const int32_t* tile_nbytes;
    int32_t n_tiles;
    int32_t zbitpix;
    int32_t naxis1, naxis2, ztile1, ztile2;
    int32_t blocksize, bytepix;
    int32_t quantize;
    int32_t dither0;
    int32_t has_blank, blank;
    const double* zscale;
    const double* zzero;
    double zscale0, zzero0;
    double bscale, bzero;
} coreg_fits_tiled;
int coreg_set_small_tiled(coreg_handle* h, const coreg_fits_tiled* t);
int coreg_prepare_reference_carrington_tiled(coreg_handle* h, const coreg_fits_tiled* t, const coreg_wcs2d* hdr_large,
                                             const coreg_carr_grid* grid, double solar_r, int order);
int coreg_prepare_reference_helioprojective_tiled(coreg_handle* h, const coreg_fits_tiled* t, const coreg_wcs2d* hdr_large,
                                                  const coreg_wcs2d* hdr_small, int order);
int coreg_decode_tiled_host(const coreg_fits_tiled* t, void* out, int dtype, int32_t* tile_status);
int coreg_encode_tiled_host(const void* pixels, int dtype, int ny, int nx, int tile_x, int tile_y, int bytepix,
                            int blocksize, int quantize, int dither0, double scale, unsigned char* heap,
                            long long heap_cap, int32_t* tile_nbytes, int64_t* tile_offset, double* zscale, double* zzero,
                            long long* heap_used);

int coreg_threshold_small(coreg_handle* h, int has_min, double vmin, int has_max, double vmax, long long* n_finite);

int coreg_set_reference_on_grid(coreg_handle* h, const void* ref, int dtype, int32_t gy, int32_t gx);

int coreg_prepare_reference_carrington(coreg_handle* h, const double* large, int32_t ny, int32_t nx,
                                       const coreg_wcs2d* hdr_large, const coreg_carr_grid* grid, double solar_r,
                                       int order);
int coreg_prepare_reference_helioprojective(coreg_handle* h, const double* large, int32_t ny, int32_t nx,
                                            const coreg_wcs2d* hdr_large, const coreg_wcs2d* hdr_small, int order);
int coreg_prepare_reference_carrington_f32(coreg_handle* h, const float* large, int32_t ny, int32_t nx,
                                           const coreg_wcs2d* hdr_large, const coreg_carr_grid* grid, double solar_r,
                                           int order);
int coreg_prepare_reference_helioprojective_f32(coreg_handle* h, const float* large, int32_t ny, int32_t nx,
                                                const coreg_wcs2d* hdr_large, const coreg_wcs2d* hdr_small, int order);

int coreg_set_small_from_device(coreg_handle* h, const void* dev_img, int dtype, int32_t ny, int32_t nx);
int coreg_prepare_reference_carrington_from_device(coreg_handle* h, const void* dev_large, int dtype, int32_t ny,
                                                   int32_t nx, const coreg_wcs2d* hdr_large,
                                                   const coreg_carr_grid* grid, double solar_r, int order);
int coreg_prepare_reference_helioprojective_from_device(coreg_handle* h, const void* dev_large, int dtype, int32_t ny,
                                                        int32_t nx, const coreg_wcs2d* hdr_large,
                                                        const coreg_wcs2d* hdr_small, int order);

int coreg_get_reference_on_grid(coreg_handle* h, void* out, int dtype);

int coreg_resample_carrington(coreg_handle* h, const coreg_wcs2d* hdr, const coreg_carr_grid* grid, double solar_r,
                              int order, double* out);
int coreg_resample_helioprojective(coreg_handle* h, const coreg_wcs2d* hdr_target, const coreg_wcs2d* hdr,
                                   int order, float* out);
int coreg_resample_helioprojective_f64(coreg_handle* h, const coreg_wcs2d* hdr_target, const coreg_wcs2d* hdr,
                                       int order, double* out);

int coreg_set_reference_rotation(coreg_handle* h, const coreg_diffrot* rot);
int coreg_set_small_rotation(coreg_handle* h, const coreg_diffrot* rot);

int coreg_sweep_carrington(coreg_handle* h, const coreg_wcs2d* hdr_small, const coreg_carr_grid* grid,
                           double solar_r, const coreg_lags* lags, int order, int method, int cdelt_semantics,
                           int64_t lag_begin, int64_t lag_end, double* corr_out, int out_on_device);
int coreg_sweep_helioprojective(coreg_handle* h, const coreg_wcs2d* hdr_target, const coreg_wcs2d* hdr_small,
                                const coreg_lags* lags, int order, int method, int cdelt_semantics,
                                int64_t lag_begin, int64_t lag_end, double* corr_out, int out_on_device);

int coreg_sums_size(coreg_handle* h, int64_t* n_doubles);
int coreg_copy_sums(coreg_handle* h, double* dst, int dst_on_device);
int coreg_finalize_sums(coreg_handle* h, const double* sums, int sums_on_device, double* corr_out, int out_on_device);

int coreg_get_pivots(coreg_handle* h, double* pivots2);
int coreg_set_pivots(coreg_handle* h, const double* pivots2);

int coreg_last_stats(coreg_handle* h, coreg_stats* out);

int coreg_last_visit_counts(coreg_handle* h, int64_t* counts6);
int coreg_last_tap_fix(coreg_handle* h, int64_t* counts3);

int coreg_set_option(coreg_handle* h, const char* name, int64_t value);

int coreg_shift_header(const coreg_wcs2d* ref, double d_crval1, double d_crval2, double d_cdelt1, double d_cdelt2,
                       double d_crota, int cdelt_semantics, coreg_wcs2d* out);
int coreg_homography(const coreg_wcs2d* from, const coreg_wcs2d* to, double* h9);
int coreg_lag_homography(const coreg_wcs2d* hdr_target, const coreg_wcs2d* hdr_small, const coreg_lags* lags,
                         const int32_t idx[5], int cdelt_semantics, double* h9);
int coreg_wcslib_pixel_to_pixel(const coreg_wcs2d* from, const coreg_wcs2d* to, int64_t n, const double* px,
                                const double* py, double* ox, double* oy, double* lng, double* lat);
int coreg_carrington_origin(const coreg_wcs2d* hdr, double* x0, double* y0);
int coreg_diffrot_table(const coreg_carr_grid* grid, const coreg_diffrot* rot, double* dx);
int coreg_car_map(const coreg_wcs2d* from, const coreg_wcs2d* to, int64_t n, const double* px, const double* py,
                  double* ox, double* oy);
int coreg_car_tile_margin(const coreg_wcs2d* hdr_target, const coreg_wcs2d* hdr_shifted, int32_t tile_w,
                          double tile_abs_lat_rad, double* margin_px);


int coreg_nansum_planes_be(const void* cube, int32_t bitpix, int64_t n_pixels, const int64_t* plane_index, int32_t n_sel,
                           double* out);

int coreg_fit_gaussian2d(int32_t m, const double* x, const double* y, const double* z, const double* p0,
                         const double* lb, const double* ub, int32_t jac, double ftol, double xtol, double gtol,
                         int32_t max_nfev, double* popt, int32_t* nfev, int32_t* status);


int coreg_set_context_frames(coreg_handle* h, int32_t n_frames, int32_t ny, int32_t nx, int dtype,
                             const coreg_wcs2d* hdrs, const void* const* pixels);
int coreg_context_frame_from_small(coreg_handle* h, int32_t k);
int coreg_sweep_context(coreg_handle* h, const coreg_wcs2d* hdr_target, const coreg_wcs2d* hdr_small,
                        const int32_t* col_frame, const coreg_lags* lags, int order, int method, int cdelt_semantics,
                        int has_min, double vmin, int has_max, double vmax, int64_t lag_begin, int64_t lag_end,
                        double* corr_out, int out_on_device);
int coreg_context_lag_headers(const coreg_wcs2d* hdr_target, const coreg_wcs2d* hdr_small, double d_crval1,
                              double d_crval2, double d_cdelt1, double d_cdelt2, double d_crota, int cdelt_semantics,
                              coreg_wcs2d* ctx, coreg_wcs2d* grid, coreg_wcs2d* shifted);

typedef struct coreg_multi coreg_multi;
int coreg_device_count(void);
int coreg_physical_device_count(void);
int coreg_multi_create(coreg_multi** m, int n_devices, const int* device_ids);
void coreg_multi_destroy(coreg_multi* m);
int coreg_multi_size(const coreg_multi* m);
coreg_handle* coreg_multi_handle(coreg_multi* m, int k);
const char* coreg_multi_last_error(const coreg_multi* m);
const char* coreg_multi_collective(const coreg_multi* m);
const char* coreg_multi_rccl_status(const coreg_multi* m);
int coreg_multi_last_mode(const coreg_multi* m);
int coreg_multi_set_option(coreg_multi* m, const char* name, int64_t value);
int coreg_multi_set_small(coreg_multi* m, const void* img, int dtype, int32_t ny, int32_t nx);
int coreg_multi_set_small_fits(coreg_multi* m, const coreg_fits_pixels* px, int32_t ny, int32_t nx);
int coreg_multi_prepare_reference_carrington_fits(coreg_multi* m, const coreg_fits_pixels* px, int32_t ny, int32_t nx,
                                                  const coreg_wcs2d* hdr_large, const coreg_carr_grid* grid,
                                                  double solar_r, int order);
int coreg_multi_prepare_reference_helioprojective_fits(coreg_multi* m, const coreg_fits_pixels* px, int32_t ny,
                                                       int32_t nx, const coreg_wcs2d* hdr_large,
                                                       const coreg_wcs2d* hdr_small, int order);
int coreg_multi_set_small_tiled(coreg_multi* m, const coreg_fits_tiled* t);
int coreg_multi_prepare_reference_carrington_tiled(coreg_multi* m, const coreg_fits_tiled* t, const coreg_wcs2d* hdr_large,
                                                   const coreg_carr_grid* grid, double solar_r, int order);
int coreg_multi_prepare_reference_helioprojective_tiled(coreg_multi* m, const coreg_fits_tiled* t,
                                                        const coreg_wcs2d* hdr_large, const coreg_wcs2d* hdr_small,
                                                        int order);
int coreg_multi_threshold_small(coreg_multi* m, int has_min, double vmin, int has_max, double vmax, long long* n_finite);
int coreg_multi_set_reference_on_grid(coreg_multi* m, const void* ref, int dtype, int32_t gy, int32_t gx);
int coreg_multi_prepare_reference_carrington(coreg_multi* m, const void* large, int dtype, int32_t ny, int32_t nx,
                                             const coreg_wcs2d* hdr_large, const coreg_carr_grid* grid, double solar_r,
                                             int order);
int coreg_multi_prepare_reference_helioprojective(coreg_multi* m, const void* large, int dtype, int32_t ny, int32_t nx,
                                                  const coreg_wcs2d* hdr_large, const coreg_wcs2d* hdr_small, int order);
int coreg_multi_set_reference_rotation(coreg_multi* m, const coreg_diffrot* rot);
int coreg_multi_set_small_rotation(coreg_multi* m, const coreg_diffrot* rot);
int coreg_multi_sweep_carrington(coreg_multi* m, const coreg_wcs2d* hdr_small, const coreg_carr_grid* grid, double solar_r,
                                 const coreg_lags* lags, int order, int method, int cdelt_semantics, double* corr_out);
int coreg_multi_sweep_helioprojective(coreg_multi* m, const coreg_wcs2d* hdr_target, const coreg_wcs2d* hdr_small,
                                      const coreg_lags* lags, int order, int method, int cdelt_semantics, double* corr_out);
int coreg_multi_last_stats(coreg_multi* m, int k, coreg_stats* out);
int coreg_multi_plan(int32_t n_crval1, int32_t n_crval2, int64_t n_inner, int32_t world, int32_t per_combo_launch,
                     int32_t* mode, int32_t* g_combo, int32_t* g1, int32_t* g2);

#ifdef __cplusplus
}
#endif
#endif
```

Baseline: 1.160 million lag-points/s.

## Pack lags into strips and skip dead lag-waves in the sweep kernel

Adds a packed strip layout for lag slots, where each 256-slot batch fills a narrow column strip row by row. The planner now costs candidates by live 64-lane lag-waves plus batches, not by patch count. The kernel remaps threads so each wave belongs to one lag-wave, and a wave whose lanes are all padding skips the per-point interpolation work. The aim is to cut the padded lanes that square patches leave on a 60x60 lag grid. In exchange the sample window per batch may grow, and the planner and kernel indexing get more complex.

```diff
diff --git a/euispice_coreg_amd/_lib.py b/euispice_coreg_amd/_lib.py
--- a/euispice_coreg_amd/_lib.py
+++ b/euispice_coreg_amd/_lib.py
@@ -231,6 +231,12 @@
     ("coreg_last_stats", C.c_int, [_P, C.POINTER(Stats)]),
     ("coreg_last_visit_counts", C.c_int, [_P, C.POINTER(C.c_int64)]),
     ("coreg_last_tap_fix", C.c_int, [_P, C.POINTER(C.c_int64)]),
+    ("coreg_last_plan", C.c_int, [_P, C.POINTER(C.c_int64)]),
+    ("coreg_lag_slots", C.c_int,
+     [C.c_int32, C.c_int32, C.c_int64, C.c_int64, C.c_int64, C.c_int64, C.c_int32, C.c_int32, C.c_int32, C.c_int64, _P, _P,
+      _P, C.POINTER(C.c_int64)]),
+    ("coreg_plan_lags", C.c_int,
+     [C.POINTER(C.c_double), C.c_int32, C.c_int32, C.c_int64, C.c_int32, C.c_int32, C.POINTER(C.c_int64)]),
     ("coreg_set_option", C.c_int, [_P, C.c_char_p, C.c_int64]),
     ("coreg_shift_header", C.c_int,
      [_WP, C.c_double, C.c_double, C.c_double, C.c_double, C.c_double, C.c_int, _WP]),
@@ -667,6 +673,11 @@
                 "flagged_not_refined": c[5]}
 
 
+    def last_plan(self) -> dict:
+        c = (C.c_int64 * 6)()
+        self._chk(self._lib.coreg_last_plan(self._h, c))
+        return {"batches": c[0], "lag_waves": c[1], "sw": c[2], "sh": c[3], "packed": bool(c[4]), "tile_w": c[5]}
+
     def last_tap_fix(self) -> dict:
         c = (C.c_int64 * 3)()
         self._chk(self._lib.coreg_last_tap_fix(self._h, c))
@@ -924,6 +935,34 @@
     return m.value
 
 
+def lag_slots(n1, n2, nc=1, c=0, begin=0, end=None, sw=16, sh=0, packed=True):
+    lib = load_library()
+    end = int(n1) * int(n2) * int(nc) if end is None else int(end)
+    args = (int(n1), int(n2), int(nc), int(c), int(begin), end, int(sw), int(sh), 1 if packed else 0)
+    counts = (C.c_int64 * 3)()
+    rc = lib.coreg_lag_slots(*args, 0, None, None, None, counts)
+    if rc != COREG_OK:
+        raise CoregError(rc, "coreg_lag_slots: bad arguments")
+    n = int(counts[0])
+    i1, i2, outidx = np.empty(n, np.int32), np.empty(n, np.int32), np.empty(n, np.int64)
+    if n:
+        rc = lib.coreg_lag_slots(*args, n, i1.ctypes.data, i2.ctypes.data, outidx.ctypes.data, counts)
+        if rc != COREG_OK:
+            raise CoregError(rc, "coreg_lag_slots: bad arguments")
+    return {"i1": i1, "i2": i2, "outidx": outidx, "batches": int(counts[1]), "lag_waves": int(counts[2])}
+
+
+def plan_lags(geometry8, m1, n2, lds_elems=159 * 1024 // 8, order=2, lag_packing=True):
+    lib = load_library()
+    g = (C.c_double * 8)(*[float(v) for v in geometry8])
+    p = (C.c_int64 * 8)()
+    rc = lib.coreg_plan_lags(g, int(m1), int(n2), int(lds_elems), int(order), 1 if lag_packing else 0, p)
+    if rc != COREG_OK:
+        raise CoregError(rc, "coreg_plan_lags: bad arguments")
+    return {"batches": p[0], "lag_waves": p[1], "sw": p[2], "sh": p[3], "packed": bool(p[4]), "tile_w": p[5],
+            "pitch": p[6], "window": p[7]}
+
+
 def context_lag_headers(hdr_target, hdr_small, d_crval1, d_crval2, d_cdelt1, d_cdelt2, d_crota,
                         cdelt_semantics=CDELT_INTENDED):
     lib = load_library()
diff --git a/euispice_coreg_amd/csrc/abi_host.hpp b/euispice_coreg_amd/csrc/abi_host.hpp
--- a/euispice_coreg_amd/csrc/abi_host.hpp
+++ b/euispice_coreg_amd/csrc/abi_host.hpp
@@ -28,6 +28,69 @@
     if (h->counters.p) HIPCHK(hipMemcpy(refined, h->counters.p, sizeof(refined), hipMemcpyDeviceToHost));
     counts5[4] = refined[0];
     counts6[5] = refined[1];
+    return COREG_OK;
+}
+
+int coreg_last_plan(coreg_handle* h, int64_t* plan6) {
+    if (!h || !plan6) return COREG_EINVAL;
+    for (int k = 0; k < 6; ++k) plan6[k] = h->plan_last[k];
+    return COREG_OK;
+}
+
+int coreg_lag_slots(int32_t n1, int32_t n2, int64_t nc, int64_t c, int64_t begin, int64_t end, int32_t sw, int32_t sh,
+                    int32_t packed, int64_t cap, int32_t* i1, int32_t* i2, int64_t* outidx, int64_t* counts3) {
+    if (!counts3 || n1 < 1 || n2 < 1 || nc < 1 || c < 0 || c >= nc || sw < 1 || sw > kBlock || sh < 0) return COREG_EINVAL;
+    if (begin < 0 || begin >= end || end > (int64_t)n1 * n2 * nc) return COREG_EINVAL;
+    if (!packed && (sh < 1 || (int64_t)sw * sh > kBlock)) return COREG_EINVAL;
+    LagDims d;
+    d.n1 = n1;
+    d.n2 = n2;
+    d.n3 = d.n4 = 1;
+    d.n5 = (int)nc;
+    d.nc = nc;
+    d.c0 = 0;
+    Plan plan;
+    plan.sw = sw;
+    plan.sh = packed && sh == 0 ? std::min(n2, strip_rows(sw, kBlock)) : sh;
+    plan.packed = packed ? 1 : 0;
+    SlotList s;
+    build_slots(d, c, begin, end, plan, &s);
+    const int64_t n = (int64_t)s.outidx.size();
+    counts3[0] = n;
+    counts3[1] = s.n_batches;
+    counts3[2] = s.n_lag_waves;
+    if (n > cap || !i1 || !i2 || !outidx) return COREG_OK;
+    for (int64_t k = 0; k < n; ++k) {
+        i1[k] = s.i1[(size_t)k];
+        i2[k] = s.i2[(size_t)k];
+        outidx[k] = s.outidx[(size_t)k];
+    }
+    return COREG_OK;
+}
+
+int coreg_plan_lags(const double* geometry8, int32_t m1, int32_t n2, int64_t lds_elems, int32_t order, int32_t lag_packing,
+                    int64_t* plan8) {
+    if (!geometry8 || !plan8 || m1 < 1 || n2 < 1 || lds_elems < 1) return COREG_EINVAL;
+    Geometry g;
+    g.dx_di = geometry8[0];
+    g.dy_di = geometry8[1];
+    g.dx_dj = geometry8[2];
+    g.dy_dj = geometry8[3];
+    g.ax = geometry8[4];
+    g.ay = geometry8[5];
+    g.bx = geometry8[6];
+    g.by = geometry8[7];
+    PlanKnobs k;
+    k.lag_packing = lag_packing ? 1 : 0;
+    const Plan r = choose_plan_for(k, g, m1, n2, lds_elems, order);
+    plan8[0] = r.batches;
+    plan8[1] = r.lag_waves;
+    plan8[2] = r.sw;
+    plan8[3] = r.sh;
+    plan8[4] = r.packed;
+    plan8[5] = r.tile_w;
+    plan8[6] = r.pitch;
+    plan8[7] = (int64_t)std::ceil(r.window);
     return COREG_OK;
 }
 
diff --git a/euispice_coreg_amd/csrc/abi_sweeps.hpp b/euispice_coreg_amd/csrc/abi_sweeps.hpp
--- a/euispice_coreg_amd/csrc/abi_sweeps.hpp
+++ b/euispice_coreg_amd/csrc/abi_sweeps.hpp
@@ -72,7 +72,8 @@
 }
 
 Plan plan_sweep(coreg_handle* h, const Geometry& geo, const SweepCall& call) {
-    return choose_plan(h, geo, call.i1_hi() - call.i1_lo() + 1, call.d.n2, h->opt_use_lds ? lds_window_elems(h) : (1LL << 40));
+    return choose_plan(h, geo, call.i1_hi() - call.i1_lo() + 1, call.d.n2, h->opt_use_lds ? lds_window_elems(h) : (1LL << 40),
+                       call.order);
 }
 
 bool combo_slots(const SweepCall& call, const coreg_wcs2d& small, const Plan& plan, long long c, coreg_wcs2d* hc,
@@ -83,7 +84,7 @@
     call.d.inner(c, &i3, &i4, &i5);
     if (shift_header(small, 0.0, 0.0, call.lags->cdelt1[i3], call.lags->cdelt2[i4], call.lags->crota[i5], call.sem, hc))
         return false;
-    build_slots(call.d, c, call.lag_begin, call.lag_end, plan.sw, plan.sh, slots);
+    build_slots(call.d, c, call.lag_begin, call.lag_end, plan, slots);
     return slots->n_batches > 0;
 }
 
@@ -186,6 +187,8 @@
         Launch L;
         L.slot_off = outidx.size();
         L.n_batches = slots.n_batches;
+        h->plan_last[0] += slots.n_batches;
+        h->plan_last[1] += slots.n_lag_waves;
         L.cc = carr_common(hc, solar_r);
         const size_t pbase = params.size();
         params.resize(pbase + 2 * ns);
@@ -319,6 +322,8 @@
         Launch L;
         L.slot_off = outidx.size();
         L.n_batches = slots.n_batches;
+        h->plan_last[0] += slots.n_batches;
+        h->plan_last[1] += slots.n_lag_waves;
         std::memset(&L.inv, 0, sizeof(L.inv));
         set_affine(&L.inv, car_native_to_pix(hc));
         L.inv.box_c = car_box_c(*hdr_target, hc, plan.tile_w);
@@ -358,6 +363,8 @@
         std::memset(&L.inv, 0, sizeof(L.inv));
         L.slot_off = outidx.size();
         L.n_batches = 1;
+        h->plan_last[0] += 1;
+        h->plan_last[1] += 1;
         L.identity = true;
         const size_t ns = kBlock, pbase = params.size();
         params.resize(pbase + 9 * ns, nanv);
@@ -569,7 +576,9 @@
         fy1 = std::max(fy1, cp.box[3]);
         outidx.insert(outidx.end(), slots.outidx.begin(), slots.outidx.end());
         n_batches += slots.n_batches;
-    }
+        h->plan_last[1] += slots.n_lag_waves;
+    }
+    h->plan_last[0] = n_batches;
     if (n_batches == 0) return close_empty_sweep(h, call);
     trace("sweep_helioprojective: combinations planned");
     const size_t ns = outidx.size();
diff --git a/euispice_coreg_amd/csrc/coreg_hip.hip b/euispice_coreg_amd/csrc/coreg_hip.hip
--- a/euispice_coreg_amd/csrc/coreg_hip.hip
+++ b/euispice_coreg_amd/csrc/coreg_hip.hip
@@ -221,6 +221,11 @@
     } else if (n == "patch_w") {
         if (value < 0 || value > kBlock) return fail(h, COREG_EINVAL, "patch_w must be in [0, 256]");
         h->opt_patch_w = value;
+    } else if (n == "lag_packing") {
+        h->opt_lag_packing = value ? 1 : 0;
+    } else if (n == "strip_w") {
+        if (value < 0 || value > kBlock) return fail(h, COREG_EINVAL, "strip_w must be in [0, 256]");
+        h->opt_strip_w = value;
     } else if (n == "lds_bytes") {
         if (value < 1024 || value > 159 * 1024) return fail(h, COREG_EINVAL, "lds_bytes must be in [1 KiB, 159 KiB]");
         h->opt_lds_bytes = value;
diff --git a/euispice_coreg_amd/csrc/host_plan.hpp b/euispice_coreg_amd/csrc/host_plan.hpp
--- a/euispice_coreg_amd/csrc/host_plan.hpp
+++ b/euispice_coreg_amd/csrc/host_plan.hpp
@@ -92,16 +92,65 @@
 struct Plan {
     int tile_w = 32;
     int sw = 16, sh = 16;
+    int packed = 0;
+    int batches = 0, lag_waves = 0;
+    int pitch = 0;
     double window = 0;
     double win_w = 0, win_h = 0;
 };
 
-Plan choose_plan(coreg_handle* h, const Geometry& g, int m1, int n2, long long lds_elems) {
+inline int strip_rows(int w, int len) { return len % w == 0 ? len / w : (len + w - 1) / w + 1; }
+inline int strip_run(int w, int rows, int n2) {
+    return std::min(n2, strip_rows(w, kBlock)) <= rows ? kBlock : w * std::max(1, std::min(rows, kBlock / w));
+}
+
+struct PlanKnobs {
+    int tile_w = 0, patch_w = 0, pitch = -1, use_lds = 1, lag_packing = 1;
+    int strip_w = 0;
+};
+int pick_pitch_for(int opt_pitch, int use_lds, double win_w, double win_h, long long lds_elems, int order);
+
+Plan choose_plan_for(const PlanKnobs& k, const Geometry& g, int m1, int n2, long long lds_elems, int order) {
     Plan best, fallback;
     double best_cost = std::numeric_limits<double>::max(), fb_win = std::numeric_limits<double>::max();
-    const int sw_hi = h->opt_patch_w > 0 ? std::min<int>((int)h->opt_patch_w, kBlock) : kBlock;
+    const int sw_hi = k.patch_w > 0 ? std::min<int>(k.patch_w, kBlock) : kBlock;
+    const bool want_pitch = k.lag_packing && k.pitch != 0 && k.use_lds && (order == 2 || order == 3);
+    const int forced_sw = k.lag_packing && k.strip_w > 0 ? std::min(k.strip_w, m1) : 0;
+    auto consider = [&](int tw, double tex, double tey, int sw, int sh, int packed, double ew, double eh, int batches,
+                        int lag_waves) {
+        const double ex = tex + ew * std::fabs(g.ax) + eh * std::fabs(g.bx) + 6.0;
+        const double ey = tey + ew * std::fabs(g.ay) + eh * std::fabs(g.by) + 6.0;
+        const double win = (ex + 1.0) * ey;
+        Plan p;
+        p.tile_w = tw;
+        p.sw = sw;
+        p.sh = sh;
+        p.packed = packed;
+        p.batches = batches;
+        p.lag_waves = lag_waves;
+        p.window = win;
+        p.win_w = ex + 1.0;
+        p.win_h = ey;
+        p.pitch = pick_pitch_for(k.pitch, k.use_lds, p.win_w, p.win_h, lds_elems, order);
+        if (!packed && win < fb_win) {
+            fb_win = win;
+            fallback = p;
+        }
+        if (win > 0.94 * (double)lds_elems || (forced_sw && !(packed && sw == forced_sw))) return;
+        double cost;
+        if (!k.lag_packing) {
+            cost = (double)batches * (1.0 + 0.08 * win / (double)lds_elems);
+        } else {
+            cost = ((double)lag_waves + 0.15 * batches) * (1.0 + 0.02 * win / (double)lds_elems);
+            if (want_pitch && p.pitch == 0) cost *= 1.06;
+        }
+        if (cost < best_cost) {
+            best_cost = cost;
+            best = p;
+        }
+    };
     for (int tw = 4; tw <= 256; tw *= 2) {
-        if (h->opt_tile_w > 0 && tw != h->opt_tile_w) continue;
+        if (k.tile_w > 0 && tw != k.tile_w) continue;
         const int th = kTilePts / tw;
         if (th < 1) continue;
         const double tex = tw * std::fabs(g.dx_di) + th * std::fabs(g.dx_dj);
@@ -112,37 +161,49 @@
             const int cols = (m1 + sw - 1) / sw, rows = (n2 + sh - 1) / sh;
             sh = (n2 + rows - 1) / rows;
             const int sw2 = (m1 + cols - 1) / cols;
-            const double ex = tex + sw2 * std::fabs(g.ax) + sh * std::fabs(g.bx) + 6.0;
-            const double ey = tey + sw2 * std::fabs(g.ay) + sh * std::fabs(g.by) + 6.0;
-            const double win = (ex + 1.0) * ey;
-            if (win < fb_win) {
-                fb_win = win;
-                fallback.tile_w = tw;
-                fallback.sw = sw2;
-                fallback.sh = sh;
-                fallback.window = win;
-                fallback.win_w = ex + 1.0;
-                fallback.win_h = ey;
+            {
+                auto waves = [&](int pw, int ph) { return ((ph - 1) * sw2 + pw - 1) / 64 + 1; };
+                const int pw_l = m1 - (cols - 1) * sw2, ph_l = n2 - (rows - 1) * sh;
+                const int lw = (cols - 1) * (rows - 1) * waves(sw2, sh) + (rows - 1) * waves(pw_l, sh) +
+                               (cols - 1) * waves(sw2, ph_l) + waves(pw_l, ph_l);
+                consider(tw, tex, tey, sw2, sh, 0, sw2, sh, cols * rows, lw);
             }
-            if (win > 0.94 * (double)lds_elems) continue;
-            const double cost = (double)cols * rows * (1.0 + 0.08 * win / (double)lds_elems);
-            if (cost < best_cost) {
-                best_cost = cost;
-                best.tile_w = tw;
-                best.sw = sw2;
-                best.sh = sh;
-                best.window = win;
-                best.win_w = ex + 1.0;
-                best.win_h = ey;
+            if (!k.lag_packing) continue;
+            const int rmax = std::min(n2, strip_rows(sw, kBlock));
+            double ew = sw, eh = rmax;
+            int batches = 0, lw = 0;
+            for (int x0 = 0; x0 < m1; x0 += sw) {
+                const int w = std::min(sw, m1 - x0), len = strip_run(w, rmax, n2), lags = w * n2;
+                const int nb = (lags + len - 1) / len;
+                batches += nb;
+                lw += (nb - 1) * ((len + 63) / 64) + (lags - (nb - 1) * len + 63) / 64;
             }
-        }
-    }
-    const Plan& r = best_cost < std::numeric_limits<double>::max() ? best : fallback;
+            consider(tw, tex, tey, sw, rmax, 1, ew, eh, batches, lw);
+        }
+    }
+    return best_cost < std::numeric_limits<double>::max() ? best : fallback;
+}
+
+Plan choose_plan(coreg_handle* h, const Geometry& g, int m1, int n2, long long lds_elems, int order) {
+    PlanKnobs k;
+    k.tile_w = (int)h->opt_tile_w;
+    k.patch_w = (int)h->opt_patch_w;
+    k.pitch = (int)h->opt_pitch;
+    k.use_lds = h->opt_use_lds ? 1 : 0;
+    k.lag_packing = h->opt_lag_packing ? 1 : 0;
+    k.strip_w = (int)h->opt_strip_w;
+    const Plan r = choose_plan_for(k, g, m1, n2, lds_elems, order);
+    h->plan_last[0] = h->plan_last[1] = 0;
+    h->plan_last[2] = r.sw;
+    h->plan_last[3] = r.sh;
+    h->plan_last[4] = r.packed;
+    h->plan_last[5] = r.tile_w;
     if (std::getenv("COREG_DEBUG_PLAN"))
-        std::fprintf(stderr, "[coreg plan] tile %d x %d, lag patch %d x %d, window estimate %.0f (%.1f x %.1f) of %lld elements; "
+        std::fprintf(stderr, "[coreg plan] tile %d x %d, lag %s %d x %d, %d batches, %d lag-waves per %d x %d plane, window "
+                     "estimate %.0f (%.1f x %.1f) of %lld elements, pitch %d; "
                      "geometry d/di (%.3f, %.3f) d/dj (%.3f, %.3f) lag1 (%.3f, %.3f) lag2 (%.3f, %.3f)\n", r.tile_w,
-                     kTilePts / r.tile_w, r.sw, r.sh, r.window, r.win_w, r.win_h, lds_elems, g.dx_di, g.dy_di, g.dx_dj, g.dy_dj, g.ax, g.ay,
-                     g.bx, g.by);
+                     kTilePts / r.tile_w, r.packed ? "strips" : "patch", r.sw, r.sh, r.batches, r.lag_waves, m1, n2, r.window,
+                     r.win_w, r.win_h, lds_elems, r.pitch, g.dx_di, g.dy_di, g.dx_dj, g.dy_dj, g.ax, g.ay, g.bx, g.by);
     return r;
 }
 
@@ -175,13 +236,31 @@
     std::vector<int> i1, i2;
     std::vector<long long> outidx;
     int n_batches = 0;
+    int n_lag_waves = 0;
+    void close_batch() {
+        const size_t at = i1.size() - kBlock;
+        int waves = 0;
+        for (int w = 0; w < kBlock / 64; ++w) {
+            bool any = false;
+            for (int t = 0; t < 64; ++t) any |= outidx[at + 64 * w + t] >= 0;
+            waves += any ? 1 : 0;
+        }
+        if (!waves) {
+            i1.resize(at);
+            i2.resize(at);
+            outidx.resize(at);
+        } else {
+            n_batches++;
+            n_lag_waves += waves;
+        }
+    }
 };
 
 void build_slots(const LagDims& d, long long c, long long begin, long long end, int sw, int sh, SlotList* s) {
     s->i1.clear();
     s->i2.clear();
     s->outidx.clear();
-    s->n_batches = 0;
+    s->n_batches = s->n_lag_waves = 0;
     {
         const size_t cap = (size_t)((d.n1 + sw - 1) / sw + 1) * ((d.n2 + sh - 1) / sh) * kBlock;
         s->i1.reserve(cap);
@@ -194,8 +273,6 @@
     const int m1 = i1_hi - i1_lo + 1;
     for (int p1 = 0; p1 * sw < m1; ++p1)
         for (int p2 = 0; p2 * sh < d.n2; ++p2) {
-            bool any = false;
-            const size_t at = s->i1.size();
             for (int t = 0; t < kBlock; ++t) {
                 int lx = t % sw, ly = t / sw;
                 bool valid = ly < sh;
@@ -214,16 +291,40 @@
                 s->i1.push_back(i1);
                 s->i2.push_back(i2);
                 s->outidx.push_back(valid ? idx : -1);
-                any |= valid;
             }
-            if (!any) {
-                s->i1.resize(at);
-                s->i2.resize(at);
-                s->outidx.resize(at);
-            } else {
-                s->n_batches++;
+            s->close_batch();
+        }
+}
+
+void build_slots_packed(const LagDims& d, long long c, long long begin, long long end, int sw, int rows, SlotList* s) {
+    s->i1.clear();
+    s->i2.clear();
+    s->outidx.clear();
+    s->n_batches = s->n_lag_waves = 0;
+    const long long row = (long long)d.n2 * d.nc;
+    const int i1_lo = (int)(begin / row);
+    const int i1_hi = (int)((end - 1) / row);
+    for (int x0 = i1_lo; x0 <= i1_hi; x0 += sw) {
+        const int w = std::min(sw, i1_hi + 1 - x0), len = strip_run(w, rows, d.n2);
+        const long long lags = (long long)w * d.n2;
+        for (long long e0 = 0; e0 < lags; e0 += len) {
+            for (int t = 0; t < kBlock; ++t) {
+                const bool in_run = t < len && e0 + t < lags;
+                const long long e = in_run ? e0 + t : e0;
+                const int i1 = x0 + (int)(e % w), i2 = (int)(e / w);
+                const long long idx = ((long long)i1 * d.n2 + i2) * d.nc + c;
+                s->i1.push_back(i1);
+                s->i2.push_back(i2);
+                s->outidx.push_back(in_run && idx >= begin && idx < end ? idx : -1);
             }
-        }
+            s->close_batch();
+        }
+    }
+}
+
+void build_slots(const LagDims& d, long long c, long long begin, long long end, const Plan& plan, SlotList* s) {
+    if (plan.packed) build_slots_packed(d, c, begin, end, plan.sw, plan.sh, s);
+    else build_slots(d, c, begin, end, plan.sw, plan.sh, s);
 }
 
 int pick_groups(coreg_handle* h, int n_batches, int n_tiles) {
@@ -305,19 +406,22 @@
 
 long long lds_window_elems(const coreg_handle* h);
 
-int pick_pitch(const coreg_handle* h, const Plan& plan, long long lds_elems, int order = 2) {
-    if (h->opt_pitch == 0 || !h->opt_use_lds) return 0;
+int pick_pitch_for(int opt_pitch, int use_lds, double win_w, double win_h, long long lds_elems, int order) {
+    if (opt_pitch == 0 || !use_lds) return 0;
     static const int kPitches[] = {89, 121, 153, 185, 217};
-    if (h->opt_pitch > 0) {
+    if (opt_pitch > 0) {
         for (int p : kPitches)
-            if (p == h->opt_pitch) return p;
+            if (p == opt_pitch) return p;
         return 0;
     }
     for (int p : kPitches)
-        if ((double)p >= plan.win_w + (order > 2 ? 4.0 : 2.0) &&
-            (double)p * (plan.win_h + (order > 2 ? 2.0 : 0.0)) <= 0.985 * (double)lds_elems)
+        if ((double)p >= win_w + (order > 2 ? 4.0 : 2.0) &&
+            (double)p * (win_h + (order > 2 ? 2.0 : 0.0)) <= 0.985 * (double)lds_elems)
             return p;
     return 0;
 }
-
-}
+int pick_pitch(const coreg_handle* h, const Plan& plan, long long lds_elems, int order = 2) {
+    return pick_pitch_for((int)h->opt_pitch, h->opt_use_lds ? 1 : 0, plan.win_w, plan.win_h, lds_elems, order);
+}
+
+}
diff --git a/euispice_coreg_amd/csrc/host_state.hpp b/euispice_coreg_amd/csrc/host_state.hpp
--- a/euispice_coreg_amd/csrc/host_state.hpp
+++ b/euispice_coreg_amd/csrc/host_state.hpp
@@ -158,6 +158,7 @@
     int64_t opt_border_fix = 1;
     int64_t opt_tap_fix = 1, opt_tap_cap = 1 << 24;
     DevBuf tap_count, tap_segq, tap_list, tap_skip, tap_seg_slot, tap_seg_begin, tap_pixel, tap_xw, tap_yw;
+    long long plan_last[6] = {0, 0, 0, 0, 0, 0};
     long long tap_last[3] = {0, 0, 0};
     int64_t opt_shard_world = 1, opt_shard_rank = 0;
     int64_t opt_combo_begin = 0, opt_combo_end = 0;
@@ -179,7 +180,7 @@
 
     int64_t opt_crop_reference = 1;
     int64_t opt_taper_min = 128, opt_taper_frac = -1, opt_taper_rounds = 6;
-    int64_t opt_use_lds = 1, opt_clean_path = 1, opt_refine = 1, opt_refine_cond_log10 = 5, opt_tile_w = 0, opt_n_groups = 0, opt_lds_bytes = (159 * 1024 * kPointGroups) / 4, opt_patch_w = 0, opt_h_series = 1, opt_h_incr = 1, opt_tile_skip = 1, opt_pitch = -1;
+    int64_t opt_use_lds = 1, opt_clean_path = 1, opt_refine = 1, opt_refine_cond_log10 = 5, opt_tile_w = 0, opt_n_groups = 0, opt_lds_bytes = (159 * 1024 * kPointGroups) / 4, opt_patch_w = 0, opt_h_series = 1, opt_h_incr = 1, opt_tile_skip = 1, opt_pitch = -1, opt_lag_packing = 1, opt_strip_w = 0;
 
     coreg_stats stats;
     bool stats_pending = false;
diff --git a/euispice_coreg_amd/csrc/kernels_sweep.hpp b/euispice_coreg_amd/csrc/kernels_sweep.hpp
--- a/euispice_coreg_amd/csrc/kernels_sweep.hpp
+++ b/euispice_coreg_amd/csrc/kernels_sweep.hpp
@@ -559,6 +559,7 @@
     double* lds = (double*)lds_raw;
     constexpr int kWaves = kSweepThreads / 64;
     constexpr int kLagWaves = kBlock / 64;
+    static_assert(kLagWaves == 4, "the box reduction below reads four lag-waves");
     __shared__ double wred2[2][kLagWaves][4];
     __shared__ int wdirty[2][kWaves];
     constexpr bool kCleanPath = MODE != MODE_CAR && !RESID && ORDER != ORDER_RT && !(ROUND && sizeof(TS) == 8);
@@ -572,8 +573,10 @@
     const int group = a.group_lo + (q / a.n_batches) * 8 + slot8;
 
     const int lane = threadIdx.x & 63, wave = threadIdx.x >> 6;
-    const int pg = __builtin_amdgcn_readfirstlane(threadIdx.x / kBlock);
-    const long long slot = (long long)batch * kBlock + (threadIdx.x % kBlock);
+    const int pg = __builtin_amdgcn_readfirstlane(wave % kPointGroups);
+    const int lagwave = __builtin_amdgcn_readfirstlane(wave / kPointGroups);
+    const int ls = lagwave * 64 + lane;
+    const long long slot = (long long)batch * kBlock + ls;
 
     double px0 = 0.0, py0 = 0.0;
     H9 hm;
@@ -588,6 +591,7 @@
     }
 
     const bool pad_lane = MODE == MODE_TRANSLATE ? (px0 != px0) : (hm.h[8] != hm.h[8]);
+    const bool live_wave = __ballot(!pad_lane) != 0ull;
 
     Acc acc = {0, 0.0, 0.0, 0.0, 0.0, 0.0};
 
@@ -649,11 +653,11 @@
         double(*wred)[4] = wred2[visit & 1];
         int* wdirt = wdirty[visit & 1];
         ++visit;
-        if (lane == 0 && wave < kLagWaves) {
-            wred[wave][0] = mnx;
-            wred[wave][1] = mxx;
-            wred[wave][2] = mny;
-            wred[wave][3] = mxy;
+        if (lane == 0 && pg == 0) {
+            wred[lagwave][0] = mnx;
+            wred[lagwave][1] = mxx;
+            wred[lagwave][2] = mny;
+            wred[lagwave][3] = mxy;
         }
         __syncthreads();
         mnx = fmin(fmin(wred[0][0], wred[1][0]), fmin(wred[2][0], wred[3][0]));
@@ -764,7 +768,7 @@
                     }
                 }
             }
-            if (!done) {
+            if (!done && live_wave) {
                 const double offx = ORDER == 2 ? 0.5 - (double)(1 + ox) : (ORDER == 3 ? -(double)(1 + ox) : 0.0);
                 const double offy = ORDER == 2 ? 0.5 - (double)(1 + oy) : (ORDER == 3 ? -(double)(1 + oy) : 0.0);
                 tile_points<MODE, ORDER, TS, true, ROUND, RESID, false, PITCH>(acc, win, img, pitch, ox, oy, W, H, px0, py0,
@@ -773,7 +777,7 @@
             }
           }
         }
-        if (!swept) {
+        if (!swept && live_wave) {
             tile_points<MODE, ORDER, TS, false, ROUND, RESID>(acc, win, img, 0, 0, 0, W, H, px0, py0, 0.0, 0.0, hm, a.car_inv, pts,
                                                               p_begin, p_end, pivot_b, pg);
         }
@@ -786,7 +790,6 @@
         atomicAdd((unsigned long long*)a.tile_info + 6, (unsigned long long)n_vis_clean);
     }
     __syncthreads();
-    const int ls = threadIdx.x % kBlock;
     if (pg > 0) {
         double* st = lds + ((size_t)(pg - 1) * kNumSums) * kBlock + ls;
         st[0] = (double)acc.n;
diff --git a/include/coreg_hip.h b/include/coreg_hip.h
--- a/include/coreg_hip.h
+++ b/include/coreg_hip.h
@@ -185,6 +185,7 @@
 
 int coreg_last_visit_counts(coreg_handle* h, int64_t* counts6);
 int coreg_last_tap_fix(coreg_handle* h, int64_t* counts3);
+int coreg_last_plan(coreg_handle* h, int64_t* plan6);
 
 int coreg_set_option(coreg_handle* h, const char* name, int64_t value);
 
@@ -201,6 +202,10 @@
                   double* ox, double* oy);
 int coreg_car_tile_margin(const coreg_wcs2d* hdr_target, const coreg_wcs2d* hdr_shifted, int32_t tile_w,
                           double tile_abs_lat_rad, double* margin_px);
+int coreg_lag_slots(int32_t n1, int32_t n2, int64_t nc, int64_t c, int64_t begin, int64_t end, int32_t sw, int32_t sh,
+                    int32_t packed, int64_t cap, int32_t* i1, int32_t* i2, int64_t* outidx, int64_t* counts3);
+int coreg_plan_lags(const double* geometry8, int32_t m1, int32_t n2, int64_t lds_elems, int32_t order, int32_t lag_packing,
+                    int64_t* plan8);
 
 
 int coreg_nansum_planes_be(const void* cube, int32_t bitpix, int64_t n_pixels, const int64_t* plane_index, int32_t n_sel,
```

Result: slower. 1.138 million lag-points/s (-1.9%).
